# danielzgtg/TTS.cpp

Measured on AMD Instinct MI355X. Metric: audio-sec/wall-sec (RTF^-1), Parler-TTS-mini v1 Q4_K AR decode + DAC decode, higher is better.
Workload: dtype q4_K weights x q8_K activations (int dot, f32 combine); DAC f16 im2col x f32 weights, f64 accumulate

## Files before the change

### include/tts_hip.h

```cpp
#ifndef TTS_HIP_H
#define TTS_HIP_H

#include <stddef.h>
#include <stdint.h>

#ifdef __cplusplus
extern "C" {
#endif

#define TTS_MAX_DIMS 4
#define TTS_MAX_SRC 4
#define TTS_MAX_OP_PARAMS 16
#define TTS_MAX_NAME 64

enum tts_type {
    TTS_TYPE_F32 = 0,
    TTS_TYPE_F16 = 1,
    TTS_TYPE_Q4_0 = 2,
    TTS_TYPE_Q4_1 = 3,
    TTS_TYPE_Q5_0 = 6,
    TTS_TYPE_Q5_1 = 7,
    TTS_TYPE_Q8_0 = 8,
    TTS_TYPE_Q8_1 = 9,
    TTS_TYPE_Q4_K = 12,
// ... 50 lines not shown
};

enum tts_custom_op {
    TTS_CUSTOM_NONE = 0,
    TTS_CUSTOM_UV_NOISE = 1,
    TTS_CUSTOM_CFG_SCALE = 2
};

enum tts_unary_op {
    TTS_UNARY_ABS = 0,
    TTS_UNARY_NEG,
    TTS_UNARY_TANH,
    TTS_UNARY_RELU,
    TTS_UNARY_SIGMOID,
    TTS_UNARY_GELU,
    TTS_UNARY_SILU,
    TTS_UNARY_EXP,
    TTS_UNARY_COUNT
};

enum tts_status {
    TTS_STATUS_SUCCESS = 0,
    TTS_STATUS_FAILED = -1,
    TTS_STATUS_ALLOC_FAILED = -2,
    TTS_STATUS_UNSUPPORTED = -3,
    TTS_STATUS_BAD_ARG = -4,
    TTS_STATUS_NO_DEVICE = -5
};

#define TTS_PROF_ATTN 39

#define TTS_FLAG_INPUT 1
#define TTS_FLAG_HOSTDATA 2
#define TTS_FLAG_OUTPUT 4
#define TTS_FLAG_PERSIST 8
#define TTS_FLAG_REPACKED 16
#define TTS_FLAG_TILED_COPY 64
#define TTS_FLAG_TILED 32

typedef struct tts_tensor {
    int32_t type;
    int32_t op;
    int64_t ne[TTS_MAX_DIMS];
    size_t nb[TTS_MAX_DIMS];
    int32_t op_params[TTS_MAX_OP_PARAMS];
    struct tts_tensor * src[TTS_MAX_SRC];
    struct tts_tensor * view_src;
    size_t view_offs;
    void * data;
    int32_t flags;
    int32_t pad_;
    char name[TTS_MAX_NAME];
} tts_tensor;

size_t tts_type_size(int type);
int64_t tts_blck_size(int type);
size_t tts_row_size(int type, int64_t ne0);
const char * tts_type_name(int type);
const char * tts_op_name(int op);

typedef struct tts_hip_backend * tts_hip_backend_t;

int tts_hip_device_count(void);
int tts_hip_device_memory(int device, size_t * free_bytes, size_t * total_bytes);
void * tts_hip_event_new(int device);
void tts_hip_event_free(void * event);
int tts_hip_event_record(tts_hip_backend_t backend, void * event);
int tts_hip_event_wait(tts_hip_backend_t backend, void * event);
int tts_hip_event_synchronize(void * event);
int tts_hip_is_device_pointer(const void * p);
tts_hip_backend_t tts_hip_backend_init(int device);
void tts_hip_backend_free(tts_hip_backend_t backend);
const char * tts_hip_backend_name(tts_hip_backend_t backend);

void * tts_hip_buffer_alloc(tts_hip_backend_t backend, size_t size);
void tts_hip_buffer_free(tts_hip_backend_t backend, void * ptr);
size_t tts_hip_buffer_alignment(void);

int tts_hip_tensor_set(tts_hip_backend_t backend, void * dst_dev, const void * src_host, size_t size);
int tts_hip_tensor_get(tts_hip_backend_t backend, void * dst_host, const void * src_dev, size_t size);
int tts_hip_tensor_copy(tts_hip_backend_t backend, void * dst_dev, const void * src_dev, size_t size);
int tts_hip_copy_stream(tts_hip_backend_t backend, void * dst_dev, const void * src_dev, size_t size);
int tts_hip_plan_stats(tts_tensor * const * nodes, int n_nodes, int mask, int32_t * counts);
int tts_hip_tensor_set_async(tts_hip_backend_t backend, void * dst_dev, const void * src_host, size_t size);
int tts_hip_memset(tts_hip_backend_t backend, void * dst_dev, int value, size_t size);
int tts_hip_synchronize(tts_hip_backend_t backend);

int tts_hip_weight_set(tts_hip_backend_t backend, tts_tensor * t, const void * src_host);
int tts_hip_weight_get(tts_hip_backend_t backend, const tts_tensor * t, void * dst_host);
int tts_hip_quantize(tts_hip_backend_t backend, int type, const float * x_dev, void * dst_dev, int64_t rows, int64_t K);
void tts_repack_q4_K(const void * src, void * dst, int64_t nblocks, int inverse);
void tts_repack_q4_K_tiled(const void * src, void * dst, int64_t nrows, int64_t nb, int inverse);

int tts_hip_supports_op(const tts_tensor * node);
int tts_hip_graph_compute(tts_hip_backend_t backend, tts_tensor * const * nodes, int n_nodes);
int tts_hip_graph_prepare(tts_hip_backend_t backend, tts_tensor * const * nodes, int n_nodes, int slot);
int tts_hip_graph_launch(tts_hip_backend_t backend, int slot);

enum tts_hip_option {
    TTS_HIP_OPT_FUSION = 0,
    TTS_HIP_OPT_PROFILE_GEMV = 1,
    TTS_HIP_OPT_GRAPHS = 2,
    TTS_HIP_OPT_CONV_F32ACC = 3,
    TTS_HIP_OPT_CONVT_LDS = 4,
    TTS_HIP_OPT_ATTN_SPLIT = 5,
    TTS_HIP_OPT_KV_PREFETCH = 6,
    TTS_HIP_OPT_KV_PREFETCH_BLOCKS = 7,
    TTS_HIP_OPT_Q4K_TILE_BYTES = 8,
    TTS_HIP_OPT_GEMV_DEBUG = 10,
    TTS_HIP_OPT_CONV_SPLIT = 12,
    TTS_HIP_OPT_GEMV_UNIQUE = 11,
    TTS_HIP_OPT_GEMV_KS = 13,
    TTS_HIP_OPT_ATTN_FUSED = 14,
    TTS_HIP_OPT_GEMM_Q8 = 18,
    TTS_HIP_OPT_BGEMM_F32 = 19,
    TTS_HIP_OPT_CU_PARTITION = 20,
    TTS_HIP_OPT_Q4K_DUAL_BYTES = 16,
    TTS_HIP_OPT_GEMV_RSPLIT = 17,
    TTS_HIP_OPT_ATTN_PV16 = 15,
    TTS_HIP_OPT_GEMV_PREQUANT = 21,
    TTS_HIP_OPT_GEMV_KRELAY = 22,
    TTS_HIP_OPT_ATTN_KS = 23,
    TTS_HIP_OPT_ATTN_PV8 = 24,
    TTS_HIP_OPT_GEMV_KRELAY_LOOP = 26,
    TTS_HIP_OPT_GEMV_Q80_PRO = 27,
    TTS_HIP_OPT_GEMV_Q80_SLAB = 28,
    TTS_HIP_OPT_GEMV_Q80_RW = 29,
    TTS_HIP_OPT_GEMM_Q8_STAGED = 30,
    TTS_HIP_OPT_GEMV_KR_INKERNEL = 31,
    TTS_HIP_OPT_GEMV_F32_WIDE = 32,
    TTS_HIP_OPT_ATTN_PV_MP = 33,
    TTS_HIP_OPT_GEMM_KR_INKERNEL = 35,
    TTS_HIP_OPT_GEMM_KR_CT2 = 36,
    TTS_HIP_OPT_GEMM_KR_NW = 34,
    TTS_HIP_OPT_GEMV_NW_MIN = 25,
    TTS_HIP_OPT_GEMM_KR_XCD = 38,
    TTS_HIP_OPT_GEMM_KR_CP = 39,
    TTS_HIP_OPT_GEMM_KR_WALK = 40,
    TTS_HIP_OPT_GEMM_PF = 41,
    TTS_HIP_OPT_GEMM_PF_NW = 42,
    TTS_HIP_OPT_ATTN_ONE = 43,
    TTS_HIP_OPT_GEMV_KR_TAIL = 44,
    TTS_HIP_OPT_GEMV_Q50_SLAB = 45,
    TTS_HIP_OPT_GEMV_Q50_RW = 46,
    TTS_HIP_OPT_GEMM_Q5 = 47,
    TTS_HIP_OPT_GEMM_Q5_STAGED = 48,
    TTS_HIP_OPT_GEMV_Q40_SLAB = 49,
    TTS_HIP_OPT_GEMV_Q40_RW = 50,
    TTS_HIP_OPT_GEMM_Q4_0 = 51,
    TTS_HIP_OPT_GEMM_Q4_0_STAGED = 52,
    TTS_HIP_OPT_CONV_VFMA = 53,
    TTS_HIP_OPT_CONV_TILE96 = 54,
    TTS_HIP_OPT_CONV_PACK = 55,
    TTS_HIP_OPT_COALESCE = 37,
};
enum tts_fuse_bits {
    TTS_FUSE_LN = 1, TTS_FUSE_GROUP = 2, TTS_FUSE_KV = 4, TTS_FUSE_EPI = 8, TTS_FUSE_HEADS = 16, TTS_FUSE_ATTN = 32,
    TTS_FUSE_LSTM = 64,
    TTS_FUSE_SNAKE = 128,
    TTS_FUSE_EMBED = 256,
    TTS_FUSE_CONV = 512,
    TTS_FUSE_ADAIN = 1024,
    TTS_FUSE_XATTN = 2048,
    TTS_FUSE_MCPY = 4096,
    TTS_FUSE_CONTREAD = 8192
};
int tts_hip_set_option(tts_hip_backend_t backend, int option, int value);
int tts_hip_attn_decode(tts_hip_backend_t backend, const tts_tensor * q, const tts_tensor * k, const tts_tensor * v,
                        const float * mask, int64_t mbs, float scale, float * out, float * out2, const int64_t * koff,
                        const int64_t * voff, const int64_t * moff, const int32_t * pseq);
int tts_hip_coalesce_stats(int device, int64_t * out, int n);
void tts_hip_coalesce_set_wait(int us);
int tts_hip_coalesce_enable(int on);
#define TTS_HIP_HOOK_FAULT_WEIGHT_SET 1
int tts_hip_test_hook(int hook, int value);
int tts_hip_install_crash_handler(void);
int tts_hip_gemv_stats(tts_hip_backend_t backend, int type, double * ms, int64_t * launches, double * bytes, int reset);
int tts_hip_greedy_step(tts_hip_backend_t backend, const float * logits, int32_t B, int32_t NH, int32_t V, int32_t step,
                        int32_t bos, int32_t eos, int32_t * eos_seen, int32_t * hist, int32_t * next);
typedef struct tts_sampling {
    float temperature;
    float top_p;
    float repetition_penalty;
    int32_t top_k;
    int32_t do_sample;
    int32_t pad_;
    uint64_t seed;
} tts_sampling;
void tts_sampling_default(tts_sampling * cfg);
uint32_t tts_sampler_call_seed(uint64_t seed, int32_t stream, int64_t call);
int tts_sampler_sample(const tts_sampling * cfg, const float * logits, int32_t NH, int32_t V, uint32_t call_seed, int32_t * last,
                       int32_t * count, int32_t * out);
int tts_hip_sample_step(tts_hip_backend_t backend, const float * logits, int32_t B, int32_t NH, int32_t V, const tts_sampling * cfg,
                        int64_t call, int32_t * rep_state, int32_t step, int32_t bos, int32_t eos, int32_t * eos_seen, int32_t * hist,
                        int32_t * next);
int tts_sampling_device_ok(const tts_sampling * cfg, int32_t V);
int tts_hip_counters(tts_hip_backend_t backend, int64_t * out, int n);

int tts_hip_gemv(tts_hip_backend_t backend, int type, const void * w, const float * x, float * y,
                 int64_t K, int64_t N, int64_t M);
int tts_hip_gemv_ex(tts_hip_backend_t backend, int type, const void * w, const float * x, float * y,
                    int64_t K, int64_t N, int64_t M, int32_t wflags);
int tts_hip_gemv_res(tts_hip_backend_t backend, int type, const void * w, const float * x, float * y, const float * res,
                     int64_t K, int64_t N, int64_t M, int32_t wflags);

typedef struct tts_backend_iface {
    void * ctx;
    const char * name;
    void * (*alloc)(void * ctx, size_t size);
    void (*free)(void * ctx, void * ptr);
    int (*set)(void * ctx, void * dst, const void * src, size_t size);
    int (*set_tensor)(void * ctx, tts_tensor * t, const void * src);
    int (*get)(void * ctx, void * dst, const void * src, size_t size);
    int (*memset)(void * ctx, void * dst, int value, size_t size);
    int (*compute)(void * ctx, tts_tensor * const * nodes, int n_nodes);
    int (*synchronize)(void * ctx);
    int (*prepare)(void * ctx, tts_tensor * const * nodes, int n_nodes, int slot);
    int (*launch)(void * ctx, int slot);
    int (*set_async)(void * ctx, void * dst, const void * src, size_t size);
    int (*copy)(void * ctx, void * dst, const void * src, size_t size);
    int (*greedy_step)(void * ctx, const float * logits, int B, int NH, int V, int step, int bos, int eos, int32_t * eos_seen,
                       int32_t * hist, int32_t * next);
    int (*sample_step)(void * ctx, const float * logits, int B, int NH, int V, const tts_sampling * cfg, int64_t call, int32_t * rep_state,
                       int step, int bos, int eos, int32_t * eos_seen, int32_t * hist, int32_t * next);
} tts_backend_iface;

int tts_hip_backend_iface(tts_hip_backend_t backend, tts_backend_iface * out);

#ifdef __cplusplus
}
#endif

#endif
```

### tts.cpp_amd/csrc/backend.hip

```cpp
#include <cmath>
#include <atomic>
#include <cstring>
#include <map>
#include <mutex>
#include <thread>

#include "hip_internal.h"
#include <hip/hip_ext.h>

#include <dlfcn.h>
#include <execinfo.h>
#include <fcntl.h>
#include <signal.h>
#include <unistd.h>

using namespace tts;


static void build_gelu_table(uint16_t * t) {
    const float GELU_COEF_A = 0.044715f;
    const float SQRT_2_OVER_PI = 0.79788456080286535587989211986876f;
    for (int i = 0; i < 65536; ++i) {
        const float x = fp16_to_fp32_host((uint16_t)i);
        const float g = 0.5f * x * (1.0f + tanhf(SQRT_2_OVER_PI * x * (1.0f + GELU_COEF_A * x * x)));
// ... 5 lines not shown
static const size_t kShadowBytes = 4u << 20;
static const size_t kLstmFloats = 4u << 20;
static const size_t kAttnFloats = 4u << 20;
static const size_t kVecScratchFloats = 1u << 18;
static const size_t kPinBytes = 16u << 20;

namespace {
std::mutex g_reg_mu;
struct BufRec {
    size_t size = 0;
};
std::map<const char *, BufRec> g_buffers;
std::unordered_map<const void *, uint8_t *> g_tiled;
std::atomic<size_t> g_tiled_n{0};
struct PackRec {
    float * img = nullptr;
    size_t src_bytes = 0;
};
std::map<tts::ConvPackKey, PackRec> g_packs;
std::atomic<size_t> g_packs_n{0};
std::atomic<size_t> g_packs_bytes{0};
std::atomic<uintptr_t> g_packs_lo{UINTPTR_MAX}, g_packs_hi{0};
}

namespace tts {
const uint8_t * tiled_copy_find(const void * w) {
    std::lock_guard<std::mutex> lk(g_reg_mu);
    auto it = g_tiled.find(w);
    return it == g_tiled.end() ? nullptr : it->second;
}
static std::atomic<int> g_coalesce_on{[] {
    const char * e = getenv("TTS_HIP_COALESCE");
    return e && e[0] == '0' ? 0 : 1;
}()};
bool coalesce_enabled() { return g_coalesce_on.load(std::memory_order_relaxed) != 0; }
const float * conv_pack_get(tts_hip_backend * be, const ConvPackKey & k) {
    std::lock_guard<std::mutex> lk(g_reg_mu);
    auto it = g_packs.find(k);
    if (it != g_packs.end()) return it->second.img;
    if (be->capturing) return nullptr;
    PackRec r;
    const size_t es = k.w16 ? 2 : 4;
    r.src_bytes = (size_t)((k.K - 1) * k.wk + (k.IC - 1) * k.wic + (k.OC - 1) * k.woc + 1) * es;
    const size_t bytes = k.floats() * sizeof(float);
    if (hipMalloc((void **)&r.img, bytes) != hipSuccess) {
        (void)hipGetLastError();
        return nullptr;
    }
    launch_conv1d_pack(be->stream, k, r.img);
    g_packs[k] = r;
    g_packs_lo.store(std::min(g_packs_lo.load(), (uintptr_t)k.w));
    g_packs_hi.store(std::max(g_packs_hi.load(), (uintptr_t)k.w + r.src_bytes));
    g_packs_n.store(g_packs.size(), std::memory_order_release);
    g_packs_bytes.fetch_add(bytes, std::memory_order_relaxed);
    return r.img;
}
void conv_pack_written(tts_hip_backend * be, const void * p, size_t n) {
    if (g_packs_n.load(std::memory_order_acquire) == 0) return;
    const char * a = (const char *)p;
    if ((uintptr_t)a >= g_packs_hi.load() || (uintptr_t)a + n <= g_packs_lo.load()) return;
    std::lock_guard<std::mutex> lk(g_reg_mu);
    for (auto & e : g_packs) {
        const char * w = (const char *)e.first.w;
        if (!(w < a + n && a < w + e.second.src_bytes)) continue;
        const tts_hip_backend * ob = e.first.be;
        if (ob->device == be->device) {
            launch_conv1d_pack(be->stream, e.first, e.second.img);
        } else {
            hipStreamSynchronize(be->stream);
            hipSetDevice(ob->device);
            launch_conv1d_pack(ob->stream, e.first, e.second.img);
            hipSetDevice(be->device);
        }
    }
}
void conv_pack_freed(const tts_hip_backend * be, const void * p, size_t n) {
    if (g_packs_n.load(std::memory_order_acquire) == 0) return;
    const char * a = (const char *)p;
    std::vector<float *> dead;
    {
        std::lock_guard<std::mutex> lk(g_reg_mu);
        for (auto it = g_packs.begin(); it != g_packs.end();) {
            const char * w = (const char *)it->first.w;
            if (be ? it->first.be == be : (w >= a && w < a + n)) {
                dead.push_back(it->second.img);
                g_packs_bytes.fetch_sub(it->first.floats() * sizeof(float), std::memory_order_relaxed);
                it = g_packs.erase(it);
            } else {
                ++it;
            }
        }
        if (g_packs.empty()) g_packs_lo.store(UINTPTR_MAX), g_packs_hi.store(0);
        g_packs_n.store(g_packs.size(), std::memory_order_release);
    }
    if (dead.empty()) return;
    hipDeviceSynchronize();
    for (float * c : dead) hipFree(c);
}
bool buffer_lookup(const void * p, const char ** base, size_t * size) {
    std::lock_guard<std::mutex> lk(g_reg_mu);
    auto it = g_buffers.upper_bound((const char *)p);
    if (it == g_buffers.begin()) return false;
    --it;
    if ((const char *)p >= it->first + it->second.size) return false;
    if (base) *base = it->first;
    if (size) *size = it->second.size;
    return true;
}
}

extern "C" {

int tts_hip_coalesce_enable(int on) { return tts::g_coalesce_on.exchange(on ? 1 : 0); }

int tts_hip_device_count(void) {
    int n = 0;
    if (hipGetDeviceCount(&n) != hipSuccess) return 0;
    return n;
}

tts_hip_backend_t tts_hip_backend_init(int device) {
    int n = tts_hip_device_count();
    if (device < 0 || device >= n) return nullptr;
    if (hipSetDevice(device) != hipSuccess) return nullptr;
    auto * be = new tts_hip_backend();
    be->device = device;
    TTS_HIP_CHECK(hipStreamCreateWithFlags(&be->stream, hipStreamNonBlocking));
    TTS_HIP_CHECK(hipStreamCreateWithFlags(&be->cap_stream, hipStreamNonBlocking));
    TTS_HIP_CHECK(hipStreamCreateWithFlags(&be->pf_stream, hipStreamNonBlocking));
    TTS_HIP_CHECK(hipEventCreateWithFlags(&be->co_ev, hipEventDisableTiming));
    TTS_HIP_CHECK(hipEventCreateWithFlags(&be->pf_fork, hipEventDisableTiming));
    TTS_HIP_CHECK(hipEventCreateWithFlags(&be->pf_join, hipEventDisableTiming));
    hipDeviceProp_t prop;
    TTS_HIP_CHECK(hipGetDeviceProperties(&prop, device));
    snprintf(be->name, sizeof(be->name), "HIP%d(%s)", device, prop.gcnArchName);
    be->cu_total = prop.multiProcessorCount > 0 ? prop.multiProcessorCount : 256;
    be->cus = be->cu_total;
    TTS_HIP_CHECK(hipMalloc((void **)&be->scratch, kScratchBytes));
    be->scratch_size = kScratchBytes;
    TTS_HIP_CHECK(hipMalloc((void **)&be->shadow, kShadowBytes));
    be->shadow_size = kShadowBytes;
    be->hoist_size = (size_t)8 << 20;
    TTS_HIP_CHECK(hipMalloc(&be->hoist, be->hoist_size));
    TTS_HIP_CHECK(hipMalloc((void **)&be->lstm_buf, kLstmFloats * sizeof(float)));
    TTS_HIP_CHECK(hipMalloc((void **)&be->attn_buf, kAttnFloats * sizeof(float)));
    be->attn_floats = kAttnFloats;
    TTS_HIP_CHECK(hipMalloc((void **)&be->vec_scratch, kVecScratchFloats * sizeof(float)));
    be->conv_stage_floats = (size_t)8 << 20;
    TTS_HIP_CHECK(hipMalloc((void **)&be->conv_stage, be->conv_stage_floats * sizeof(float)));
    if (const char * e = getenv("TTS_HIP_OPT_CONV_VFMA"))
        if (e[0] >= '0' && e[0] <= '2' && !e[1]) be->conv_vfma = e[0] - '0';
    if (const char * e = getenv("TTS_HIP_OPT_CONV_PACK"))
        if (e[0] >= '0' && e[0] <= '1' && !e[1]) be->conv_pack = e[0] - '0';
    be->conv_part_doubles = (size_t)8 << 20;
    TTS_HIP_CHECK(hipMalloc((void **)&be->conv_part, be->conv_part_doubles * sizeof(double)));
    be->lstm_floats = kLstmFloats;
    TTS_HIP_CHECK(hipMalloc((void **)&be->argmax_keys, kArgmaxRows * sizeof(unsigned long long)));
    TTS_HIP_CHECK(hipMalloc((void **)&be->argmax_counts, kArgmaxRows * sizeof(unsigned)));
    TTS_HIP_CHECK(hipMemset(be->argmax_keys, 0, kArgmaxRows * sizeof(unsigned long long)));
    TTS_HIP_CHECK(hipMemset(be->argmax_counts, 0, kArgmaxRows * sizeof(unsigned)));
    TTS_HIP_CHECK(hipHostMalloc((void **)&be->pin, kPinBytes, hipHostMallocDefault));
    be->pin_size = kPinBytes;
    for (auto & e : be->plan_ev) TTS_HIP_CHECK(hipEventCreateWithFlags(&e, hipEventDisableTiming));
    std::vector<uint16_t> tab(65536);
    build_gelu_table(tab.data());
    TTS_HIP_CHECK(hipMalloc((void **)&be->gelu_table, 65536 * sizeof(uint16_t)));
    TTS_HIP_CHECK(hipMemcpy(be->gelu_table, tab.data(), 65536 * sizeof(uint16_t), hipMemcpyHostToDevice));
    return be;
}

void tts_hip_backend_free(tts_hip_backend_t be) {
    if (!be) return;
    tts::coalesce_backend_gone(be);
    hipSetDevice(be->device);
    hipStreamSynchronize(be->stream);
    tts::conv_pack_freed(be, nullptr, 0);
    for (auto & p : be->ev_pending) {
        hipEventDestroy(p.first);
        hipEventDestroy(p.second);
    }
    for (auto e : be->ev_free) hipEventDestroy(e);
    for (auto & r : be->pin_pending) hipEventDestroy(r.ev);
    for (auto e : be->pin_events) hipEventDestroy(e);
    for (auto e : be->plan_ev) hipEventDestroy(e);
    hipHostFree(be->pin);
    if (be->rb_host) hipHostFree(be->rb_host);
    hipFree(be->scratch);
    hipFree(be->shadow);
    hipFree(be->argmax_keys);
    hipFree(be->argmax_counts);
    hipFree(be->lstm_buf);
    hipFree(be->hoist);
    hipFree(be->attn_buf);
    hipFree(be->vec_scratch);
    hipFree(be->conv_stage);
    hipFree(be->conv_part);
    hipFree(be->gelu_table);
    if (be->sample_cand) hipFree(be->sample_cand);
    if (be->repack_tmp) hipFree(be->repack_tmp);
    for (char * r : be->repack_retired) hipFree(r);
    if (be->attn_stage) hipFree(be->attn_stage);
    for (auto & ex : be->gsig_exec)
        if (ex) hipGraphExecDestroy(ex);
    for (auto & ex : be->pexec)
        if (ex) hipGraphExecDestroy(ex);
    hipStreamDestroy(be->stream);
    hipStreamDestroy(be->cap_stream);
    hipStreamDestroy(be->pf_stream);
    hipEventDestroy(be->pf_fork);
    hipEventDestroy(be->pf_join);
    hipEventDestroy(be->co_ev);
    delete be;
}

const char * tts_hip_backend_name(tts_hip_backend_t be) { return be ? be->name : "HIP(null)"; }

int tts_hip_device_memory(int device, size_t * free_bytes, size_t * total_bytes) {
    if (device < 0 || device >= tts_hip_device_count()) return TTS_STATUS_NO_DEVICE;
    int prev = 0;
    hipGetDevice(&prev);
    hipSetDevice(device);
    size_t f = 0, t = 0;
    const hipError_t e = hipMemGetInfo(&f, &t);
    hipSetDevice(prev);
    if (e != hipSuccess) return TTS_STATUS_FAILED;
    if (free_bytes) *free_bytes = f;
    if (total_bytes) *total_bytes = t;
    return 0;
}

void * tts_hip_event_new(int device) {
    if (device < 0 || device >= tts_hip_device_count()) return nullptr;
    hipSetDevice(device);
    hipEvent_t ev = nullptr;
    if (hipEventCreateWithFlags(&ev, hipEventDisableTiming) != hipSuccess) return nullptr;
    return (void *)ev;
}
void tts_hip_event_free(void * event) {
    if (event) hipEventDestroy((hipEvent_t)event);
}
int tts_hip_event_record(tts_hip_backend_t be, void * event) {
    if (!be || !event) return TTS_STATUS_BAD_ARG;
    hipSetDevice(be->device);
    return hipEventRecord((hipEvent_t)event, be->stream) == hipSuccess ? 0 : TTS_STATUS_FAILED;
}
int tts_hip_event_wait(tts_hip_backend_t be, void * event) {
    if (!be || !event) return TTS_STATUS_BAD_ARG;
    hipSetDevice(be->device);
    return hipStreamWaitEvent(be->stream, (hipEvent_t)event, 0) == hipSuccess ? 0 : TTS_STATUS_FAILED;
}
int tts_hip_event_synchronize(void * event) {
    if (!event) return TTS_STATUS_BAD_ARG;
    return hipEventSynchronize((hipEvent_t)event) == hipSuccess ? 0 : TTS_STATUS_FAILED;
}
int tts_hip_is_device_pointer(const void * p) {
    if (!p) return 0;
    hipPointerAttribute_t a;
    if (hipPointerGetAttributes(&a, p) != hipSuccess) {
        (void)hipGetLastError();
        return 0;
    }
    return a.type == hipMemoryTypeDevice ? 1 : 0;
}

size_t tts_hip_buffer_alignment(void) { return 256; }

void * tts_hip_buffer_alloc(tts_hip_backend_t be, size_t size) {
    if (!be) return nullptr;
    hipSetDevice(be->device);
    void * p = nullptr;
    BufRec r;
    r.size = size ? size : 256;
    if (hipMalloc(&p, r.size) != hipSuccess) return nullptr;
    std::lock_guard<std::mutex> lk(g_reg_mu);
    g_buffers[(const char *)p] = r;
    return p;
}

static void drop_tiled_copies(const void * p, size_t n) {
    if (g_tiled_n.load(std::memory_order_acquire) == 0) return;
    const char * a = (const char *)p;
    std::vector<uint8_t *> dead;
    {
        std::lock_guard<std::mutex> lk(g_reg_mu);
        for (auto it = g_tiled.begin(); it != g_tiled.end();) {
            const char * k = (const char *)it->first;
            if (k >= a && k < a + n) {
                dead.push_back(it->second);
                it = g_tiled.erase(it);
            } else {
                ++it;
            }
        }
        g_tiled_n.store(g_tiled.size(), std::memory_order_release);
    }
    if (dead.empty()) return;
    hipDeviceSynchronize();
    for (uint8_t * c : dead) hipFree(c);
}

void tts_hip_buffer_free(tts_hip_backend_t be, void * ptr) {
    if (!be || !ptr) return;
    hipSetDevice(be->device);
    hipStreamSynchronize(be->stream);
    BufRec r;
    bool known = false;
// ... 324 lines not shown
        l0 = l1 + 1;
    }
    const struct sigaction & prev = sig == SIGBUS ? g_prev_bus : g_prev_segv;
    if (prev.sa_flags & SA_SIGINFO) {
        if (prev.sa_sigaction) prev.sa_sigaction(sig, si, uc);
    } else if (prev.sa_handler != SIG_DFL && prev.sa_handler != SIG_IGN && prev.sa_handler) {
        prev.sa_handler(sig);
    }
    signal(sig, SIG_DFL);
    raise(sig);
}

int tts_hip_install_crash_handler(void) {
    void * warm[2];
    (void)backtrace(warm, 2);
    struct sigaction sa;
    memset(&sa, 0, sizeof sa);
    sa.sa_sigaction = crash_handler;
    sa.sa_flags = SA_SIGINFO | SA_RESETHAND;
    sigemptyset(&sa.sa_mask);
    if (sigaction(SIGSEGV, &sa, &g_prev_segv) != 0 || sigaction(SIGBUS, &sa, &g_prev_bus) != 0) return TTS_STATUS_FAILED;
    return 0;
}

int tts_hip_test_hook(int hook, int value) {
    if (hook == TTS_HIP_HOOK_FAULT_WEIGHT_SET) {
        g_fault_weight_set.store(value != 0);
        return 0;
    }
    return TTS_STATUS_BAD_ARG;
}

int tts_hip_weight_set(tts_hip_backend_t be, tts_tensor * t, const void * src) {
    if (!be || !t) return TTS_STATUS_BAD_ARG;
    if (t->type == TTS_TYPE_Q4_K && g_fault_weight_set.load(std::memory_order_relaxed)) return TTS_STATUS_ALLOC_FAILED;
    return weight_set_impl(be, t, src);
}

static int weight_set_impl(tts_hip_backend_t be, tts_tensor * t, const void * src) {
    const size_t n = tensor_bytes(t);
    if (t->type == TTS_TYPE_Q4_K && t->ne[0] % 256 == 0 && t->ne[1] % 4 == 0 && t->ne[2] == 1 && t->ne[3] == 1 &&
        be->q4k_tile_bytes > 0 && (int64_t)n >= be->q4k_tile_bytes) {
        std::vector<uint8_t> tmp(n);
        tts_repack_q4_K_tiled(src, tmp.data(), t->ne[1], t->ne[0] / 256, 0);
        int st = tts_hip_tensor_set(be, t->data, tmp.data(), n);
        if (st == 0) t->flags |= TTS_FLAG_REPACKED | TTS_FLAG_TILED;
        return st;
    }
    if (t->type == TTS_TYPE_Q4_K && t->ne[0] % 256 == 0) {
        std::vector<uint8_t> tmp(n);
        tts_repack_q4_K(src, tmp.data(), (int64_t)(n / 144), 0);
        t->flags &= ~TTS_FLAG_TILED_COPY;
        int st = tts_hip_tensor_set(be, t->data, tmp.data(), n);
        if (st == 0) t->flags |= TTS_FLAG_REPACKED;
        if (st == 0 && be->q4k_dual_bytes > 0 && (int64_t)n >= be->q4k_dual_bytes && t->ne[0] >= 2048 && t->ne[1] % 16 == 0 &&
            t->ne[2] == 1 && t->ne[3] == 1) {
            tts_repack_q4_K_tiled(src, tmp.data(), t->ne[1], t->ne[0] / 256, 0);
            uint8_t * cp = nullptr;
            if (hipMalloc((void **)&cp, n) != hipSuccess) return TTS_STATUS_ALLOC_FAILED;
            if (hipMemcpy(cp, tmp.data(), n, hipMemcpyHostToDevice) != hipSuccess) {
                hipFree(cp);
                return TTS_STATUS_FAILED;
            }
            {
                std::lock_guard<std::mutex> lk(g_reg_mu);
                g_tiled[t->data] = cp;
                g_tiled_n.store(g_tiled.size(), std::memory_order_release);
            }
            t->flags |= TTS_FLAG_TILED_COPY;
        }
        return st;
    }
    return tts_hip_tensor_set(be, t->data, src, n);
}

int tts_hip_weight_get(tts_hip_backend_t be, const tts_tensor * t, void * dst) {
    if (!be || !t) return TTS_STATUS_BAD_ARG;
    const size_t n = tensor_bytes(t);
    if (t->type == TTS_TYPE_Q4_K && (t->flags & TTS_FLAG_TILED)) {
        std::vector<uint8_t> tmp(n);
        int st = tts_hip_tensor_get(be, tmp.data(), t->data, n);
        if (st == 0) tts_repack_q4_K_tiled(tmp.data(), dst, t->ne[1], t->ne[0] / 256, 1);
        return st;
    }
    if (t->type == TTS_TYPE_Q4_K && (t->flags & TTS_FLAG_REPACKED)) {
        std::vector<uint8_t> tmp(n);
        int st = tts_hip_tensor_get(be, tmp.data(), t->data, n);
        if (st == 0) tts_repack_q4_K(tmp.data(), dst, (int64_t)(n / 144), 1);
        return st;
    }
    return tts_hip_tensor_get(be, dst, t->data, n);
}

static bool is_f32(const tts_tensor * t) { return t && t->type == TTS_TYPE_F32; }

int tts_hip_supports_op(const tts_tensor * n) {
    if (!n) return 0;
    for (int i = 0; i < TTS_MAX_SRC; ++i)
        if (n->src[i] && (n->src[i]->flags & 2)) return 0;
    switch (n->op) {
        case TTS_OP_NONE: case TTS_OP_VIEW: case TTS_OP_RESHAPE: case TTS_OP_PERMUTE: case TTS_OP_TRANSPOSE:
            return 1;
        case TTS_OP_DUP: case TTS_OP_CONT: case TTS_OP_CPY:
            return (n->type == TTS_TYPE_F32 || n->type == TTS_TYPE_F16 || n->type == TTS_TYPE_I32) &&
                   (n->src[0]->type == TTS_TYPE_F32 || n->src[0]->type == TTS_TYPE_F16 || n->src[0]->type == TTS_TYPE_I32);
        case TTS_OP_ADD: case TTS_OP_SUB: case TTS_OP_MUL: case TTS_OP_DIV:
        case TTS_OP_SQR: case TTS_OP_SQRT: case TTS_OP_SIN: case TTS_OP_COS: case TTS_OP_SCALE: case TTS_OP_CLAMP:
        case TTS_OP_LEAKY_RELU: case TTS_OP_ROUND: case TTS_OP_MOD: case TTS_OP_UNARY: case TTS_OP_CONCAT:
        case TTS_OP_REPEAT: case TTS_OP_SUM_ROWS:
            return 1;
        case TTS_OP_NORM: case TTS_OP_RMS_NORM:
            return is_f32(n->src[0]) && n->src[0]->nb[0] == 4;
        case TTS_OP_SOFT_MAX:
            return is_f32(n->src[0]);
        case TTS_OP_ROPE:
            return is_f32(n->src[0]);
        case TTS_OP_IM2COL:
            return is_f32(n->src[1]) && n->op_params[6] == 0 && (n->type == TTS_TYPE_F16 || n->type == TTS_TYPE_F32);
        case TTS_OP_CONV_TRANSPOSE_1D:
            return is_f32(n->src[0]) && is_f32(n->src[1]) && n->op_params[4] >= 1;
        case TTS_OP_CUMSUM: case TTS_OP_UPSCALE: case TTS_OP_STFT: case TTS_OP_ISTFT: case TTS_OP_MAP_CUSTOM3: case TTS_OP_MAP_CUSTOM2:
            return tts::audio_op_supported(n);
        case TTS_OP_GET_ROWS:
            return n->src[1]->type == TTS_TYPE_I32 &&
                   (n->src[0]->type == TTS_TYPE_F32 || n->src[0]->type == TTS_TYPE_F16 || n->src[0]->type == TTS_TYPE_Q4_K ||
                    n->src[0]->type == TTS_TYPE_Q8_0 || n->src[0]->type == TTS_TYPE_Q5_0 || n->src[0]->type == TTS_TYPE_Q4_0 ||
                    (n->src[0]->type == TTS_TYPE_Q6_K && n->src[0]->ne[0] % 256 == 0));
        case TTS_OP_MUL_MAT: {
            const tts_tensor * a = n->src[0];
            const tts_tensor * b = n->src[1];
            if (!is_f32(b)) return 0;
            if (a->ne[0] != b->ne[0] || b->ne[2] % a->ne[2] || b->ne[3] % a->ne[3]) return 0;
            if (a->type == TTS_TYPE_F32 || a->type == TTS_TYPE_F16) return 1;
            if (a->type == TTS_TYPE_Q4_K || a->type == TTS_TYPE_Q6_K) return a->ne[0] % 256 == 0;
            if (a->type == TTS_TYPE_Q8_0 || a->type == TTS_TYPE_Q5_0 || a->type == TTS_TYPE_Q4_0) return a->ne[0] % 32 == 0;
            return 0;
        }
        default:
            return 0;
    }
}

}

extern "C" int tts_hip_set_option(tts_hip_backend_t be, int option, int value) {
    if (!be) return TTS_STATUS_BAD_ARG;
    switch (option) {
        case TTS_HIP_OPT_FUSION: be->fusion = value; return 0;
        case TTS_HIP_OPT_CONVT_LDS: be->convt_lds = value != 0; return 0;
        case TTS_HIP_OPT_CONV_SPLIT: be->conv_split = value < 0 ? 1 : value; return 0;
        case TTS_HIP_OPT_CONV_VFMA: be->conv_vfma = value < 0 || value > 2 ? 1 : value; return 0;
        case TTS_HIP_OPT_CONV_TILE96: be->conv_tile96 = value != 0; return 0;
        case TTS_HIP_OPT_CONV_PACK: be->conv_pack = value != 0; return 0;
        case TTS_HIP_OPT_PROFILE_GEMV: be->profile_gemv = value != 0; return 0;
        case TTS_HIP_OPT_GRAPHS: be->use_graphs = value != 0; return 0;
        case TTS_HIP_OPT_CONV_F32ACC:
            be->conv_f32acc = value == 1;
            be->conv_acc_mode = value == 2 ? 2 : 0;
            return 0;
        case TTS_HIP_OPT_ATTN_SPLIT: be->attn_split_minp = value; return 0;
        case TTS_HIP_OPT_ATTN_FUSED: be->attn_fused_minp = value; return 0;
        case TTS_HIP_OPT_ATTN_PV16: be->attn_pv_uv16 = value != 0; return 0;
        case TTS_HIP_OPT_KV_PREFETCH: be->kv_prefetch_minp = value; return 0;
        case TTS_HIP_OPT_Q4K_TILE_BYTES: be->q4k_tile_bytes = value; return 0;
        case TTS_HIP_OPT_Q4K_DUAL_BYTES: be->q4k_dual_bytes = value; return 0;
        case TTS_HIP_OPT_GEMV_RSPLIT: be->gemv_mf_rsplit = value != 0; return 0;
        case TTS_HIP_OPT_GEMV_PREQUANT: be->gemv_mf_prequant = value != 0; return 0;
        case TTS_HIP_OPT_GEMV_KRELAY: be->gemv_kr = value != 0; return 0;
        case TTS_HIP_OPT_GEMV_KRELAY_LOOP: be->gemv_kr_loop = value != 0; return 0;
        case TTS_HIP_OPT_GEMV_Q80_PRO: be->gemv_q80_pro = value != 0; return 0;
        case TTS_HIP_OPT_GEMV_Q80_SLAB: be->gemv_q80_slab = value != 0; return 0;
        case TTS_HIP_OPT_GEMV_KR_INKERNEL:
            if (value < 0) return TTS_STATUS_BAD_ARG;
            be->gemv_kr_ink = value;
            return 0;
        case TTS_HIP_OPT_GEMM_Q8_STAGED:
            if (value < 0 || value > 2) return TTS_STATUS_BAD_ARG;
            be->gemm_q8_staged = value;
            return 0;
        case TTS_HIP_OPT_GEMV_Q80_RW:
            if (value < 0 || value > 32 || (value & (value - 1))) return TTS_STATUS_BAD_ARG;
            be->gemv_q80_rw = value;
            return 0;
        case TTS_HIP_OPT_GEMV_Q50_SLAB: be->gemv_q50_slab = value != 0; return 0;
        case TTS_HIP_OPT_GEMV_Q50_RW:
            if (value < 0 || value > 32 || (value & (value - 1))) return TTS_STATUS_BAD_ARG;
            be->gemv_q50_rw = value;
            return 0;
        case TTS_HIP_OPT_GEMM_Q5: be->gemm_q5 = value != 0; return 0;
        case TTS_HIP_OPT_GEMM_Q5_STAGED:
            if (value < 0 || value > 2) return TTS_STATUS_BAD_ARG;
            be->gemm_q5_staged = value;
            return 0;
        case TTS_HIP_OPT_GEMV_Q40_SLAB: be->gemv_q40_slab = value != 0; return 0;
        case TTS_HIP_OPT_GEMV_Q40_RW:
            if (value < 0 || value > 32 || (value & (value - 1))) return TTS_STATUS_BAD_ARG;
            be->gemv_q40_rw = value;
            return 0;
        case TTS_HIP_OPT_GEMM_Q4_0: be->gemm_q4_0 = value != 0; return 0;
        case TTS_HIP_OPT_GEMM_Q4_0_STAGED:
            if (value < 0 || value > 2) return TTS_STATUS_BAD_ARG;
            be->gemm_q4_0_staged = value;
            return 0;
        case TTS_HIP_OPT_ATTN_KS: be->attn_ks = value; return 0;
        case TTS_HIP_OPT_GEMV_NW_MIN: be->gemv_nw_min = value; return 0;
        case TTS_HIP_OPT_ATTN_PV8: be->attn_pv8 = value != 0; return 0;
        case TTS_HIP_OPT_GEMM_KR_CT2: be->gemm_kr_ct2 = value != 0; return 0;
        case TTS_HIP_OPT_GEMM_KR_INKERNEL: be->gemm_kr_ink = value < 0 ? 0 : value; return 0;
        case TTS_HIP_OPT_ATTN_PV_MP: be->attn_pv_mp = value == 2 ? 2 : value != 0; return 0;
        case TTS_HIP_OPT_ATTN_ONE:
            if (value < 0 || value > 2) return TTS_STATUS_BAD_ARG;
            be->attn_one = value;
            return 0;
        case TTS_HIP_OPT_GEMV_KR_TAIL:
            if (value < 0 || value > 4) return TTS_STATUS_BAD_ARG;
            be->gemv_kr_tail = value;
            return 0;
        case TTS_HIP_OPT_GEMM_KR_NW: be->gemm_kr_nw = value == 8 ? 8 : 4; return 0;
        case TTS_HIP_OPT_GEMM_Q8: be->gemm_q8 = value != 0; return 0;
        case TTS_HIP_OPT_CU_PARTITION: {
            const int count = value & 0xFF, index = (value >> 8) & 0xFF;
            const bool inter = (value >> 16) & 1;
            hipSetDevice(be->device);
            TTS_HIP_CHECK(hipStreamSynchronize(be->stream));
            hipStream_t ns = nullptr;
            if (count <= 1) {
                TTS_HIP_CHECK(hipStreamCreateWithFlags(&ns, hipStreamNonBlocking));
                be->cus = be->cu_total;
            } else {
                if (index >= count) return TTS_STATUS_BAD_ARG;
                std::vector<uint32_t> mask((be->cu_total + 31) / 32, 0u);
                const int per = be->cu_total / count;
                int n = 0;
                for (int c = 0; c < be->cu_total; ++c) {
                    const bool on = inter ? (c % count == index) : (c / per == index && c < per * count);
                    if (on) mask[c / 32] |= 1u << (c % 32), ++n;
                }
                if (hipExtStreamCreateWithCUMask(&ns, (uint32_t)mask.size(), mask.data()) != hipSuccess) return TTS_STATUS_FAILED;
                be->cus = n;
            }
            TTS_HIP_CHECK(hipStreamDestroy(be->stream));
            be->stream = ns;
            for (auto & ex : be->gsig_exec)
                if (ex) hipGraphExecDestroy(ex), ex = nullptr;
            for (auto & g : be->gsig) g = 0;
            return 0;
        }
        case TTS_HIP_OPT_BGEMM_F32: be->bgemm_f32 = value != 0; return 0;
        case TTS_HIP_OPT_GEMV_F32_WIDE: be->gemv_f32_wide = value != 0; return 0;
        case TTS_HIP_OPT_GEMV_DEBUG: be->gemv_dbg = value; return 0;
        case TTS_HIP_OPT_GEMV_UNIQUE: be->gemv_unique = value != 0; return 0;
        case TTS_HIP_OPT_GEMV_KS: be->gemv_ks_tiles = value > 0 ? value : 0; return 0;
        case TTS_HIP_OPT_COALESCE: be->co_member = value != 0; return 0;
        case TTS_HIP_OPT_GEMM_KR_XCD: be->gemm_kr_xcd = value != 0; return 0;
        case TTS_HIP_OPT_GEMM_KR_CP: be->gemm_kr_cp = value != 0; return 0;
        case TTS_HIP_OPT_GEMM_KR_WALK: be->gemm_kr_walk = value < 0 ? 0 : value; return 0;
        case TTS_HIP_OPT_GEMM_PF: be->gemm_pf = value < 0 ? 0 : value; return 0;
        case TTS_HIP_OPT_GEMM_PF_NW: be->gemm_pf_nw = value == 8 ? 8 : 4; return 0;
        case TTS_HIP_OPT_KV_PREFETCH_BLOCKS: be->kv_prefetch_blocks = value > 0 ? value : 1; return 0;
        default: return TTS_STATUS_BAD_ARG;
    }
}

extern "C" int tts_hip_counters(tts_hip_backend_t be, int64_t * out, int n) {
    if (!be || !out) return TTS_STATUS_BAD_ARG;
    const int64_t v[10] = {be->graph_updates, be->graph_instantiations, be->lstm_chains, be->lstm_steps, be->plan_wait_ns,
                           be->cap_plan_ns, be->cap_launch_ns, be->cap_update_ns, (int64_t)g_packs_n.load(), (int64_t)g_packs_bytes.load()};
    int k = 0;
    for (; k < n && k < 10; ++k) out[k] = v[k];
    return k;
}

extern "C" int tts_hip_gemv_stats(tts_hip_backend_t be, int type, double * ms, int64_t * launches, double * bytes, int reset) {
    if (!be) return TTS_STATUS_BAD_ARG;
    hipSetDevice(be->device);
    TTS_HIP_CHECK(hipStreamSynchronize(be->stream));
    for (size_t i = 0; i < be->ev_pending.size(); ++i) {
        float t = 0;
        TTS_HIP_CHECK(hipEventElapsedTime(&t, be->ev_pending[i].first, be->ev_pending[i].second));
        const int ty = be->ev_type[i];
        be->gemv_ms[ty] += t;
        be->gemv_launches[ty] += 1;
        be->gemv_bytes[ty] += be->ev_bytes[i];
        be->ev_free.push_back(be->ev_pending[i].first);
        be->ev_free.push_back(be->ev_pending[i].second);
    }
    be->ev_pending.clear();
    be->ev_bytes.clear();
    be->ev_type.clear();
    double a = 0, c = 0;
    int64_t b = 0;
    for (int ty = 0; ty < TTS_TYPE_COUNT; ++ty) {
        if (type >= 0 && ty != type) continue;
        a += be->gemv_ms[ty];
        b += be->gemv_launches[ty];
        c += be->gemv_bytes[ty];
    }
    if (ms) *ms = a;
    if (launches) *launches = b;
    if (bytes) *bytes = c;
    if (reset) {
        for (int ty = 0; ty < TTS_TYPE_COUNT; ++ty) {
            be->gemv_ms[ty] = 0;
            be->gemv_launches[ty] = 0;
            be->gemv_bytes[ty] = 0;
        }
// ... 47 lines not shown
```

### tts.cpp_amd/csrc/graph_exec.hip

```cpp
#include <algorithm>
#include <cstring>
#include <deque>
#include <unordered_map>
#include <vector>

#include <array>

#include "hip_internal.h"
#include <chrono>

using namespace tts;

namespace tts {
void launch_kv_prefetch(tts_hip_backend * be, hipStream_t st, const TD & t, int pdim, int blocks);
void launch_gemv_q4K_xattn(tts_hip_backend * be, const GemvJob & j, const XAttnArgs & a);
void launch_attn_decode(tts_hip_backend * be, const TD & q, const TD & k, const TD & v, const float * mask, float scale,
                        float * out, int hd, int P, int H, int n, int B, float * out2, int64_t obs = -1, int64_t mbs = 0,
                        const int64_t * koff = nullptr, const int64_t * voff = nullptr, const int64_t * moff = nullptr,
                        const int * pseq = nullptr);
void launch_attn_bias(tts_hip_backend * be, const TD & q, const TD & k, const TD & v, const float * bias, const float * mask,
                      float scale, float * out, int P, int H, int n);
void launch_layernorm(tts_hip_backend * be, const tts_tensor * dst, const tts_tensor * x, const float * w, const float * b,
                      float eps, bool rms);
}
// ... 1160 lines not shown
                it.snake_mask = m;
                act[index[x]] = -1;
            }
        }
        act[index[M1]] = act[index[S]] = act[index[Q]] = act[index[M2]] = -1;
        if (rfuse) {
            it.b = nullptr;
            it.snake_one = O;
            act[index[R]] = -1;
        }
        act[i] = add_item(std::move(it));
    }

    static bool vec_c(const tts_tensor * t, int64_t C) {
        if (!t || t->type != TTS_TYPE_F32 || t->ne[2] * t->ne[3] != 1 || t->nb[0] != 4) return false;
        return (t->ne[0] == C && t->ne[1] == 1) || (t->ne[0] == 1 && t->ne[1] == C && t->nb[1] == 4);
    }
    static bool same_shape(const tts_tensor * a, int64_t n0, int64_t n1) {
        return a->type == TTS_TYPE_F32 && a->ne[0] == n0 && a->ne[1] == n1 && a->ne[2] * a->ne[3] == 1;
    }
    static bool plan_debug() {
        static const bool dbg = getenv("TTS_PLAN_DEBUG") != nullptr;
        return dbg;
    }
    static void plan_reject(const char * what, int code) {
        if (plan_debug()) fprintf(stderr, "plan: %s not fused (check %d)\n", what, code);
    }
    static bool adain_fail(int code) {
        plan_reject("adain", code);
        return false;
    }
    bool try_adain(int i) {
        const tts_tensor * N = nodes[i];
        const tts_tensor * X = N->src[0];
        if (!X || X->type != TTS_TYPE_F32 || N->type != TTS_TYPE_F32 || X->nb[0] != 4 || N->ne[2] * N->ne[3] != 1) return adain_fail(1);
        const int64_t T = N->ne[0], C = N->ne[1];
        if (!adain_supported(T)) return adain_fail(2);
        const tts_tensor * T1 = sole_consumer(N);
        if (!T1 || T1->op != TTS_OP_TRANSPOSE) return adain_fail(3);
        const tts_tensor * C1 = sole_consumer(T1);
        if (!C1 || C1->op != TTS_OP_CONT || !same_shape(C1, C, T) || uses[C1] != 2) return adain_fail(4);
        const auto & cc = consumers[C1];
        if (cc.size() != 2) return adain_fail(5);
        const tts_tensor *M = nodes[cc[0]], *A1 = nodes[cc[1]];
        if (M->op != TTS_OP_MUL || M->src[0] != C1 || !vec_c(M->src[1], C) || sole_consumer(M) != A1) return adain_fail(6);
        if (A1->op != TTS_OP_ADD || A1->src[0] != C1 || A1->src[1] != M || !same_shape(A1, C, T)) return adain_fail(7);
        const tts_tensor * A2 = sole_consumer(A1);
        if (!A2 || A2->op != TTS_OP_ADD || A2->src[0] != A1 || !vec_c(A2->src[1], C) || !same_shape(A2, C, T)) return adain_fail(8);
        const tts_tensor * T2 = sole_consumer(A2);
        if (!T2 || T2->op != TTS_OP_TRANSPOSE) return adain_fail(9);
        const tts_tensor * C2 = sole_consumer(T2);
        if (!C2 || C2->op != TTS_OP_CONT || !same_shape(C2, T, C) || !contiguous(C2)) return adain_fail(10);
        const tts_tensor *gamma = M->src[1], *beta = A2->src[1];
        std::vector<int> absorbed = {i, index[C1], index[M], index[A1], index[A2], index[C2]};
        auto affine_src = [&](const tts_tensor * v, const tts_tensor * user, const tts_tensor *& W, const tts_tensor *& B,
                              const tts_tensor *& st) {
            if (!v || v->op != TTS_OP_ADD || sole_consumer(v) != user) return false;
            const tts_tensor * mm = v->src[0];
            if (!mm || mm->op != TTS_OP_MUL_MAT || sole_consumer(mm) != v || !vec_c(v->src[1], C) || v->src[1]->ne[0] != C) return false;
            W = mm->src[0], st = mm->src[1], B = v->src[1];
            const int64_t S = W->ne[0];
            return W->type == TTS_TYPE_F32 && contiguous(W) && W->ne[1] == C && W->ne[2] * W->ne[3] == 1 && S % 4 == 0 &&
                   ((uintptr_t)W->data % 16) == 0 && st->type == TTS_TYPE_F32 && contiguous(st) && st->ne[0] == S &&
                   st->ne[1] * st->ne[2] * st->ne[3] == 1 && ((uintptr_t)st->data % 16) == 0;
        };
        const tts_tensor *gW = nullptr, *gB = nullptr, *gS = nullptr, *bW = nullptr, *bB = nullptr, *bS = nullptr;
        const bool inline_gb = affine_src(gamma, M, gW, gB, gS) && affine_src(beta, A2, bW, bB, bS) && gS == bS;
        if (inline_gb) {
            for (const tts_tensor * t : {gamma, (const tts_tensor *)gamma->src[0], beta, (const tts_tensor *)beta->src[0]}) absorbed.push_back(index[t]);
            gamma = beta = nullptr;
        }
        const tts_tensor * out = C2;
        const tts_tensor *alpha = nullptr, *recip = nullptr, *one = nullptr;
        if ((mask & TTS_FUSE_SNAKE) && uses[C2] == 2) {
            const auto & sc = consumers[C2];
            const tts_tensor *M1 = nodes[sc[0]], *SA = nodes[sc[1]];
            const tts_tensor *S = sole_consumer(M1), *Q = S ? sole_consumer(S) : nullptr, *M2 = Q ? sole_consumer(Q) : nullptr;
            const tts_tensor * R = M2 ? M2->src[1] : nullptr;
            const tts_tensor * O = R ? R->src[0] : nullptr;
            const bool r_inline = R && R->op == TTS_OP_DIV && O && R->src[1] == M1->src[1] && sole_consumer(R) == M2 &&
                                  O->type == TTS_TYPE_F32 && O->nb[1] == 0 && O->ne[0] == 1 && O->ne[2] * O->ne[3] == 1 &&
                                  same_shape(R, 1, C);
            if (M1->op == TTS_OP_MUL && M1->src[0] == C2 && S && S->op == TTS_OP_SIN && Q && Q->op == TTS_OP_SQR && M2 &&
                M2->op == TTS_OP_MUL && M2->src[0] == Q && sole_consumer(M2) == SA && SA->op == TTS_OP_ADD && SA->src[0] == C2 &&
                SA->src[1] == M2 && vec_c(M1->src[1], C) && vec_c(M2->src[1], C) && same_shape(SA, T, C) && contiguous(SA) &&
                same_shape(M1, T, C) && same_shape(S, T, C) && same_shape(Q, T, C) && same_shape(M2, T, C)) {
                alpha = M1->src[1];
                recip = M2->src[1];
                out = SA;
                for (const tts_tensor * t : {M1, S, Q, M2, SA}) absorbed.push_back(index[t]);
                if (r_inline) {
                    absorbed.push_back(index[R]);
                    recip = nullptr;
                    one = O;
                }
            }
        }
        const bool in_place = out->data == X->data && out->nb[1] == X->nb[1];
        if (overlap(out, X) && !in_place) return adain_fail(11);
        bool stage = false;
        for (const tts_tensor * t : {gamma, beta, alpha, recip, one})
            if (t && overlap(out, t)) stage = true;
        if (inline_gb)
            for (const tts_tensor * t : {gW, gB, bW, bB, gS})
                if (overlap(out, t)) return adain_fail(14);
        if (stage && 4 * C + 1 > (int64_t)vec_cap) return adain_fail(12);
        const int last = *std::max_element(absorbed.begin(), absorbed.end());
        std::vector<bool> is_abs(n, false);
        for (int k : absorbed) is_abs[k] = true;
        for (int k = i + 1; k < last; ++k) {
            if (is_abs[k] || is_view(nodes[k]->op)) continue;
            const tts_tensor * w = nodes[k];
            for (const tts_tensor * t : {X, gamma, beta, alpha, recip, one, gW, gB, bW, bB, gS})
                if (t && t != w && overlap(w, t)) {
                    if (plan_debug()) fprintf(stderr, "plan: adain node %d (%s) between %d..%d overlaps an input\n", k, tts_op_name(w->op), i, last);
                    return adain_fail(13);
                }
        }
        AdainArgs a;
        a.x = (const float *)X->data;
        a.xcs = (int64_t)(X->nb[1] / 4);
        a.y = (float *)out->data;
        a.ycs = (int64_t)(out->nb[1] / 4);
        auto vstride = [](const tts_tensor * t) { return t->ne[0] == 1 ? (int64_t)(t->nb[1] / 4) : (int64_t)1; };
        if (inline_gb) {
            a.gw = (const float *)gW->data, a.gb = (const float *)gB->data;
            a.bw = (const float *)bW->data, a.bb = (const float *)bB->data;
            a.style = (const float *)gS->data, a.S = gW->ne[0];
        } else {
            a.gamma = (const float *)gamma->data, a.gcs = vstride(gamma);
            a.beta = (const float *)beta->data, a.bcs = vstride(beta);
        }
        if (alpha) {
            a.alpha = (const float *)alpha->data, a.acs = vstride(alpha);
            if (recip) a.recip = (const float *)recip->data, a.rcs = vstride(recip);
            else a.one = (const float *)one->data;
        }
        a.T = T, a.C = C;
        a.stage = stage;
        memcpy(&a.eps, &N->op_params[0], 4);
        Item it;
        it.kind = Item::ADAIN;
        it.adain = a;
        it.dst = out;
        for (int k : absorbed)
            if (k != last) act[k] = -1;
        act[last] = add_item(std::move(it));
        return true;
    }

    static const tts_tensor * through_view(const tts_tensor * t) { return t && t->op == TTS_OP_RESHAPE ? t->src[0] : t; }
    bool wr_hull = false;
    const char *wr_lo = nullptr, *wr_hi = nullptr;
    void try_conv(int i) {
        const tts_tensor * col = nodes[i];
        const tts_tensor *kern = col->src[0], *x = col->src[1];
        if (col->type != TTS_TYPE_F16 || col->op_params[6] != 0 || col->ne[2] * col->ne[3] != 1) return plan_reject("conv", 1);
        if (!x || x->type != TTS_TYPE_F32 || x->ne[2] * x->ne[3] != 1) return plan_reject("conv", 2);
        if (!kern || (kern->type != TTS_TYPE_F32 && kern->type != TTS_TYPE_F16) || kern->ne[3] != 1) return plan_reject("conv", 3);
        const tts_tensor * cv = sole_consumer(col);
        if (!cv || cv->op != TTS_OP_RESHAPE || !contiguous(col)) return plan_reject("conv", 4);
        const tts_tensor * mm = sole_consumer(cv);
        if (!mm || mm->op != TTS_OP_MUL_MAT || mm->src[0] != cv || mm->type != TTS_TYPE_F32) return plan_reject("conv", 5);
        const tts_tensor * wv = mm->src[1];
        if (!wv || through_view(wv) != kern) return plan_reject("conv", 6);
        const int K = (int)kern->ne[0];
        const int64_t IC = kern->ne[1], OC = kern->ne[2], L = x->ne[0], OL = col->ne[1];
        if (x->ne[1] != IC || mm->ne[0] != OL || mm->ne[1] != OC || !contiguous(mm)) return plan_reject("conv", 7);
        const int s = col->op_params[0], p = col->op_params[2], d = col->op_params[4];
        if (!conv1d_fused_ok(IC, K, s, d, nullptr)) return plan_reject("conv", 8);
        if (kern->nb[0] != tts_type_size(kern->type)) return plan_reject("conv", 9);
        const tts_tensor * out = mm;
        std::vector<int> absorbed = {i, (int)index[mm]};
        const tts_tensor * r3 = sole_consumer(mm);
        const tts_tensor * cur = mm;
        if (r3 && r3->op == TTS_OP_RESHAPE && r3->ne[0] == OL && r3->ne[1] == OC) cur = r3;
        Conv1dArgs a;
        const tts_tensor * bias = nullptr;
        const tts_tensor * res = nullptr;
        const tts_tensor * nb = sole_consumer(cur);
        if (nb && nb->op == TTS_OP_ADD && nb->src[0] == cur && nb->type == TTS_TYPE_F32 && contiguous(nb) && nb->ne[0] == OL &&
            nb->ne[1] == OC && nb->ne[2] * nb->ne[3] == 1 && chan_vec(nb->src[1], OC) && nb->src[1]->ne[1] == OC) {
            bias = nb->src[1];
            out = nb;
            absorbed.push_back(index[nb]);
            const tts_tensor * nr = sole_consumer(nb);
            if (nr && nr->op == TTS_OP_ADD && nr->type == TTS_TYPE_F32 && contiguous(nr) && nr->ne[0] == OL && nr->ne[1] == OC &&
                nr->ne[2] * nr->ne[3] == 1) {
                const tts_tensor * other = nr->src[0] == nb ? nr->src[1] : nr->src[0];
                if (other && other != nb && other->type == TTS_TYPE_F32 && contiguous(other) && other->ne[0] == OL && other->ne[1] == OC &&
                    other->ne[2] * other->ne[3] == 1 && (!overlap(nr, other) || nr->data == other->data)) {
                    res = other;
                    out = nr;
                    absorbed.push_back(index[nr]);
                }
            }
        }
        float * stage = nullptr;
        for (;;) {
            if (overlap(out, kern) || (bias && overlap(out, bias))) return plan_reject("conv", 10);
            stage = nullptr;
            bool ok = true;
            bool in_col = false;
            if (overlap(out, x)) {
                const size_t need = (size_t)OL * (size_t)OC * 4;
                if (tbytes(col) >= need && !overlap(col, x) && !overlap(col, out) && !(res && overlap(col, res)) && !overlap(col, kern) &&
                    !(bias && overlap(col, bias))) {
                    stage = (float *)col->data;
                    in_col = true;
                } else if (conv_stage && need <= 4 * conv_stage_cap) {
                    stage = conv_stage;
                } else {
                    ok = false;
                }
            }
            for (int j = i + 1; ok && j < absorbed.back(); ++j) {
                if (std::find(absorbed.begin(), absorbed.end(), j) != absorbed.end() || is_view(nodes[j]->op)) continue;
                if (overlap(nodes[j], x) || (in_col && overlap(nodes[j], col))) ok = false;
            }
            if (ok) break;
            if (!res) return plan_reject("conv", 11);
            res = nullptr;
            absorbed.pop_back();
            out = bias ? nb : mm;
        }
        a.x = make_td(x);
        a.w = kern->data;
        a.w16 = kern->type == TTS_TYPE_F16;
        const size_t es = tts_type_size(kern->type);
        a.wk = (int64_t)(kern->nb[0] / es), a.wic = (int64_t)(kern->nb[1] / es), a.woc = (int64_t)(kern->nb[2] / es);
        a.y = (float *)out->data;
        a.ycs = (int64_t)(out->nb[1] / 4);
        if (stage) {
            a.copy_dst = a.y;
            a.y = stage;
            a.ycs = OL;
        }
        if (bias) a.bias = (const float *)bias->data, a.bcs = bias->ne[1] == 1 ? 0 : (int64_t)(bias->nb[1] / 4);
        if (res) a.res = (const float *)res->data, a.rcs = (int64_t)(res->nb[1] / 4);
        a.L = L, a.IC = IC, a.OL = OL, a.OC = OC;
        a.K = K, a.s = s, a.p = p, a.d = d;
        const size_t xb = (size_t)((x->ne[0] - 1) * x->nb[0] + (x->ne[1] - 1) * x->nb[1]) + 4;
        const size_t wb = tbytes(kern);
        if (xb >= 0x80000000u || wb >= 0x80000000u) return plan_reject("conv", 12);
        a.x_bytes = (uint32_t)xb, a.w_bytes = (uint32_t)wb;
        a.w_stable = kern->op == TTS_OP_NONE && !(kern->flags & (TTS_FLAG_HOSTDATA | TTS_FLAG_OUTPUT)) && buffer_lookup(kern->data, nullptr, nullptr);
        if (a.w_stable && !wr_hull) {
            wr_hull = true;
            for (int j = 0; j < n; ++j) {
                if (is_view(nodes[j]->op) || !nodes[j]->data) continue;
                const char * lo = (const char *)nodes[j]->data;
                wr_lo = wr_lo ? std::min(wr_lo, lo) : lo;
                wr_hi = std::max(wr_hi, lo + tbytes(nodes[j]));
            }
        }
        if (a.w_stable && wr_lo && (const char *)kern->data < wr_hi && (const char *)kern->data + wb > wr_lo)
            for (int j = 0; a.w_stable && j < n; ++j)
                if (!is_view(nodes[j]->op) && nodes[j]->data && overlap(nodes[j], kern)) a.w_stable = 0;
        Item it;
        it.kind = Item::CONV;
        it.conv = a;
        it.dst = out;
        for (size_t k = 0; k + 1 < absorbed.size(); ++k) act[absorbed[k]] = -1;
        act[absorbed.back()] = add_item(std::move(it));
    }

    bool embed_terms(const tts_tensor * a, const tts_tensor * root, std::vector<const tts_tensor *> & terms, std::vector<int> & members) {
        if (a->op != TTS_OP_ADD || a->type != TTS_TYPE_F32) return false;
        for (int d = 0; d < 4; ++d)
            if (a->ne[d] != root->ne[d]) return false;
        const tts_tensor *l = a->src[0], *r = a->src[1];
        if (!l || !r) return false;
        const bool la = l->op == TTS_OP_ADD, ra = r->op == TTS_OP_ADD;
        if (la && ra) return false;
        auto leaf_ok = [&](const tts_tensor * g) {
            if (g->op != TTS_OP_GET_ROWS || sole_consumer(g) != a || g->type != TTS_TYPE_F32) return false;
            const tts_tensor *tab = g->src[0], *idx = g->src[1];
            if (tab->type != TTS_TYPE_F32 && tab->type != TTS_TYPE_F16 && tab->type != TTS_TYPE_Q8_0 && tab->type != TTS_TYPE_Q5_0 && tab->type != TTS_TYPE_Q4_0 && tab->type != TTS_TYPE_Q4_K && tab->type != TTS_TYPE_Q6_K) return false;
            if (idx->type != TTS_TYPE_I32 || idx->ne[1] * idx->ne[2] * idx->ne[3] != 1 || (idx->nb[0] % 4)) return false;
            if (tab->ne[0] != root->ne[0] || g->ne[0] != root->ne[0] || tab->ne[2] * tab->ne[3] != 1) return false;
            const int64_t rows = g->ne[1] * g->ne[2] * g->ne[3], M = root->ne[1] * root->ne[2] * root->ne[3];
            return idx->ne[0] == rows && (rows == 1 || rows == M);
        };
        if (la || ra) {
            const tts_tensor * inner = la ? l : r;
            const tts_tensor * leaf = la ? r : l;
            if (sole_consumer(inner) != a || !leaf_ok(leaf)) return false;
            if (!embed_terms(inner, root, terms, members)) return false;
            terms.push_back(leaf);
            members.push_back(index[leaf]);
            members.push_back(index[inner]);
            return true;
        }
        if (!leaf_ok(l) || !leaf_ok(r)) return false;
        terms.push_back(l);
        terms.push_back(r);
        members.push_back(index[l]);
        members.push_back(index[r]);
        return true;
    }
    void try_rint(int i) {
        const tts_tensor * R = nodes[i];
        if (R->type != TTS_TYPE_F32 || R->op_params[0] != 1 || !contiguous(R)) return;
        std::vector<const tts_tensor *> leaves;
        std::vector<int> members{i};
        const tts_tensor * t = R;
        while (t->op == TTS_OP_CONCAT && t->op_params[0] == 1) {
            leaves.push_back(t->src[1]);
            t = t->src[0];
            if (t->op == TTS_OP_CONCAT) {
                if (uses[t] != 1 || !index.count(t)) return;
                members.push_back(index[t]);
            }
        }
        leaves.push_back(t);
        std::reverse(leaves.begin(), leaves.end());
        const tts_tensor * a = nullptr;
        int64_t r = 0;
        for (size_t k = 0; k < leaves.size(); ++k) {
            const tts_tensor * rp = leaves[k];
            if (rp->op != TTS_OP_REPEAT || uses[rp] != 1 || !index.count(rp)) return;
            const tts_tensor * c = rp->src[0];
            if (!c || c->op != TTS_OP_CONT || uses[c] != 1 || !index.count(c)) return;
            const tts_tensor * v = c->src[0];
            if (!v || v->op != TTS_OP_VIEW || !v->view_src || v->ne[1] != 1) return;
            const tts_tensor * base = v->view_src;
            if (k == 0) {
                a = base;
                r = rp->ne[1];
                if (a->type != TTS_TYPE_F32 || (int64_t)leaves.size() != a->ne[1]) return;
            }
            if (base != a || rp->ne[1] != r || (const char *)v->data != (const char *)a->data + k * a->nb[1]) return;
            for (int d = 0; d < 4; ++d)
                if (d != 1 && (v->ne[d] != a->ne[d] || v->nb[d] != a->nb[d] || rp->ne[d] != a->ne[d])) return;
            members.push_back(index[rp]);
            members.push_back(index[c]);
        }
        if (!a || R->ne[1] != a->ne[1] * r || overlap(R, a)) return;
        for (int m : members)
            if (act[m] != 0) return;
        const int first = *std::min_element(members.begin(), members.end());
        for (int j = first + 1; j < i; ++j) {
            if (is_view(nodes[j]->op) || std::find(members.begin(), members.end(), j) != members.end()) continue;
            if (overlap(nodes[j], a)) return;
        }
        Item it;
        it.kind = Item::RINT;
        it.x = a;
        it.dst = R;
        it.rint = (int)r;
        for (int m : members) act[m] = -1;
        if (a->op == TTS_OP_CONT && a->src[0] && index.count(a) && act[index[a]] == 0) {
            const tts_tensor * s0 = a->src[0];
            bool ok = s0->type == TTS_TYPE_F32 && !overlap(R, s0);
            for (int d = 0; d < 4; ++d) ok &= s0->ne[d] == a->ne[d];
            auto ca = consumers.find(a);
            ok &= ca != consumers.end();
            if (ok)
                for (int k : ca->second) {
                    const tts_tensor * v = nodes[k];
                    const tts_tensor * u = sole_consumer(v);
                    ok &= v->op == TTS_OP_VIEW && u && std::find(members.begin(), members.end(), index[u]) != members.end();
                }
            const int ia = ok ? index[a] : 0;
            for (int j = ia + 1; ok && j < i; ++j) {
                if (is_view(nodes[j]->op) || std::find(members.begin(), members.end(), j) != members.end()) continue;
                if (overlap(nodes[j], s0)) ok = false;
            }
            if (ok) {
                it.x = s0;
                act[ia] = -1;
            }
        }
        rint_to_cpy(i, R, it);
        act[i] = add_item(std::move(it));
    }

    void rint_to_cpy(int i, const tts_tensor * R, Item & it) {
        const tts_tensor * X = sole_consumer(R);
        std::vector<int> skip;
        while (X && X->op == TTS_OP_RESHAPE && X->src[0] && contiguous(X)) X = sole_consumer(X);
        if (X && X->op == TTS_OP_CONT && contiguous(X) && index.count(X) && act[index[X]] == 0) {
            skip.push_back(index[X]);
            X = sole_consumer(X);
        }
        if (!X || X->op != TTS_OP_CPY || !index.count(X) || act[index[X]] != 0) return;
        const int iP = index[X];
        skip.push_back(iP);
        const tts_tensor * D = X;
        if (D->type != TTS_TYPE_F32 || D->nb[0] != 4 || D->ne[0] != R->ne[0] * R->ne[1] * R->ne[2] || D->ne[1] != R->ne[3] ||
            D->ne[2] != 1 || D->ne[3] != 1 || overlap(D, it.x))
            return;
        for (int j = i + 1; j < iP; ++j)
            if (!is_view(nodes[j]->op) && std::find(skip.begin(), skip.end(), j) == skip.end()) return;
        tts_tensor t = *R;
        t.data = D->data;
        t.nb[0] = 4;
        t.nb[1] = 4 * R->ne[0];
        t.nb[2] = t.nb[1] * R->ne[1];
        t.nb[3] = D->nb[1];
        it.node = t;
        it.rint_cpy = true;
        for (int k : skip) act[k] = -1;
    }

    void try_gather_t(int i) {
        const tts_tensor * C2 = nodes[i];
        const tts_tensor * Tv = C2->src[0];
        if (!Tv || Tv->op != TTS_OP_TRANSPOSE || C2->type != TTS_TYPE_F32 || !contiguous(C2) || uses[Tv] != 1) return;
        const tts_tensor * G = Tv->view_src ? Tv->view_src : Tv->src[0];
        if (!G || G->op != TTS_OP_GET_ROWS || !index.count(G) || act[index[G]] != 0 || uses[G] != 1 || G->type != TTS_TYPE_F32 ||
// ... 930 lines not shown
                        CO_NO();
                    pseq = (int *)&tab[of[3]];
                    pseq[k] = (int)mk->ne[1];
                    pmax = std::max(pmax, (int)mk->ne[1]);
                    ragged |= mk->ne[1] != it.k->ne[1];
                    if (it.mask) {
                        const tts_tensor * mm = cm.member(bc, it.mask, k);
                        if (!mm || mm->ne[0] != mk->ne[1] || mm->ne[1] < it.q->ne[1]) CO_NO();
                    }
                }
                tb.pmax = pmax;
                bc.ragged |= ragged;
                for (int w = 0; w < 2; ++w) {
                    const tts_tensor * kv = w ? it.v : it.k;
                    if (inter(kv)) {
                        if (ragged) CO_NO();
                        continue;
                    }
                    if (bc.stride(kv->data)) CO_NO();
                    of[1 + w] = alloc(N);
                    if (!offsets(kv, of[1 + w], 16)) CO_NO();
                    for (int k = 0; k < N; ++k) tab[of[1 + w] + k] *= 16;
                }
                if (it.mask) {
                    if (inter(it.mask)) {
                        if (ragged) CO_NO();
                    } else {
                        of[4] = alloc(N);
                        if (!offsets(it.mask, of[4], 4)) CO_NO();
                    }
                }
                break;
            }
            case Item::LN:
                if (it.dst->ne[3] != 1 || it.x->ne[3] != 1 || !inter(it.dst) || !inter(it.x) || !equal_all(it.dst) || !equal_all(it.x)) CO_NO();
                if (!share(it.w) || !share(it.b)) CO_NO();
                break;
            case Item::EMBED:
                if (it.gather_t || it.dst->ne[1] * it.dst->ne[2] * it.dst->ne[3] != 1 || !inter(it.dst) || !equal_all(it.dst)) CO_NO();
                if (it.terms.size() > (size_t)EMBED_MAX_TERMS) CO_NO();
                for (size_t t = 0; t < it.terms.size(); ++t) {
                    const tts_tensor * g = it.terms[t];
                    if (g->ne[1] * g->ne[2] * g->ne[3] != 1 || !equal_all(g) || !share(g->src[0])) CO_NO();
                    const tts_tensor * idx = g->src[1];
                    if (inter(idx)) continue;
                    if (!input_mem(idx) || !equal_all(idx)) CO_NO();
                    ioffs[a - 1][t] = alloc(N);
                    if (!offsets(idx, ioffs[a - 1][t], 4)) CO_NO();
                }
                break;
            case Item::NODE: {
                auto * e = cm.pos.find(nd);
                if (!e) CO_NO();
                cm.pos[&it.node] = e->second;
                if (!equal_all(nd)) CO_NO();
                for (int s2 = 0; s2 < TTS_MAX_SRC; ++s2) {
                    const tts_tensor * x = it.node.src[s2];
                    if (!x) continue;
                    if (!cm.pos.find(x) && owned_mem(x)) CO_NO();
                    if (cm.pos.find(x) && !equal_all(x)) CO_NO();
                }
                if (co_per_slice(bc, &it.node))
                    for (int s2 = 0; s2 < TTS_MAX_SRC; ++s2)
                        if (it.node.src[s2] && owned_mem(it.node.src[s2]) && !share(it.node.src[s2])) CO_NO();
                break;
            }
            default: CO_NO();
        }
    }
    *n_scatter = 0;
    std::vector<const tts_tensor *> outs;
    for (int i = 0; i < n_nodes; ++i)
        if ((nodes[i]->flags & TTS_FLAG_OUTPUT) || i == n_nodes - 1) outs.push_back(nodes[i]);
    std::vector<std::array<int64_t, 3>> sc;
    for (const tts_tensor * o : outs) {
        if (owned_mem(o) || is_view(o->op)) continue;
        if (!inter(o) || !contiguous(o) || (tbytes(o) & 3) || !equal_all(o)) CO_NO();
        for (int k = 0; k < N; ++k) {
            const tts_tensor * m = cm.member(bc, o, k);
            if (!m || !m->data || !contiguous(m)) CO_NO();
            sc.push_back({(int64_t)(uintptr_t)bc.reloc(o->data, k), (int64_t)(uintptr_t)m->data, (int64_t)tbytes(o)});
        }
    }
    if (!sc.empty()) {
        *scatter = alloc(3 * sc.size());
        for (size_t e = 0; e < sc.size(); ++e)
            for (int c = 0; c < 3; ++c) tab[*scatter + 3 * (int64_t)e + c] = sc[e][c];
        *n_scatter = (int)sc.size();
    }
    for (size_t a = 0; a < pl.items.size(); ++a)
        for (int t = 0; t < EMBED_MAX_TERMS; ++t)
            if (ioffs[a][t] >= 0) bc.tabs[a].ioff[t] = (const int64_t *)(intptr_t)(ioffs[a][t] + 1);
    return true;
}

static void co_readback(tts_hip_backend * be, const std::vector<int64_t> & sc, int n_sc) {
    BatchCtx & bc = *be->bat;
    const int N = bc.N;
    if ((int)bc.mbe.size() != N) return;
    std::vector<size_t> need(N, 0), off(N, 0);
    for (int e = 0; e < n_sc; ++e) need[e % N] += ((size_t)sc[3 * e + 2] + 255) & ~(size_t)255;
    for (int k = 0; k < N; ++k) {
        tts_hip_backend * m = bc.mbe[k];
        m->rb_clear();
        if (need[k] <= m->rb_cap) continue;
        if (m->rb_host) {
            TTS_HIP_CHECK(hipStreamSynchronize(be->stream));
            TTS_HIP_CHECK(hipHostFree(m->rb_host));
            m->rb_host = nullptr;
            m->rb_cap = 0;
        }
        if (hipHostMalloc((void **)&m->rb_host, need[k], hipHostMallocDefault) != hipSuccess) {
            (void)hipGetLastError();
            m->rb_host = nullptr;
            continue;
        }
        m->rb_cap = need[k];
    }
    for (int e = 0; e < n_sc; ++e) {
        const int k = e % N;
        tts_hip_backend * m = bc.mbe[k];
        if (!m->rb_host) continue;
        const size_t bytes = (size_t)sc[3 * e + 2];
        TTS_HIP_CHECK(hipMemcpyAsync(m->rb_host + off[k], (const void *)(uintptr_t)sc[3 * e], bytes, hipMemcpyDeviceToHost, be->stream));
        std::lock_guard<std::mutex> l(m->rb_mu);
        m->rb.push_back({(const char *)(uintptr_t)sc[3 * e + 1], bytes, off[k]});
        m->rb_any.store(true, std::memory_order_release);
        off[k] += (bytes + 255) & ~(size_t)255;
    }
}

__global__ void k_co_scatter(const int64_t * __restrict__ tab, int n) {
    const int e = blockIdx.y;
    if (e >= n) return;
    const uint32_t * src = (const uint32_t *)(uintptr_t)tab[3 * e];
    uint32_t * dst = (uint32_t *)(uintptr_t)tab[3 * e + 1];
    const int64_t w = tab[3 * e + 2] / 4;
    for (int64_t i = (int64_t)blockIdx.x * blockDim.x + threadIdx.x; i < w; i += (int64_t)gridDim.x * blockDim.x) dst[i] = src[i];
}

static bool capture_worthy(tts_hip_backend * be, tts_tensor * const * nodes, int n_nodes) {
    if (!be->use_graphs || be->profile_gemv) return false;
    for (int i = 0; i < n_nodes; ++i) {
        const tts_tensor * t = nodes[i];
        if (t->op == TTS_OP_MUL_MAT && t->src[1] && t->src[1]->ne[1] > 64) return false;
    }
    return true;
}

namespace tts {
static void plan_setup(Planner & pl, const tts_hip_backend * be);
}
static void conv_pack_prepare(tts_hip_backend * be, tts_tensor * const * nodes, int n_nodes) {
    if (!be->conv_pack || !(be->fusion & TTS_FUSE_CONV)) return;
    bool any = false;
    for (int i = 0; i < n_nodes && !any; ++i) any = nodes[i]->op == TTS_OP_IM2COL;
    if (!any) return;
    Planner pl;
    plan_setup(pl, be);
    pl.build(nodes, n_nodes);
    for (const Item & it : pl.items) {
        ConvPackKey k;
        if (it.kind == Item::CONV && conv1d_pack_key(be, it.conv, &k)) (void)conv_pack_get(be, k);
    }
}

static int capture_into(tts_hip_backend * be, tts_tensor * const * nodes, int n_nodes, hipGraphExec_t & ex) {
    conv_pack_prepare(be, nodes, n_nodes);
    hipStream_t run = be->stream;
    be->stream = be->cap_stream;
    be->capturing = true;
    const auto t0 = std::chrono::steady_clock::now();
    TTS_HIP_CHECK(hipStreamBeginCapture(be->stream, hipStreamCaptureModeThreadLocal));
    const int st = graph_compute_launches(be, nodes, n_nodes);
    hipGraph_t graph = nullptr;
    TTS_HIP_CHECK(hipStreamEndCapture(be->stream, &graph));
    be->stream = run;
    be->capturing = false;
    const auto t1 = std::chrono::steady_clock::now();
    be->cap_launch_ns += std::chrono::duration_cast<std::chrono::nanoseconds>(t1 - t0).count();
    if (st != 0) {
        if (graph) hipGraphDestroy(graph);
        return st;
    }
    bool ok = false;
    if (ex) {
        hipGraphNode_t err_node = nullptr;
        hipGraphExecUpdateResult res;
        ok = hipGraphExecUpdate(ex, graph, &err_node, &res) == hipSuccess && res == hipGraphExecUpdateSuccess;
        if (ok) be->graph_updates++;
        else {
            (void)hipGetLastError();
            TTS_HIP_CHECK(hipGraphExecDestroy(ex));
            ex = nullptr;
        }
    }
    if (!ok) {
        TTS_HIP_CHECK(hipGraphInstantiate(&ex, graph, nullptr, nullptr, 0));
        be->graph_instantiations++;
    }
    TTS_HIP_CHECK(hipGraphDestroy(graph));
    be->cap_update_ns += std::chrono::duration_cast<std::chrono::nanoseconds>(std::chrono::steady_clock::now() - t1).count();
    return 0;
}

extern "C" int tts_hip_graph_compute(tts_hip_backend_t be, tts_tensor * const * nodes, int n_nodes) {
    if (!be) return TTS_STATUS_BAD_ARG;
    hipSetDevice(be->device);
    be->rb_clear();
    const int cs = coalesce_submit(be, nodes, n_nodes);
    if (cs != kCoalesceNotTaken) return cs;
    uint64_t sig = 0x9E3779B97F4A7C15ull ^ (uint64_t)n_nodes;
    for (int i = 0; i < n_nodes; ++i) sig = (sig ^ (uint64_t)nodes[i]->op) * 0x100000001B3ull;
    if (n_nodes > 0)
        for (int d = 0; d < 4; ++d)
            sig = (sig ^ (uint64_t)nodes[0]->ne[d] ^ ((uint64_t)nodes[n_nodes - 1]->ne[d] << 32)) * 0x100000001B3ull;
    sig |= 1;
    int slot = -1;
    for (int k = 0; k < tts_hip_backend::N_GSIG; ++k)
        if (be->gsig[k] == sig) slot = k;
    if (slot < 0) {
        slot = be->gsig_next;
        be->gsig_next = (be->gsig_next + 1) % tts_hip_backend::N_GSIG;
        be->gsig[slot] = sig;
        if (be->gsig_exec[slot]) {
            TTS_HIP_CHECK(hipGraphExecDestroy(be->gsig_exec[slot]));
            be->gsig_exec[slot] = nullptr;
        }
        return graph_compute_launches(be, nodes, n_nodes);
    }
    if (!capture_worthy(be, nodes, n_nodes)) return graph_compute_launches(be, nodes, n_nodes);
    const int st = capture_into(be, nodes, n_nodes, be->gsig_exec[slot]);
    if (st != 0) return st;
    TTS_HIP_CHECK(hipGraphLaunch(be->gsig_exec[slot], be->stream));
    return 0;
}

extern "C" int tts_hip_graph_prepare(tts_hip_backend_t be, tts_tensor * const * nodes, int n_nodes, int slot) {
    if (!be || slot < 0 || slot > 1) return TTS_STATUS_BAD_ARG;
    hipSetDevice(be->device);
    be->rb_clear();
    if (be->plan_ev_pending[slot]) {
        const auto t0 = std::chrono::steady_clock::now();
        TTS_HIP_CHECK(hipEventSynchronize(be->plan_ev[slot]));
        be->plan_wait_ns += std::chrono::duration_cast<std::chrono::nanoseconds>(std::chrono::steady_clock::now() - t0).count();
        be->plan_ev_pending[slot] = false;
    }
    be->plan_nodes[slot] = nodes;
    be->plan_n[slot] = n_nodes;
    be->plan_eager[slot] = !capture_worthy(be, nodes, n_nodes);
    if (be->plan_eager[slot]) return 0;
    const int st = capture_into(be, nodes, n_nodes, be->pexec[slot]);
    be->plan_prepared[slot] = st == 0;
    return st;
}

extern "C" int tts_hip_graph_launch(tts_hip_backend_t be, int slot) {
    if (!be || slot < 0 || slot > 1) return TTS_STATUS_BAD_ARG;
    hipSetDevice(be->device);
    be->rb_clear();
    if (be->plan_eager[slot]) {
        const int st = graph_compute_launches(be, be->plan_nodes[slot], be->plan_n[slot]);
        if (st != 0) return st;
    } else {
        if (!be->pexec[slot]) return TTS_STATUS_BAD_ARG;
        TTS_HIP_CHECK(hipGraphLaunch(be->pexec[slot], be->stream));
        be->plan_prepared[slot] = false;
    }
    TTS_HIP_CHECK(hipEventRecord(be->plan_ev[slot], be->stream));
    be->plan_ev_pending[slot] = true;
    return 0;
}

extern "C" int tts_hip_plan_stats(tts_tensor * const * nodes, int n_nodes, int mask, int32_t * counts) {
    Planner pl;
    pl.mask = mask;
    pl.vec_cap = 1u << 18;
    static float lstm_stand_in alignas(256);
    pl.lstm_buf = &lstm_stand_in;
    pl.lstm_cap = (size_t)4 << 20;
    static float conv_stand_in alignas(256);
    pl.conv_stage = &conv_stand_in;
    pl.conv_stage_cap = (size_t)8 << 20;
    static char hoist_stand_in alignas(256);
    pl.hoist_buf = &hoist_stand_in;
    pl.hoist_cap = (size_t)8 << 20;
    if (mask) pl.build(nodes, n_nodes);
    else pl.act.assign(n_nodes, 0);
    for (int k = 0; k < 16; ++k) counts[k] = 0;
    for (const Item & it : pl.items) {
        counts[(int)it.kind]++;
        if (it.xattn >= 0) counts[14]++;
        if (it.kind == Item::GEMV) {
            counts[12] += (int32_t)it.mms.size();
            if ((int32_t)it.mms.size() > counts[13]) counts[13] = (int32_t)it.mms.size();
        }
    }
    static const bool dump = getenv("TTS_PLAN_DUMP") != nullptr;
    if (dump)
        for (int i = 0; i < n_nodes; ++i)
            if (pl.act[i] > 0) {
                const Item & it = pl.items[pl.act[i] - 1];
                fprintf(stderr, "item %d kind %d", i, (int)it.kind);
                if (it.kind == Item::GEMV)
                    fprintf(stderr, " mms %d K %lld N %lld M %lld epi %d ln %d", (int)it.mms.size(), (long long)it.mms[0]->src[0]->ne[0],
                            (long long)it.mms[0]->src[0]->ne[1], (long long)(nel(it.mms[0]->src[1]) / it.mms[0]->src[1]->ne[0]), it.epi, (int)it.ln);
                if (it.kind == Item::COPY) fprintf(stderr, " bytes %zu", it.cp_bytes);
                fprintf(stderr, "\n");
            }
    for (int i = 0; i < n_nodes; ++i)
        if (pl.act[i] == 0 && !is_view(nodes[i]->op)) {
            counts[15]++;
            if (dump)
                fprintf(stderr, "unfused %d op %d [%lld %lld %lld %lld] %s <- %s\n", i, (int)nodes[i]->op, (long long)nodes[i]->ne[0],
                        (long long)nodes[i]->ne[1], (long long)nodes[i]->ne[2], (long long)nodes[i]->ne[3], nodes[i]->name,
                        nodes[i]->src[0] ? nodes[i]->src[0]->name : "");
        }
    return (int)pl.items.size();
}

namespace tts {
static void plan_setup(Planner & pl, const tts_hip_backend * be) {
    pl.mask = be->fusion;
    pl.q80pro = be->gemv_q80_pro != 0;
    pl.lstm_buf = be->lstm_buf;
    pl.lstm_cap = be->lstm_floats;
    pl.vec_cap = be->vec_scratch ? (1u << 18) : 0;
    pl.conv_stage = be->conv_stage;
    pl.conv_stage_cap = be->conv_stage_floats;
    pl.hoist_buf = (char *)be->hoist;
    pl.hoist_cap = be->hoist_size;
}

int graph_compute_launches(tts_hip_backend_t be, tts_tensor * const * nodes, int n_nodes) {
    be->graph_epoch++;
    be->aq.src = nullptr;
    if (be->profile_gemv) launch_profile_spin(be, 4000.0);
    const auto tp0 = std::chrono::steady_clock::now();
    Planner pl;
    plan_setup(pl, be);
    if (be->fusion) pl.build(nodes, n_nodes);
    else pl.act.assign(n_nodes, 0);
    be->cap_plan_ns += std::chrono::duration_cast<std::chrono::nanoseconds>(std::chrono::steady_clock::now() - tp0).count();
    CoMap cm;
    int64_t sc_off = -1;
    int n_sc = 0;
    std::vector<int64_t> sc_host;
    if (be->bat) {
        const auto tq0 = std::chrono::steady_clock::now();
        struct Acc {
            tts_hip_backend * be;
            std::chrono::steady_clock::time_point t0;
            ~Acc() { be->co_prep_ns += std::chrono::duration_cast<std::chrono::nanoseconds>(std::chrono::steady_clock::now() - t0).count(); }
        } acc{be, tq0};
        BatchCtx & bc = *be->bat;
        cm.build(nodes, n_nodes);
        bc.comap = &cm;
        std::vector<std::tuple<const void *, const void *, size_t>> shared;
        std::vector<int64_t> tab;
        std::vector<std::array<int64_t, 5>> offs;
        if (!co_prepare(be, pl, nodes, n_nodes, shared, tab, offs, &sc_off, &n_sc)) {
            bc.comap = nullptr;
            return TTS_STATUS_UNSUPPORTED;
        }
        if (!coalesce_check_shared(be, shared)) {
            bc.differs = true;
            bc.comap = nullptr;
            return TTS_STATUS_UNSUPPORTED;
        }
        if (n_sc > 0) sc_host.assign(tab.begin() + sc_off, tab.begin() + sc_off + 3 * (int64_t)n_sc);
        if (!tab.empty()) {
            const size_t bytes = tab.size() * sizeof(int64_t);
            if (bytes > be->co_tab_bytes) {
                TTS_HIP_CHECK(hipStreamSynchronize(be->stream));
                if (be->co_tab) TTS_HIP_CHECK(hipFree(be->co_tab));
                be->co_tab_bytes = std::max(bytes * 2, (size_t)64 << 10);
                TTS_HIP_CHECK(hipMalloc((void **)&be->co_tab, be->co_tab_bytes));
            }
            if (tts_hip_tensor_set_async(be, be->co_tab, tab.data(), bytes) != 0) {
                bc.comap = nullptr;
                return TTS_STATUS_UNSUPPORTED;
            }
        }
        for (size_t a = 0; a < pl.items.size(); ++a) {
            ItemTab & tb = bc.tabs[a];
            const auto & of = offs[a];
            tb.yoff = of[0] >= 0 ? be->co_tab + of[0] : nullptr;
            tb.koff = of[1] >= 0 ? be->co_tab + of[1] : nullptr;
            tb.voff = of[2] >= 0 ? be->co_tab + of[2] : nullptr;
            tb.pseq = of[3] >= 0 ? (const int *)(be->co_tab + of[3]) : nullptr;
            tb.moff = of[4] >= 0 ? be->co_tab + of[4] : nullptr;
            for (auto & io : tb.ioff)
                if (io) io = be->co_tab + ((intptr_t)io - 1);
        }
    }
    std::vector<int> pf_items;
    if (be->fusion && be->kv_prefetch_minp > 0) {
        for (int i = 0; i < n_nodes; ++i) {
            const int a = pl.act[i];
            if (a > 0 && pl.items[a - 1].kind == Item::ATTN && pl.items[a - 1].k->ne[1] >= be->kv_prefetch_minp) pf_items.push_back(a - 1);
        }
    }
    size_t pf_next = 0;
    int pf_pending = -1;
    auto pf_fork = [&]() {
        if (pf_next >= pf_items.size()) return;
        const Item & t = pl.items[pf_items[pf_next]];
        TTS_HIP_CHECK(hipEventRecord(be->pf_fork, be->stream));
        TTS_HIP_CHECK(hipStreamWaitEvent(be->pf_stream, be->pf_fork, 0));
        launch_kv_prefetch(be, be->pf_stream, make_td(t.k), 1, be->kv_prefetch_blocks);
        launch_kv_prefetch(be, be->pf_stream, make_td(t.v), 0, be->kv_prefetch_blocks);
        TTS_HIP_CHECK(hipEventRecord(be->pf_join, be->pf_stream));
        pf_pending = pf_items[pf_next];
    };
    pf_fork();
    for (int i = 0; i < n_nodes; ++i) {
        tts_tensor * n = nodes[i];
        const int a = be->fusion ? pl.act[i] : 0;
        if (a < 0) continue;
        if (a == 0 && is_view(n->op)) continue;
        const bool is_pf = a > 0 && pf_pending == a - 1;
        if (is_pf) {
            TTS_HIP_CHECK(hipStreamWaitEvent(be->stream, be->pf_join, 0));
            pf_pending = -1;
        }
        const int st = a > 0 ? run_item(be, pl.items[a - 1], pl.items) : run_node(be, n);
        if (is_pf) {
            ++pf_next;
            pf_fork();
        }
        if (st != 0) {
            fprintf(stderr, "tts_hip_graph_compute: node %d (%s, %s) failed: %d\n", i, n->name, tts_op_name(n->op), st);
            if (pf_pending >= 0) (void)hipStreamWaitEvent(be->stream, be->pf_join, 0);
            return st;
        }
        if (be->bat) be->aq.src = nullptr;
        if (be->aq.src) {
            const char * s0 = (const char *)be->aq.src;
            const char * s1 = s0 + (size_t)be->aq.K * (size_t)be->aq.M * 4;
            bool keep = false;
            if (a > 0) {
                const Item & it = pl.items[a - 1];
                if (it.kind == Item::GEMV) {
                    keep = true;
                    for (size_t k = 0; k < it.tgt.size(); ++k) {
                        const char * y0 = (const char *)it.tgt[k].y;
                        const tts_tensor * mm = it.mms[k];
                        const int64_t Mm = mm->ne[1] * mm->ne[2] * mm->ne[3];
                        const char * y1 = y0 + 4 * (size_t)((Mm - 1) * it.tgt[k].ycs + (mm->ne[0] - 1) * it.tgt[k].yrs + 1);
                        if (y0 < s1 && s0 < y1) keep = false;
                    }
                }
            } else if (n->op == TTS_OP_MUL_MAT) {
                const char * y0 = (const char *)n->data;
                keep = !(y0 < s1 && s0 < y0 + tbytes(n));
            }
            if (!keep) be->aq.src = nullptr;
        }
    }
    if (pf_pending >= 0) TTS_HIP_CHECK(hipStreamWaitEvent(be->stream, be->pf_join, 0));
    if (be->bat) {
        if (n_sc > 0) {
            hipLaunchKernelGGL(k_co_scatter, dim3(4, (unsigned)n_sc), dim3(256), 0, be->stream, (const int64_t *)be->co_tab + sc_off, n_sc);
            TTS_HIP_CHECK(hipGetLastError());
            co_readback(be, sc_host, n_sc);
        }
        be->bat->comap = nullptr;
    }
    return 0;
}
}

extern "C" int tts_hip_gemv(tts_hip_backend_t be, int type, const void * w, const float * x, float * y, int64_t K, int64_t N,
                            int64_t M) {
    return tts_hip_gemv_ex(be, type, w, x, y, K, N, M, 0);
}

extern "C" int tts_hip_gemv_ex(tts_hip_backend_t be, int type, const void * w, const float * x, float * y, int64_t K, int64_t N,
                               int64_t M, int32_t wflags) {
    return tts_hip_gemv_res(be, type, w, x, y, nullptr, K, N, M, wflags);
}

extern "C" int tts_hip_gemv_res(tts_hip_backend_t be, int type, const void * w, const float * x, float * y, const float * res,
                                int64_t K, int64_t N, int64_t M, int32_t wflags) {
    if (!be) return TTS_STATUS_BAD_ARG;
    if ((wflags & TTS_FLAG_TILED) && (type != TTS_TYPE_Q4_K || N % 4)) return TTS_STATUS_BAD_ARG;
    if (tts::wtype_q8k_act(type) && K % 256) return TTS_STATUS_BAD_ARG;
    if (type == TTS_TYPE_Q6_K && ((uintptr_t)w & 1)) return TTS_STATUS_BAD_ARG;
    if (tts::wtype_q80_act(type) && K % 32) return TTS_STATUS_BAD_ARG;
    if (type != TTS_TYPE_Q4_K && type != TTS_TYPE_Q6_K && type != TTS_TYPE_Q8_0 && type != TTS_TYPE_Q5_0 && type != TTS_TYPE_Q4_0 && type != TTS_TYPE_F16 && type != TTS_TYPE_F32) return TTS_STATUS_UNSUPPORTED;
    if ((type == TTS_TYPE_F32 || type == TTS_TYPE_F16) && K % 4) return TTS_STATUS_BAD_ARG;
    hipSetDevice(be->device);
    GemvJob j;
    j.wtype = type;
    j.K = K;
    j.N = N;
    j.M = M;
    j.w_row_bytes = (int64_t)tts_row_size(type, K);
    j.W[0] = (const uint8_t *)w;
    j.Y[0] = y;
    j.ycs[0] = N;
    j.yrs[0] = 1;
    j.x = x;
    j.xcs = K;
    if (res) {
        j.epi = EPI_ADD;
        j.res = res;
        j.rcs = N;
    }
    const bool q80pro = tts::wtype_q80_act(type) && K % QK_K == 0 && M <= 8 && be->gemv_q80_pro;
    if (tts::wtype_q8k_act(type) || q80pro) {
        j.pro = PRO_QUANT;
        j.tiled = (wflags & TTS_FLAG_TILED) ? 1 : 0;
        if ((uintptr_t)x & 15) {
            if ((size_t)(4 * K * M) > be->scratch_size) return TTS_STATUS_ALLOC_FAILED;
            launch_copy_cols(be, (float *)be->scratch, x, K, K, M);
            be->aq.src = nullptr;
            j.x = (const float *)be->scratch;
        }
    } else if (type != TTS_TYPE_F32) {
        if (act_quant_bytes(type, K, M) > be->scratch_size) return TTS_STATUS_ALLOC_FAILED;
        launch_quantize_act(be, type, x, K, K, M, j.aq);
    } else {
        j.aq.vtype = TTS_TYPE_F32;
    }
    be->aq.src = nullptr;
    if (type == TTS_TYPE_Q6_K && !tts::gemv_q6k_ok(j)) return TTS_STATUS_UNSUPPORTED;
    launch_gemv_job(be, j);
    return 0;
}
```

### tts.cpp_amd/csrc/hip_internal.h

```cpp
#pragma once

#include <hip/hip_fp16.h>
#include <hip/hip_runtime.h>

#include <cstdio>
#include <cstdlib>
#include <atomic>
#include <deque>
#include <mutex>
#include <unordered_map>
#include <tuple>
#include <vector>

#include "common.h"

#define TTS_HIP_CHECK(expr)                                                                          \
    do {                                                                                             \
        hipError_t err_ = (expr);                                                                    \
        if (err_ != hipSuccess) {                                                                    \
            fprintf(stderr, "%s:%d: HIP error %s: %s\n", __FILE__, __LINE__, #expr, hipGetErrorString(err_)); \
            abort();                                                                                 \
        }                                                                                            \
    } while (0)

// ... 253 lines not shown
    const int64_t * voff = nullptr;
    const int64_t * moff = nullptr;
    const int * pseq = nullptr;
};

constexpr int EMBED_MAX_TERMS = 16;
struct BatchCls {
    const char * b0 = nullptr;
    size_t size = 0;
    char * win = nullptr;
    int64_t stride = 0;
};
struct ItemTab {
    const int64_t * yoff = nullptr;
    int32_t yoff_mats = 0;
    const int64_t *koff = nullptr, *voff = nullptr;
    const int64_t * moff = nullptr;
    const int * pseq = nullptr;
    int pmax = 0;
    const int64_t * ioff[EMBED_MAX_TERMS] = {};
};
struct BatchCtx {
    int N = 0;
    uint64_t key = 0;
    std::vector<BatchCls> cls;
    std::vector<tts_tensor * const *> mnodes;
    std::vector<tts_hip_backend *> mbe;
    int n_nodes = 0;
    bool checked = false;
    int canon = 0;
    bool ragged = false;
    bool differs = false;
    std::vector<ItemTab> tabs;
    void * comap = nullptr;
    const BatchCls * find(const void * p) const {
        const char * c = (const char *)p;
        size_t lo = 0, hi = cls.size();
        while (lo < hi) {
            const size_t m = (lo + hi) / 2;
            if (cls[m].b0 <= c) lo = m + 1;
            else hi = m;
        }
        if (lo == 0) return nullptr;
        const BatchCls & b = cls[lo - 1];
        return c < b.b0 + b.size ? &b : nullptr;
    }
    template <typename T>
    T * win(T * p) const {
        const BatchCls * b = p ? find(p) : nullptr;
        return b ? (T *)(b->win + ((const char *)p - b->b0)) : p;
    }
    int64_t stride(const void * p) const {
        const BatchCls * b = p ? find(p) : nullptr;
        return b ? b->stride : 0;
    }
    template <typename T>
    T * reloc(T * p, int k) const {
        const BatchCls * b = p ? find(p) : nullptr;
        return b ? (T *)(b->win + k * b->stride + ((const char *)p - b->b0)) : p;
    }
};

}

struct tts_hip_backend {
    int device = 0;
    hipStream_t stream = nullptr;
    char name[64] = {0};
    char * scratch = nullptr;
    size_t scratch_size = 0;
    float * shadow = nullptr;
    size_t shadow_size = 0;
    void * hoist = nullptr;
    size_t hoist_size = 0;
    float * attn_buf = nullptr;
    size_t attn_floats = 0;
    int attn_split_minp = 128;
    int attn_ks = 2;
    int attn_pv_mp = 1;
    int attn_one = 1;
    int attn_pv8 = 0;
    int attn_pv_uv16 = 0;
    int attn_fused_minp = 0;
    unsigned long long * argmax_keys = nullptr;
    unsigned * argmax_counts = nullptr;
    int64_t q4k_tile_bytes = 4 << 20;
    int gemv_dbg = 0;
    int gemv_unique = 1;
    int gemm_q8 = 1;
    int64_t cus = 256;
    int cu_total = 256;
    int bgemm_f32 = 1;
    int gemv_f32_wide = 1;
    int gemm_kr_nw = 4;
    int64_t gemv_ks_tiles = 256;
    int gemv_mf_prequant = 1;
    int gemv_kr = 1;
    int gemv_kr_loop = 1;
    int gemv_kr_tail = 1;
    int gemv_q80_pro = 1;
    int gemv_q80_slab = 1;
    int gemv_q80_rw = 0;
    int gemm_q8_staged = 2;
    int gemv_q50_slab = 1;
    int gemv_q50_rw = 0;
    int gemm_q5 = 1;
    int gemm_q5_staged = 2;
    int gemv_q40_slab = 1;
    int gemv_q40_rw = 0;
    int gemm_q4_0 = 1;
    int gemm_q4_0_staged = 2;
    int64_t gemv_kr_ink = 0;
    int gemm_kr_walk = 0;
    int gemm_pf = 64;
    int gemm_pf_nw = 4;
    int gemm_kr_cp = 0;
    int gemm_kr_xcd = 0;
    int gemm_kr_ct2 = 0;
    int64_t gemm_kr_ink = 0;
    int gemv_nw_min = 0;
    int gemv_mf_rsplit = 1;
    int64_t q4k_dual_bytes = 1 << 20;
    void * sample_cand = nullptr;
    size_t sample_cand_size = 0;
    int kv_prefetch_minp = 0;
    int kv_prefetch_blocks = 128;
    hipStream_t pf_stream = nullptr;
    hipEvent_t pf_fork = nullptr, pf_join = nullptr;
    uint8_t * pin = nullptr;
    size_t pin_size = 0, pin_head = 0;
    struct PinRec {
        size_t off, size;
        hipEvent_t ev;
    };
    std::deque<PinRec> pin_pending;
    std::vector<hipEvent_t> pin_events;
    std::mutex pin_mu;
    hipEvent_t plan_ev[2] = {nullptr, nullptr};
    bool plan_ev_pending[2] = {false, false};
    float * lstm_buf = nullptr;
    float * conv_stage = nullptr;
    size_t conv_stage_floats = 0;
    float * vec_scratch = nullptr;
    size_t lstm_floats = 0;
    tts::ActQuant aq;
    int64_t graph_epoch = 0;
    uint16_t * gelu_table = nullptr;
    bool convt_lds = true;
    double * conv_part = nullptr;
    size_t conv_part_doubles = 0;
    int conv_vfma = 1;
    int conv_tile96 = 1;
    int conv_pack = 1;
    bool capturing = false;
    int conv_split = 1;
    int fusion = 0x3FFF;
    bool profile_gemv = false;
    double gemv_ms[TTS_TYPE_COUNT] = {0};
    int64_t gemv_launches[TTS_TYPE_COUNT] = {0};
    double gemv_bytes[TTS_TYPE_COUNT] = {0};
    std::vector<std::pair<hipEvent_t, hipEvent_t>> ev_pending;
    std::vector<double> ev_bytes;
    std::vector<int> ev_type;
    std::vector<hipEvent_t> ev_free;
    char * repack_tmp = nullptr;
    size_t repack_tmp_size = 0;
    std::vector<char *> repack_retired;
    float * attn_stage = nullptr;
    size_t attn_stage_size = 0;
    bool use_graphs = false;
    static constexpr int N_GSIG = 4;
    uint64_t gsig[N_GSIG] = {};
    hipGraphExec_t gsig_exec[N_GSIG] = {};
    int gsig_next = 0;
    bool conv_f32acc = false;
    int conv_acc_mode = 0;
    hipStream_t cap_stream = nullptr;
    int64_t graph_updates = 0, graph_instantiations = 0;
    int64_t lstm_chains = 0, lstm_steps = 0;
    int64_t plan_wait_ns = 0;
    int64_t cap_plan_ns = 0, cap_launch_ns = 0, cap_update_ns = 0;
    hipGraphExec_t pexec[2] = {nullptr, nullptr};
    tts_tensor * const * plan_nodes[2] = {nullptr, nullptr};
    int plan_n[2] = {0, 0};
    bool plan_eager[2] = {true, true};
    bool plan_prepared[2] = {false, false};
    tts::BatchCtx * bat = nullptr;
    hipEvent_t co_ev = nullptr;
    int64_t * co_tab = nullptr;
    size_t co_tab_bytes = 0;
    int64_t co_prep_ns = 0;
    bool co_member = true;
    struct RbEnt {
        const char * dev;
        size_t bytes, off;
    };
    char * rb_host = nullptr;
    size_t rb_cap = 0;
    std::vector<RbEnt> rb;
    std::mutex rb_mu;
    std::atomic<bool> rb_any{false};
    void rb_clear() {
        if (!rb_any.load(std::memory_order_acquire)) return;
        std::lock_guard<std::mutex> l(rb_mu);
        rb.clear();
        rb_any.store(false, std::memory_order_release);
    }
};

namespace tts {

const uint8_t * tiled_copy_find(const void * weight);

void profile_pair(tts_hip_backend * be, hipEvent_t & e0, hipEvent_t & e1);
void profile_push(tts_hip_backend * be, hipEvent_t e0, hipEvent_t e1, double bytes, int type);

void launch_quantize_act(tts_hip_backend * be, int wtype, const float * x, int64_t xcs, int64_t K, int64_t M, ActQuant & aq);
void launch_gemv_job(tts_hip_backend * be, const GemvJob & job);
bool gemv_q6k_ok(const GemvJob & j);
bool launch_bgemm_f32(tts_hip_backend * be, const tts_tensor * node);
bool gemm_f32_ok(const GemvJob & j);
void launch_gemm_f32(tts_hip_backend * be, const GemvJob & j);
void launch_copy_cols(tts_hip_backend * be, float * dst, const float * src, int64_t K, int64_t scs, int64_t M);
void launch_profile_spin(tts_hip_backend * be, double us);
void launch_im2col(tts_hip_backend * be, const tts_tensor * node);
constexpr int kLstmQMaxK = 512;
struct LstmStepArgs {
    const float * pre[4];
    const void * w[4];
    int64_t w_rs[4];
    const float * bias[4];
    const float * hprev;
    const float * cprev;
    float * h;
    float * c;
    int Hd, K, wtype;
};
void launch_lstm_step(tts_hip_backend * be, const LstmStepArgs & a, const LstmStepArgs * b = nullptr);
void launch_repeat_interleave1(tts_hip_backend * be, const tts_tensor * dst, const tts_tensor * a, int r);
void launch_copy_bytes(tts_hip_backend * be, void * dst, const void * src, size_t bytes);
void launch_cpy_multi(tts_hip_backend * be, const tts_tensor * src, const tts_tensor * const * dsts, int nd);
void launch_rope_multi(tts_hip_backend * be, const tts_tensor * rope, const tts_tensor * src, const tts_tensor * const * dsts, int nd);
void launch_greedy_step(tts_hip_backend * be, const float * logits, int B, int NH, int V, int step, int bos, int eos, int32_t * eos_seen,
                        int32_t * hist, int32_t * next);
int launch_sample_step(tts_hip_backend * be, const float * logits, int B, int NH, int V, const tts_sampling * c, int64_t call,
                       int32_t * rep_state, int step, int bos, int eos, int32_t * eos_seen, int32_t * hist, int32_t * next);
struct BatchCtx;
void launch_embed_sum(tts_hip_backend * be, const tts_tensor * out, const tts_tensor * const * gr, int n, const BatchCtx * bat = nullptr,
                      const ItemTab * tab = nullptr);
void launch_snake(tts_hip_backend * be, const tts_tensor * dst, const tts_tensor * x, const tts_tensor * alpha, const tts_tensor * recip,
                  const tts_tensor * one = nullptr, const tts_tensor * mask = nullptr);
void launch_lstm_finish(tts_hip_backend * be, const tts_tensor * final_out, const float * hist, int64_t Hd, int64_t T);
bool audio_op_supported(const tts_tensor * n);
int launch_audio_op(tts_hip_backend * be, const tts_tensor * n);
void launch_conv_transpose_1d(tts_hip_backend * be, const tts_tensor * node);
constexpr int CONV1D_MAX_R = 128;
struct Conv1dArgs {
    TD x;
    const void * w = nullptr;
    int w16 = 0;
    int64_t wk = 0, wic = 0, woc = 0;
    float * y = nullptr;
    int64_t ycs = 0;
    const float * bias = nullptr;
    int64_t bcs = 0;
    const float * res = nullptr;
    int64_t rcs = 0;
    int64_t L = 0, IC = 0, OL = 0, OC = 0;
    int K = 1, s = 1, p = 0, d = 1;
    int icc = 0, xw = 0, rs = 0;
    float * copy_dst = nullptr;
    uint32_t x_bytes = 0, w_bytes = 0;
    double * part = nullptr;
    int ic_per_split = 0;
    int w_stable = 0;
    const float * wimg = nullptr;
};
constexpr int CONV1D_XN = 16, CONV1D_WN = 16;
inline int conv1d_icc(int64_t IC, int K, int xw) {
    int best = 0;
    double best_eff = -1.0;
    const int top = (int)(IC < 64 ? IC : 64);
    for (int c = 1; c <= top; ++c) {
        const int r = c * K, rp = (r + 31) & ~31;
        if (rp > 64 || c * xw > 256 * CONV1D_XN) break;
        const double eff = (double)r / rp + 1e-4 * c;
        if (eff > best_eff) best_eff = eff, best = c;
    }
    return best;
}
bool conv1d_fused_ok(int64_t IC, int K, int s, int d, size_t * lds);
__host__ __device__ inline int64_t conv1d_pack_index(int nchunk, int oct, int rp, int ct, int chunk, int row, int r) {
    const int lane = (r & 3) * 16 + (row & 15);
    return (int64_t)(ct * nchunk + chunk) * oct * rp + ((((row >> 4) * (rp >> 4) + (r >> 4)) * 64 + lane) * 4 + ((r >> 2) & 3));
}
struct ConvPackKey {
    const tts_hip_backend * be;
    const void * w;
    int w16, K, oct, icc, rp;
    int64_t IC, OC, wk, wic, woc;
    bool operator<(const ConvPackKey & o) const {
        return std::tie(be, w, w16, K, oct, icc, rp, IC, OC, wk, wic, woc) <
               std::tie(o.be, o.w, o.w16, o.K, o.oct, o.icc, o.rp, o.IC, o.OC, o.wk, o.wic, o.woc);
    }
    int nchunk() const { return (int)((IC + icc - 1) / icc); }
    int ntile() const { return (int)((OC + oct - 1) / oct); }
    size_t floats() const { return (size_t)ntile() * nchunk() * oct * rp; }
};
void launch_conv1d_pack(hipStream_t stream, const ConvPackKey & k, float * img);
const float * conv_pack_get(tts_hip_backend * be, const ConvPackKey & k);
void conv_pack_written(tts_hip_backend * be, const void * p, size_t n);
void conv_pack_freed(const tts_hip_backend * be, const void * p, size_t n);
bool conv1d_pack_key(const tts_hip_backend * be, const Conv1dArgs & a, ConvPackKey * k);
struct AdainArgs {
    const float * x = nullptr;
    int64_t xcs = 0;
    float * y = nullptr;
    int64_t ycs = 0;
    const float *gamma = nullptr, *beta = nullptr, *alpha = nullptr, *recip = nullptr;
    const float * one = nullptr;
    int stage = 0;
    const float *gw = nullptr, *gb = nullptr, *bw = nullptr, *bb = nullptr, *style = nullptr;
    int64_t S = 0;
    int64_t gcs = 1, bcs = 1, acs = 1, rcs = 1;
    int64_t T = 0, C = 0;
    float eps = 0.f;
};
bool adain_supported(int64_t T);
void launch_adain_snake(tts_hip_backend * be, const AdainArgs & a);
void launch_conv1d_fused(tts_hip_backend * be, Conv1dArgs a);
bool launch_gemm_f16(tts_hip_backend * be, const tts_tensor * node);
size_t act_quant_bytes(int wtype, int64_t K, int64_t M);
void act_quant_layout(int wtype, char * base, int64_t K, int64_t M, ActQuant & aq);

void launch_repack_q4_K(tts_hip_backend * be, const void * src, void * dst, int64_t nblocks, int inverse);

int launch_op(tts_hip_backend * be, const tts_tensor * node);
void launch_copy_stream(tts_hip_backend * be, void * dst, const void * src, int64_t n16);

int graph_compute_launches(tts_hip_backend * be, tts_tensor * const * nodes, int n_nodes);
constexpr int kCoalesceNotTaken = 1 << 20;
int coalesce_submit(tts_hip_backend * be, tts_tensor * const * nodes, int n_nodes);
bool buffer_lookup(const void * p, const char ** base, size_t * size);
bool coalesce_check_shared(tts_hip_backend * ex, const std::vector<std::tuple<const void *, const void *, size_t>> & pairs);
void coalesce_backend_gone(const tts_hip_backend * be);
void coalesce_written(const void * p, size_t size);
bool coalesce_enabled();
bool co_debug();

}
```

### tts.cpp_amd/csrc/k_conv.hip

```cpp
#include "hip_internal.h"

namespace tts {

template <bool F16OUT>
__global__ void k_im2col(TD dst, TD x, int K, int s0, int p0, int d0, int64_t n) {
    const int64_t KW = dst.ne[0];
    const int64_t OL = dst.ne[1];
    const int64_t L = x.ne[0];
    for (int64_t e = (int64_t)blockIdx.x * blockDim.x + threadIdx.x; e < n; e += (int64_t)gridDim.x * blockDim.x) {
        const int64_t kk = e % KW;
        const int64_t ol = (e / KW) % OL;
        const int64_t nn = e / (KW * OL);
        const int64_t ic = kk / K, k = kk % K;
        const int64_t il = ol * s0 + k * d0 - p0;
        float v = 0.f;
        if (il >= 0 && il < L) v = *(const float *)(x.data + il * x.nb[0] + ic * x.nb[1] + nn * x.nb[2]);
        char * o = dst.data + kk * dst.nb[0] + ol * dst.nb[1] + nn * dst.nb[2];
        if (F16OUT) *(__half *)o = __float2half_rn(v);
        else *(float *)o = v;
    }
}

void launch_im2col(tts_hip_backend * be, const tts_tensor * node) {
    const tts_tensor * a = node->src[0];
// ... 273 lines not shown

template <bool W16, bool BIAS, bool RES, bool H32 = false, int MT = 2>
__global__ __launch_bounds__(256) __attribute__((amdgpu_waves_per_eu(MT == 2 ? 1 : 2))) void k_conv1d_f64(Conv1dArgs a) {
    constexpr int OCT = 32 * MT, WN = CONV1D_WN * MT / 2;
    extern __shared__ float sm[];
    __shared__ int xoff[CONV1D_MAX_R];
    __shared__ int wofs[CONV1D_MAX_R];
    const int lane = threadIdx.x & 63, wave = threadIdx.x >> 6;
    const int c16 = lane & 15, kq = lane >> 4;
    const int64_t ol0 = (int64_t)blockIdx.x * 64;
    const int oc0 = blockIdx.y * OCT;
    const int K = a.K, s = a.s, icc = a.icc, xw = a.xw, rs = a.rs;
    const int R = icc * K, Rp = (R + 31) & ~31;
    float * xs = sm;
    float * ws = sm + icc * xw + 1;
    const int zslot = icc * xw;
    for (int r = threadIdx.x; r < Rp; r += 256) {
        const int ic = r / K, k = r - ic * K;
        xoff[r] = r < R ? ic * xw + k * a.d : zslot;
        wofs[r] = r < R ? (int)(k * a.wk + ic * a.wic) : -1;
    }
    if (threadIdx.x == 0) xs[zslot] = 0.f;
    __syncthreads();
    const int wr0 = (wave >> 1) * 16 * MT, wc0 = (wave & 1) * 32;
    const bool wave_live = oc0 + wr0 < a.OC && ol0 + wc0 < a.OL;
    f64x4_t acc[MT][2] = {};
    const int64_t base = ol0 * s - a.p;
    const int EX = icc * xw, EW = OCT * Rp;
    constexpr int esz = W16 ? 2 : 4;
    const uint32_t OOB = 0x80000000u;
    const auto xr = __builtin_amdgcn_make_buffer_rsrc(a.x.data, 0, a.x_bytes, 0x00020000);
    const auto wr = __builtin_amdgcn_make_buffer_rsrc(const_cast<void *>(a.w), 0, a.w_bytes, 0x00020000);
    const int rsh = Rp == 64 ? 6 : 5;
    uint32_t xrel[CONV1D_XN], wrel[WN];
#pragma unroll
    for (int u = 0; u < CONV1D_XN; ++u) {
        const int e = (int)threadIdx.x + 256 * u;
        const int ic = e / xw, q = e - ic * xw;
        const int64_t pos = base + q;
        const bool ok = e < EX && pos >= 0 && pos < a.L;
        xrel[u] = ok ? (uint32_t)(pos * a.x.nb[0] + (int64_t)ic * a.x.nb[1]) : OOB;
    }
#pragma unroll
    for (int u = 0; u < WN; ++u) {
        const int e = (int)threadIdx.x + 256 * u;
        const int oc = e >> rsh, r = e & (Rp - 1);
        const int wo = e < EW ? wofs[r] : -1;
        const bool ok = wo >= 0 && oc0 + oc < a.OC;
        wrel[u] = ok ? (uint32_t)(((int64_t)(oc0 + oc) * a.woc + wo) * esz) : OOB;
    }
    float xv[CONV1D_XN], wv[WN];
    auto fetch = [&](int ic0) {
        const int nic = min(icc, (int)(a.IC - ic0));
        const uint32_t xc = (uint32_t)((int64_t)ic0 * a.x.nb[1]);
        const uint32_t wc = (uint32_t)((int64_t)ic0 * a.wic * esz);
#pragma unroll
        for (int u = 0; u < CONV1D_XN; ++u) {
            const uint32_t off = (xrel[u] == OOB || (int)threadIdx.x + 256 * u >= nic * xw) ? OOB : xrel[u] + xc;
            xv[u] = __builtin_bit_cast(float, __builtin_amdgcn_raw_buffer_load_b32(xr, off, 0, 0));
        }
#pragma unroll
        for (int u = 0; u < WN; ++u) {
            const uint32_t off = (wrel[u] == OOB || (((int)threadIdx.x + 256 * u) & (Rp - 1)) >= nic * K) ? OOB : wrel[u] + wc;
            if (W16) wv[u] = __half2float(__builtin_bit_cast(__half, __builtin_amdgcn_raw_buffer_load_b16(wr, off, 0, 0)));
            else wv[u] = __builtin_bit_cast(float, __builtin_amdgcn_raw_buffer_load_b32(wr, off, 0, 0));
        }
    };
    const int ic_lo = a.part ? (int)blockIdx.z * a.ic_per_split : 0;
    const int ic_hi = a.part ? (int)min((int64_t)(ic_lo + a.ic_per_split), a.IC) : (int)a.IC;
    fetch(ic_lo);
    for (int ic0 = ic_lo; ic0 < ic_hi; ic0 += icc) {
#pragma unroll
        for (int u = 0; u < CONV1D_XN; ++u)
            if ((int)threadIdx.x + 256 * u < EX) xs[(int)threadIdx.x + 256 * u] = __half2float(__float2half_rn(xv[u]));
#pragma unroll
        for (int u = 0; u < WN; ++u) {
            const int e = (int)threadIdx.x + 256 * u;
            if (e < EW) ws[e + (e >> rsh)] = W16 ? wv[u] : __half2float(__float2half_rn(wv[u]));
        }
        __syncthreads();
        if (ic0 + icc < ic_hi) fetch(ic0 + icc);
        if (!wave_live) {
            __syncthreads();
            continue;
        }
        if (H32) {
            for (int r0 = 0; r0 < Rp; r0 += 32) {
                int xo[8];
#pragma unroll
                for (int u = 0; u < 8; ++u) xo[u] = xoff[r0 + 8 * kq + u];
                h16x8_t A[MT], B[2];
#pragma unroll
                for (int u = 0; u < 8; ++u) {
                    const bool z = xo[u] == zslot;
#pragma unroll
                    for (int t = 0; t < MT; ++t) A[t][u] = (_Float16)ws[(wr0 + 16 * t + c16) * rs + r0 + 8 * kq + u];
#pragma unroll
                    for (int t = 0; t < 2; ++t) B[t][u] = (_Float16)xs[z ? zslot : xo[u] + (wc0 + 16 * t + c16) * s];
                }
#pragma unroll
                for (int ti = 0; ti < MT; ++ti)
#pragma unroll
                    for (int tj = 0; tj < 2; ++tj) {
                        const f32x4 pr = __builtin_amdgcn_mfma_f32_16x16x32_f16(A[ti], B[tj], f32x4{0.f, 0.f, 0.f, 0.f}, 0, 0, 0);
#pragma unroll
                        for (int e = 0; e < 4; ++e) acc[ti][tj][e] += (double)pr[e];
                    }
            }
        } else
        for (int r0 = 0; r0 < Rp; r0 += 32) {
            int xo[8];
#pragma unroll
            for (int u = 0; u < 8; ++u) xo[u] = xoff[r0 + 4 * u + kq];
            float af[8][MT], bf[8][2];
#pragma unroll
            for (int u = 0; u < 8; ++u) {
                const int r = r0 + 4 * u + kq;
                const bool z = xo[u] == zslot;
#pragma unroll
                for (int t = 0; t < MT; ++t) af[u][t] = ws[(wr0 + 16 * t + c16) * rs + r];
#pragma unroll
                for (int t = 0; t < 2; ++t) bf[u][t] = xs[z ? zslot : xo[u] + (wc0 + 16 * t + c16) * s];
            }
#pragma unroll
            for (int u = 0; u < 8; ++u)
#pragma unroll
                for (int ti = 0; ti < MT; ++ti)
#pragma unroll
                    for (int tj = 0; tj < 2; ++tj)
                        acc[ti][tj] = __builtin_amdgcn_mfma_f64_16x16x4f64((double)af[u][ti], (double)bf[u][tj], acc[ti][tj], 0, 0, 0);
        }
        __syncthreads();
    }
    conv1d_store<BIAS, RES, H32, MT>(a, acc, ol0, oc0, wr0, wc0, c16, kq);
}

__global__ __launch_bounds__(256) void k_conv1d_pack(ConvPackKey k, float * __restrict__ img, int nchunk, int64_t n) {
    const int64_t e = (int64_t)blockIdx.x * 256 + threadIdx.x;
    if (e >= n) return;
    const int per = k.oct * k.rp;
    const int slice = (int)(e / per), w = (int)(e - (int64_t)slice * per);
    const int ct = slice / nchunk, chunk = slice - ct * nchunk;
    const int row = w / k.rp, r = w - row * k.rp;
    const int icl = r / k.K, tap = r - icl * k.K;
    const int64_t oc = (int64_t)ct * k.oct + row, ic = (int64_t)chunk * k.icc + icl;
    float v = 0.f;
    if (icl < k.icc && ic < k.IC && oc < k.OC) {
        const int64_t o = oc * k.woc + (int64_t)tap * k.wk + ic * k.wic;
        v = k.w16 ? __half2float(((const __half *)k.w)[o]) : __half2float(__float2half_rn(((const float *)k.w)[o]));
    }
    img[conv1d_pack_index(nchunk, k.oct, k.rp, ct, chunk, row, r)] = v;
}

void launch_conv1d_pack(hipStream_t stream, const ConvPackKey & k, float * img) {
    const int64_t n = (int64_t)k.floats();
    hipLaunchKernelGGL(k_conv1d_pack, dim3((unsigned)((n + 255) / 256)), dim3(256), 0, stream, k, img, k.nchunk(), n);
    TTS_HIP_CHECK(hipGetLastError());
}

template <bool BIAS, bool RES, int MT>
__global__ __launch_bounds__(256) __attribute__((amdgpu_waves_per_eu(MT == 2 ? 1 : 2))) void k_conv1d_f64p(Conv1dArgs a) {
    constexpr int OCT = 32 * MT, WQ = 2 * MT;
    extern __shared__ float sm[];
    __shared__ int xoff[CONV1D_MAX_R];
    const int tid = threadIdx.x, lane = tid & 63, wave = tid >> 6;
    const int c16 = lane & 15, kq = lane >> 4;
    const int64_t ol0 = (int64_t)blockIdx.x * 64;
    const int oc0 = blockIdx.y * OCT;
    const int K = a.K, s = a.s, icc = a.icc, xw = a.xw;
    const int R = icc * K, Rp = (R + 31) & ~31;
    f32x4_t * ws4 = (f32x4_t *)sm;
    float * xs = sm + OCT * Rp;
    const int zslot = icc * xw;
    for (int r = tid; r < Rp; r += 256) {
        const int ic = r / K, k = r - ic * K;
        xoff[r] = r < R ? ic * xw + k * a.d : zslot;
    }
    if (tid == 0) xs[zslot] = 0.f;
    __syncthreads();
    const int wr0 = (wave >> 1) * 16 * MT, wc0 = (wave & 1) * 32;
    const bool wave_live = oc0 + wr0 < a.OC && ol0 + wc0 < a.OL;
    f64x4_t acc[MT][2] = {};
    const int64_t base = ol0 * s - a.p;
    const int EX = icc * xw;
    const int nx = (EX + 255) >> 8;
    const int nw = Rp == 64 ? WQ : WQ / 2;
    const int G = Rp >> 4;
    const uint32_t OOB = 0x80000000u;
    const auto xr = __builtin_amdgcn_make_buffer_rsrc(a.x.data, 0, a.x_bytes, 0x00020000);
    uint32_t xrel[CONV1D_XN];
#pragma unroll
    for (int u = 0; u < CONV1D_XN; ++u) {
        const int e = tid + 256 * u;
        const int ic = e / xw, q = e - ic * xw;
        const int64_t pos = base + q;
        const bool ok = e < EX && pos >= 0 && pos < a.L;
        xrel[u] = ok ? (uint32_t)(pos * a.x.nb[0] + (int64_t)ic * a.x.nb[1]) : OOB;
    }
    const int nchunk = (int)((a.IC + icc - 1) / icc);
    const int slice4 = OCT * Rp / 4;
    const f32x4_t * wp = (const f32x4_t *)a.wimg + (int64_t)blockIdx.y * nchunk * slice4 + tid;
    float xv[CONV1D_XN];
    f32x4_t wv[WQ];
    auto fetch = [&](int ic0) {
        const int nic = min(icc, (int)(a.IC - ic0));
        const uint32_t xc = (uint32_t)((int64_t)ic0 * a.x.nb[1]);
#pragma unroll
        for (int u = 0; u < CONV1D_XN; ++u)
            if (u < nx) {
                const uint32_t off = (xrel[u] == OOB || tid + 256 * u >= nic * xw) ? OOB : xrel[u] + xc;
                xv[u] = __builtin_bit_cast(float, __builtin_amdgcn_raw_buffer_load_b32(xr, off, 0, 0));
            }
#pragma unroll
        for (int u = 0; u < WQ; ++u)
            if (u < nw) wv[u] = wp[256 * u];
        wp += slice4;
    };
    fetch(0);
    for (int ic0 = 0; ic0 < a.IC; ic0 += icc) {
#pragma unroll
        for (int u = 0; u < CONV1D_XN; ++u)
            if (u < nx && tid + 256 * u < EX) xs[tid + 256 * u] = __half2float(__float2half_rn(xv[u]));
#pragma unroll
        for (int u = 0; u < WQ; ++u)
            if (u < nw) ws4[tid + 256 * u] = wv[u];
        __syncthreads();
        if (ic0 + icc < a.IC) fetch(ic0 + icc);
        if (!wave_live) {
            __syncthreads();
            continue;
        }
        for (int r0 = 0; r0 < Rp; r0 += 32) {
            int xo[8];
#pragma unroll
            for (int u = 0; u < 8; ++u) xo[u] = xoff[r0 + 4 * u + kq];
            float af[8][MT], bf[8][2];
#pragma unroll
            for (int h = 0; h < 2; ++h)
#pragma unroll
                for (int t = 0; t < MT; ++t) {
                    const f32x4_t v = ws4[(((wr0 >> 4) + t) * G + (r0 >> 4) + h) * 64 + lane];
#pragma unroll
                    for (int j = 0; j < 4; ++j) af[4 * h + j][t] = v[j];
                }
#pragma unroll
            for (int u = 0; u < 8; ++u) {
                const bool z = xo[u] == zslot;
#pragma unroll
                for (int t = 0; t < 2; ++t) bf[u][t] = xs[z ? zslot : xo[u] + (wc0 + 16 * t + c16) * s];
            }
#pragma unroll
            for (int u = 0; u < 8; ++u)
#pragma unroll
                for (int ti = 0; ti < MT; ++ti)
#pragma unroll
                    for (int tj = 0; tj < 2; ++tj)
                        acc[ti][tj] = __builtin_amdgcn_mfma_f64_16x16x4f64((double)af[u][ti], (double)bf[u][tj], acc[ti][tj], 0, 0, 0);
        }
        __syncthreads();
    }
    conv1d_store<BIAS, RES, false, MT>(a, acc, ol0, oc0, wr0, wc0, c16, kq);
}

constexpr int CONV1DV_NP = 4;
template <bool W16, bool BIAS, bool RES>
__global__ __launch_bounds__(256) void k_conv1d_f64v(Conv1dArgs a) {
    constexpr int NP = CONV1DV_NP;
    extern __shared__ double smd[];
    const int K = a.K, d = a.d, icc = a.icc, xw = a.xw, R = icc * K;
    double * xs = smd;
    double * ws = smd + icc * xw;
    const int tid = threadIdx.x;
    const int64_t ol0 = (int64_t)blockIdx.x * (256 * NP);
    const int oc = blockIdx.y;
    const int64_t base = ol0 - a.p;
    const int EX = icc * xw;
    constexpr int esz = W16 ? 2 : 4;
    const uint32_t OOB = 0x80000000u;
    const auto xr = __builtin_amdgcn_make_buffer_rsrc(a.x.data, 0, a.x_bytes, 0x00020000);
    const auto wr = __builtin_amdgcn_make_buffer_rsrc(const_cast<void *>(a.w), 0, a.w_bytes, 0x00020000);
    uint32_t xrel[CONV1D_XN];
#pragma unroll
    for (int u = 0; u < CONV1D_XN; ++u) {
        const int e = tid + 256 * u;
        const int ic = e / xw, q = e - ic * xw;
        const int64_t pos = base + q;
        const bool ok = e < EX && pos >= 0 && pos < a.L;
        xrel[u] = ok ? (uint32_t)(pos * a.x.nb[0] + (int64_t)ic * a.x.nb[1]) : OOB;
    }
    const int wicl = tid < R ? tid / K : -1;
    const uint32_t wrel = tid < R ? (uint32_t)(((int64_t)oc * a.woc + (int64_t)(tid - wicl * K) * a.wk + (int64_t)wicl * a.wic) * esz) : OOB;
    float xv[CONV1D_XN], wv;
    auto fetch = [&](int ic0) {
        const int nic = min(icc, (int)(a.IC - ic0));
        const uint32_t xc = (uint32_t)((int64_t)ic0 * a.x.nb[1]);
        const uint32_t wc = (uint32_t)((int64_t)ic0 * a.wic * esz);
#pragma unroll
        for (int u = 0; u < CONV1D_XN; ++u) {
            const uint32_t off = (xrel[u] == OOB || tid + 256 * u >= nic * xw) ? OOB : xrel[u] + xc;
            xv[u] = __builtin_bit_cast(float, __builtin_amdgcn_raw_buffer_load_b32(xr, off, 0, 0));
        }
        const uint32_t off = (wrel == OOB || wicl >= nic) ? OOB : wrel + wc;
        if (W16) wv = __half2float(__builtin_bit_cast(__half, __builtin_amdgcn_raw_buffer_load_b16(wr, off, 0, 0)));
        else wv = __builtin_bit_cast(float, __builtin_amdgcn_raw_buffer_load_b32(wr, off, 0, 0));
    };
    double acc[NP];
#pragma unroll
    for (int j = 0; j < NP; ++j) acc[j] = 0.0;
    fetch(0);
    for (int ic0 = 0; ic0 < a.IC; ic0 += icc) {
        const int nic = min(icc, (int)(a.IC - ic0));
#pragma unroll
        for (int u = 0; u < CONV1D_XN; ++u)
            if (tid + 256 * u < EX) xs[tid + 256 * u] = (double)__half2float(__float2half_rn(xv[u]));
        if (wicl >= 0) ws[tid] = (double)(W16 ? wv : __half2float(__float2half_rn(wv)));
        __syncthreads();
        if (ic0 + icc < a.IC) fetch(ic0 + icc);
        const double * xp = xs + tid;
        for (int icl = 0; icl < nic; ++icl, xp += xw)
            for (int k = 0; k < K; ++k) {
                const double w = ws[icl * K + k];
#pragma unroll
                for (int j = 0; j < NP; ++j) acc[j] = __builtin_fma(xp[k * d + 256 * j], w, acc[j]);
            }
        __syncthreads();
    }
    const float bias = BIAS ? a.bias[(int64_t)oc * a.bcs] : 0.f;
#pragma unroll
    for (int j = 0; j < NP; ++j) {
        const int64_t ol = ol0 + tid + 256 * j;
        if (ol >= a.OL) continue;
        const float res = RES ? a.res[ol + (int64_t)oc * a.rcs] : 0.f;
        a.y[ol + (int64_t)oc * a.ycs] = conv1d_epilogue<BIAS, RES>(acc[j], bias, res);
    }
}

static bool conv1d_vfma_geometry(const Conv1dArgs & a, int * xw, int * icc, size_t * lds) {
    if (a.s != 1 || a.K < 1 || a.K > 64 || a.OC > 65535) return false;
    const int64_t w = 256 * CONV1DV_NP + (int64_t)(a.K - 1) * a.d;
    if (w > 256 * CONV1D_XN) return false;
    int c = (int)std::min<int64_t>(std::min<int64_t>(a.IC, 256 * CONV1D_XN / w), 256 / a.K);
    if (c < 1) return false;
    *xw = (int)w, *icc = c, *lds = ((size_t)c * (size_t)w + (size_t)c * a.K) * sizeof(double);
    return true;
}

bool conv1d_fused_ok(int64_t IC, int K, int s, int d, size_t * lds) {
    if (K < 1 || K > 64 || s < 1 || d < 1 || IC < 1) return false;
    const int xw = 63 * s + (K - 1) * d + 1;
    const int icc = conv1d_icc(IC, K, xw);
    if (icc < 1) return false;
    const int rs = ((icc * K + 31) & ~31) + 1;
    const size_t bytes = ((size_t)icc * xw + 1 + 64 * (size_t)rs) * 4;
    if (lds) *lds = bytes;
    return bytes <= 64 * 1024;
}

bool conv1d_pack_key(const tts_hip_backend * be, const Conv1dArgs & a0, ConvPackKey * k) {
    if (!be->conv_pack || !a0.w_stable || be->conv_acc_mode == 2) return false;
    Conv1dArgs a = a0;
    a.xw = 63 * a.s + (a.K - 1) * a.d + 1;
    a.icc = conv1d_icc(a.IC, a.K, a.xw);
    if (a.icc < 1) return false;
    const int64_t tiles = ((a.OL + 63) / 64) * ((a.OC + 63) / 64), nchunk = (a.IC + a.icc - 1) / a.icc;
    if (split_count(be, tiles, nchunk, 2, a.OL * a.OC) > 1) return false;
    int vxw = 0, vicc = 0;
    size_t vlds = 0;
    if (be->conv_vfma && (be->conv_vfma == 2 || a.OC < 8) && conv1d_vfma_geometry(a, &vxw, &vicc, &vlds)) return false;
    k->be = be, k->w = a.w, k->w16 = a.w16, k->K = a.K;
    k->oct = be->conv_tile96 && a.OC % 96 == 0 ? 96 : 64;
    k->icc = a.icc, k->rp = (a.icc * a.K + 31) & ~31;
    k->IC = a.IC, k->OC = a.OC, k->wk = a.wk, k->wic = a.wic, k->woc = a.woc;
    return true;
}

void launch_conv1d_fused(tts_hip_backend * be, Conv1dArgs a) {
    ConvPackKey pk;
    a.wimg = conv1d_pack_key(be, a, &pk) ? conv_pack_get(be, pk) : nullptr;
    a.xw = 63 * a.s + (a.K - 1) * a.d + 1;
    a.icc = conv1d_icc(a.IC, a.K, a.xw);
    a.rs = ((a.icc * a.K + 31) & ~31) + 1;
    size_t lds = 0;
    if (!conv1d_fused_ok(a.IC, a.K, a.s, a.d, &lds)) {
        fprintf(stderr, "tts_hip: conv1d_fused shape unsupported\n");
        abort();
    }
    dim3 grid((unsigned)((a.OL + 63) / 64), (unsigned)((a.OC + 63) / 64));
    Conv1dArgs e = a;
    const int64_t nchunk = (a.IC + a.icc - 1) / a.icc;
    const int nz = be->conv_acc_mode == 2 ? 1 : split_count(be, (int64_t)grid.x * grid.y, nchunk, 2, a.OL * a.OC);
    if (nz > 1) {
        a.ic_per_split = (int)(((nchunk + nz - 1) / nz) * a.icc);
        grid.z = (unsigned)((a.IC + a.ic_per_split - 1) / a.ic_per_split);
        a.part = be->conv_part;
        a.bias = nullptr;
        a.res = nullptr;
    }
    const int sel = (a.w16 ? 4 : 0) | (a.bias ? 2 : 0) | (a.res ? 1 : 0);
#define TTS_CONV1D_SEL(KERNEL, GRID, LDS, ...)                                                                           \
    switch (sel) {                                                                                                        \
        case 0: hipLaunchKernelGGL((KERNEL<false, false, false __VA_ARGS__>), GRID, dim3(256), LDS, be->stream, a); break; \
        case 1: hipLaunchKernelGGL((KERNEL<false, false, true __VA_ARGS__>), GRID, dim3(256), LDS, be->stream, a); break;  \
        case 2: hipLaunchKernelGGL((KERNEL<false, true, false __VA_ARGS__>), GRID, dim3(256), LDS, be->stream, a); break;  \
        case 3: hipLaunchKernelGGL((KERNEL<false, true, true __VA_ARGS__>), GRID, dim3(256), LDS, be->stream, a); break;   \
        case 4: hipLaunchKernelGGL((KERNEL<true, false, false __VA_ARGS__>), GRID, dim3(256), LDS, be->stream, a); break;  \
        case 5: hipLaunchKernelGGL((KERNEL<true, false, true __VA_ARGS__>), GRID, dim3(256), LDS, be->stream, a); break;   \
        case 6: hipLaunchKernelGGL((KERNEL<true, true, false __VA_ARGS__>), GRID, dim3(256), LDS, be->stream, a); break;   \
        default: hipLaunchKernelGGL((KERNEL<true, true, true __VA_ARGS__>), GRID, dim3(256), LDS, be->stream, a); break;   \
    }
#define TTS_COMMA ,
    int vxw = 0, vicc = 0;
    size_t vlds = 0;
    if (nz == 1 && be->conv_acc_mode != 2 && be->conv_vfma && (be->conv_vfma == 2 || a.OC < 8) && conv1d_vfma_geometry(a, &vxw, &vicc, &vlds)) {
        a.xw = vxw, a.icc = vicc;
        const dim3 vgrid((unsigned)((a.OL + 256 * CONV1DV_NP - 1) / (256 * CONV1DV_NP)), (unsigned)a.OC);
        TTS_CONV1D_SEL(k_conv1d_f64v, vgrid, vlds)
    } else if (a.wimg) {
        const size_t plds = ((size_t)pk.oct * pk.rp + (size_t)a.icc * a.xw + 1) * 4;
        grid.y = (unsigned)pk.ntile();
        const int psel = (pk.oct == 96 ? 4 : 0) | (a.bias ? 2 : 0) | (a.res ? 1 : 0);
        switch (psel) {
            case 0: hipLaunchKernelGGL((k_conv1d_f64p<false, false, 2>), grid, dim3(256), plds, be->stream, a); break;
            case 1: hipLaunchKernelGGL((k_conv1d_f64p<false, true, 2>), grid, dim3(256), plds, be->stream, a); break;
            case 2: hipLaunchKernelGGL((k_conv1d_f64p<true, false, 2>), grid, dim3(256), plds, be->stream, a); break;
            case 3: hipLaunchKernelGGL((k_conv1d_f64p<true, true, 2>), grid, dim3(256), plds, be->stream, a); break;
            case 4: hipLaunchKernelGGL((k_conv1d_f64p<false, false, 3>), grid, dim3(256), plds, be->stream, a); break;
            case 5: hipLaunchKernelGGL((k_conv1d_f64p<false, true, 3>), grid, dim3(256), plds, be->stream, a); break;
            case 6: hipLaunchKernelGGL((k_conv1d_f64p<true, false, 3>), grid, dim3(256), plds, be->stream, a); break;
            default: hipLaunchKernelGGL((k_conv1d_f64p<true, true, 3>), grid, dim3(256), plds, be->stream, a); break;
        }
    } else if (nz == 1 && be->conv_acc_mode != 2 && be->conv_tile96 && a.OC % 96 == 0) {
        grid.y = (unsigned)(a.OC / 96);
        lds += 32 * (size_t)a.rs * 4;
        TTS_CONV1D_SEL(k_conv1d_f64, grid, lds, TTS_COMMA false TTS_COMMA 3)
    } else if (be->conv_acc_mode == 2) {
        TTS_CONV1D_SEL(k_conv1d_f64, grid, lds, TTS_COMMA true)
    } else {
        TTS_CONV1D_SEL(k_conv1d_f64, grid, lds)
    }
#undef TTS_COMMA
#undef TTS_CONV1D_SEL
    TTS_HIP_CHECK(hipGetLastError());
    if (a.part) launch_split_reduce(be, (int)grid.z, a.OL, a.OC, e.y, e.ycs, e.bias, e.bcs, e.res, e.rcs);
    if (a.copy_dst)
        launch_copy_bytes(be, a.copy_dst, a.y, (size_t)a.OL * (size_t)a.OC * 4);
}

__global__ __launch_bounds__(256) void k_conv_transpose_1d(TD y, TD x, TD w, int s, int p, int d, int g) {
    const int64_t OL = y.ne[0];
    const int64_t o = (int64_t)blockIdx.x * blockDim.x + threadIdx.x;
    const int oc = blockIdx.y;
    if (o >= OL) return;
    const int K = (int)w.ne[0], OCg = (int)w.ne[1];
    const int64_t L = x.ne[0];
    const int IC = (int)x.ne[1], ICg = IC / g;
    const int grp = oc / OCg, ocl = oc % OCg;
    double acc = 0.0;
    const int64_t num0 = o + p;
    for (int k = (d == 1 ? (int)(num0 % s) : 0); k < K; k += (d == 1 ? s : 1)) {
        const int64_t num = num0 - (int64_t)k * d;
        if (num < 0) break;
        if (num % s) continue;
        const int64_t i = num / s;
        if (i >= L) continue;
        const char * xp = x.data + i * x.nb[0] + (int64_t)grp * ICg * x.nb[1];
        const char * wp = w.data + (int64_t)k * w.nb[0] + (int64_t)ocl * w.nb[1] + (int64_t)grp * ICg * w.nb[2];
        if (w.type == TTS_TYPE_F16) {
            for (int icl = 0; icl < ICg; ++icl)
                acc = __fma_rn((double)__half2float(__float2half_rn(*(const float *)(xp + icl * x.nb[1]))),
                               (double)__half2float(*(const __half *)(wp + icl * w.nb[2])), acc);
        } else {
            for (int icl = 0; icl < ICg; ++icl)
                acc = __fma_rn((double)*(const float *)(xp + icl * x.nb[1]), (double)*(const float *)(wp + icl * w.nb[2]), acc);
        }
    }
    *(float *)(y.data + o * y.nb[0] + (int64_t)oc * y.nb[1]) = (float)acc;
}

__global__ __launch_bounds__(64) void k_conv_transpose_1d_mfma(TD y, TD x, TD w, int s, int p) {
    const int lane = threadIdx.x, r16 = lane & 15, kq = lane >> 4;
    const int rr = blockIdx.z;
    const int64_t q0 = (int64_t)blockIdx.x * 16;
    const int oc0 = blockIdx.y * 16;
    const int K = (int)w.ne[0], OC = (int)w.ne[1], IC = (int)w.ne[2];
    const int64_t L = x.ne[0], OL = y.ne[0];
    const int J = (K - rr + s - 1) / s;
    const int oca = min(oc0 + r16, OC - 1);
    const int64_t qb = q0 + r16;
    f64x4_t acc = {};
    for (int j = 0; j < J; ++j) {
        const int k = rr + s * j;
        const int64_t i = qb - j;
        const bool iin = i >= 0 && i < L;
        const char * wp = w.data + (int64_t)k * w.nb[0] + (int64_t)oca * w.nb[1];
        const char * xp = x.data + (iin ? i : 0) * x.nb[0];
        for (int ic0 = 0; ic0 < IC; ic0 += 16) {
            double av[4], bv[4];
#pragma unroll
            for (int u = 0; u < 4; ++u) {
                const int ic = ic0 + 4 * u + kq;
                const int icc = min(ic, IC - 1);
                const bool w16 = w.type == TTS_TYPE_F16;
                const float wa = w16 ? __half2float(*(const __half *)(wp + (int64_t)icc * w.nb[2])) : *(const float *)(wp + (int64_t)icc * w.nb[2]);
                float xb = *(const float *)(xp + (int64_t)icc * x.nb[1]);
                if (w16) xb = __half2float(__float2half_rn(xb));
                av[u] = ic < IC ? (double)wa : 0.0;
                bv[u] = (ic < IC && iin) ? (double)xb : 0.0;
            }
#pragma unroll
            for (int u = 0; u < 4; ++u) acc = __builtin_amdgcn_mfma_f64_16x16x4f64(av[u], bv[u], acc, 0, 0, 0);
        }
    }
    const int64_t o = qb * s + rr - p;
    if (o < 0 || o >= OL) return;
#pragma unroll
    for (int e = 0; e < 4; ++e) {
        const int oc = oc0 + kq + 4 * e;
        if (oc < OC) *(float *)(y.data + o * y.nb[0] + (int64_t)oc * y.nb[1]) = (float)acc[e];
    }
}

template <int S, bool W16>
__global__ __launch_bounds__(256) void k_convt_f64_lds(TD y, TD x, TD w, int p, double * __restrict__ part = nullptr, int icps = 0) {
    constexpr int JM = 2, K = 2 * S;
    constexpr int QT = 64, OCT = 32, ICC = 16, XW = QT + JM - 1;
    constexpr int NX = ICC * XW, NW4 = ICC * K * OCT / 4;
    constexpr int XR = (NX + 255) / 256, WR = (NW4 + 255) / 256;
    constexpr int XWP = 80;
    constexpr int WK = S == 8 ? 34 : S == 4 ? 36 : OCT + 1;
    constexpr int WIC0 = K * WK, WIC = WIC0 + ((16 - WIC0 % 32) + 32) % 32;
    __shared__ float xs[ICC][XWP];
    __shared__ float ws[ICC * WIC];
    const int lane = threadIdx.x & 63, qw = threadIdx.x >> 6;
    const int c16 = lane & 15, kq = lane >> 4;
    const int OC = (int)w.ne[1], IC = (int)w.ne[2];
    const int64_t L = x.ne[0], OL = y.ne[0];
    const int64_t q0 = (int64_t)blockIdx.x * QT;
    const int oc0 = blockIdx.y * OCT;
    f64x4_t acc[S][2];
#pragma unroll
    for (int r = 0; r < S; ++r) acc[r][0] = acc[r][1] = (f64x4_t){0.0, 0.0, 0.0, 0.0};
    float xr[XR];
    float4 wr[WR];
    auto fetch = [&](int ic0) {
#pragma unroll
        for (int u = 0; u < XR; ++u) {
            const int t = threadIdx.x + 256 * u;
            const int ic = t / XW, qq = t - ic * XW;
            const int64_t pos = q0 - (JM - 1) + qq;
            const bool ok = t < NX && pos >= 0 && pos < L && ic0 + ic < IC;
            xr[u] = ok ? *(const float *)(x.data + pos * x.nb[0] + (int64_t)(ic0 + ic) * x.nb[1]) : 0.f;
            if (W16) xr[u] = __half2float(__float2half_rn(xr[u]));
        }
#pragma unroll
        for (int u = 0; u < WR; ++u) {
            const int t = threadIdx.x + 256 * u;
            const int ic = t / (K * OCT / 4), rem = (t - ic * (K * OCT / 4)) * 4;
            const int oc = rem / K;
            const bool ok = t < NW4 && oc0 + oc < OC && ic0 + ic < IC;
            const char * src = w.data + (int64_t)(oc0 + oc) * w.nb[1] + (int64_t)(ic0 + ic) * w.nb[2] + (rem - oc * K) * (W16 ? 2 : 4);
            if (W16) {
                const uint2 h = ok ? *(const uint2 *)src : make_uint2(0u, 0u);
                wr[u] = make_float4(__half2float(__ushort_as_half((unsigned short)(h.x & 0xFFFF))), __half2float(__ushort_as_half((unsigned short)(h.x >> 16))),
                                    __half2float(__ushort_as_half((unsigned short)(h.y & 0xFFFF))), __half2float(__ushort_as_half((unsigned short)(h.y >> 16))));
            } else {
                wr[u] = ok ? *(const float4 *)src : make_float4(0.f, 0.f, 0.f, 0.f);
            }
        }
    };
    auto stage = [&]() {
#pragma unroll
        for (int u = 0; u < XR; ++u) {
            const int t = threadIdx.x + 256 * u;
            if (t < NX) xs[t / XW][t % XW] = xr[u];
        }
#pragma unroll
        for (int u = 0; u < WR; ++u) {
            const int t = threadIdx.x + 256 * u;
            if (t >= NW4) continue;
            const int ic = t / (K * OCT / 4), rem = (t - ic * (K * OCT / 4)) * 4;
            const int oc = rem / K, k = rem - oc * K;
            float * o = ws + ic * WIC + k * WK + oc;
            o[0] = wr[u].x, o[WK] = wr[u].y, o[2 * WK] = wr[u].z, o[3 * WK] = wr[u].w;
        }
    };
    const int ic_lo = part ? (int)blockIdx.z * icps : 0;
    const int ic_hi = part ? min(IC, ic_lo + icps) : IC;
    fetch(ic_lo);
    for (int ic0 = ic_lo; ic0 < ic_hi; ic0 += ICC) {
        stage();
        __syncthreads();
        if (ic0 + ICC < ic_hi) fetch(ic0 + ICC);
#pragma unroll
        for (int kk = 0; kk < 4; ++kk) {
            const int icl = 4 * kk + kq;
            float bx[JM], aw[JM][S][2];
#pragma unroll
            for (int j = 0; j < JM; ++j) {
                bx[j] = xs[icl][qw * 16 + c16 + (JM - 1) - j];
#pragma unroll
                for (int r = 0; r < S; ++r)
#pragma unroll
                    for (int h = 0; h < 2; ++h) aw[j][r][h] = ws[icl * WIC + (r + S * j) * WK + h * 16 + c16];
            }
#pragma unroll
            for (int j = 0; j < JM; ++j) {
                const double bv = (double)bx[j];
#pragma unroll
                for (int r = 0; r < S; ++r)
#pragma unroll
                    for (int h = 0; h < 2; ++h) acc[r][h] = __builtin_amdgcn_mfma_f64_16x16x4f64((double)aw[j][r][h], bv, acc[r][h], 0, 0, 0);
            }
        }
        __syncthreads();
    }
    const int64_t q = q0 + qw * 16 + c16;
#pragma unroll
    for (int r = 0; r < S; ++r) {
        const int64_t o = q * S + r - p;
        if (o < 0 || o >= OL) continue;
#pragma unroll
        for (int h = 0; h < 2; ++h)
#pragma unroll
            for (int e = 0; e < 4; ++e) {
                const int oc = oc0 + h * 16 + kq + 4 * e;
                if (oc >= OC) continue;
                if (part) part[((int64_t)blockIdx.z * OC + oc) * OL + o] = acc[r][h][e];
                else *(float *)(y.data + o * y.nb[0] + (int64_t)oc * y.nb[1]) = (float)acc[r][h][e];
            }
    }
}

void launch_conv_transpose_1d(tts_hip_backend * be, const tts_tensor * node) {
    const tts_tensor * w = node->src[0];
    const tts_tensor * x = node->src[1];
    const int s = node->op_params[0], p = node->op_params[1], d = node->op_params[2], g = node->op_params[4];
    const bool w16 = w->type == TTS_TYPE_F16;
    const size_t wal = w16 ? 8 : 16;
    const bool wvec = w->nb[0] == (w16 ? 2u : 4u) && w->nb[1] % wal == 0 && w->nb[2] % wal == 0 && ((uintptr_t)w->data % 16) == 0;
    if (d == 1 && g == 1 && w->ne[1] >= 16 && x->ne[1] >= 16 && (s == 2 || s == 4 || s == 6 || s == 8 || s == 10) && w->ne[0] == 2 * s && wvec &&
        be->convt_lds && node->nb[0] == 4) {
        const int64_t nq = (node->ne[0] + p) / s + 1;
        dim3 grid((unsigned)((nq + 63) / 64), (unsigned)((w->ne[1] + 31) / 32));
        const TD Y = make_td(node), X = make_td(x), W = make_td(w);
        const int64_t IC = x->ne[1], OL = node->ne[0], OC = node->ne[1];
        const int64_t nchunk = (IC + 15) / 16;
        const int nz = split_count(be, (int64_t)grid.x * grid.y, nchunk, 2, OL * OC);
        const int icps = nz > 1 ? (int)(((nchunk + nz - 1) / nz) * 16) : 0;
        double * part = nz > 1 ? be->conv_part : nullptr;
        grid.z = nz > 1 ? (unsigned)((IC + icps - 1) / icps) : 1u;
#define TTS_CONVT_LDS(SS)                                                                                       \
    do {                                                                                                        \
        if (w16) hipLaunchKernelGGL((k_convt_f64_lds<SS, true>), grid, dim3(256), 0, be->stream, Y, X, W, p, part, icps);  \
        else hipLaunchKernelGGL((k_convt_f64_lds<SS, false>), grid, dim3(256), 0, be->stream, Y, X, W, p, part, icps);     \
    } while (0)
        if (s == 2) TTS_CONVT_LDS(2);
        else if (s == 4) TTS_CONVT_LDS(4);
        else if (s == 6) TTS_CONVT_LDS(6);
        else if (s == 8) TTS_CONVT_LDS(8);
        else TTS_CONVT_LDS(10);
#undef TTS_CONVT_LDS
        TTS_HIP_CHECK(hipGetLastError());
        if (part) launch_split_reduce(be, (int)grid.z, OL, OC, (float *)node->data, (int64_t)(node->nb[1] / 4), nullptr, 0, nullptr, 0);
        return;
    }
    if (d == 1 && g == 1 && w->ne[1] >= 16 && x->ne[1] >= 16) {
        const int64_t nq = (node->ne[0] + p) / s + 1;
        const dim3 grid((unsigned)((nq + 15) / 16), (unsigned)((w->ne[1] + 15) / 16), (unsigned)s);
        hipLaunchKernelGGL(k_conv_transpose_1d_mfma, grid, dim3(64), 0, be->stream, make_td(node), make_td(x), make_td(w), s, p);
        TTS_HIP_CHECK(hipGetLastError());
        return;
    }
    const dim3 grid((unsigned)((node->ne[0] + 255) / 256), (unsigned)node->ne[1]);
    hipLaunchKernelGGL(k_conv_transpose_1d, grid, dim3(256), 0, be->stream, make_td(node), make_td(x), make_td(w), node->op_params[0],
                       node->op_params[1], node->op_params[2], node->op_params[4]);
    TTS_HIP_CHECK(hipGetLastError());
}

}
```

### tts.cpp_amd/ttship/__init__.py

```python
import ctypes
import os
import pathlib

_HERE = pathlib.Path(__file__).resolve().parent
PKG_ROOT = _HERE.parent
REPO_ROOT = PKG_ROOT.parent
LIB_PATH = PKG_ROOT / "lib" / "libtts_hip.so"

F32, F16, Q4_0, Q5_0, Q8_0, Q4_K, Q6_K, Q8_K, I32 = 0, 1, 2, 6, 8, 12, 14, 15, 26
QUANT_MIX_Q4_K_M = 1
PROF_ATTN = 39

OPS = ["NONE", "DUP", "ADD", "SUB", "MUL", "DIV", "SQR", "SQRT", "SIN", "COS", "SUM_ROWS", "REPEAT",
       "CONCAT", "NORM", "RMS_NORM", "MUL_MAT", "SCALE", "CPY", "CONT", "RESHAPE", "VIEW", "PERMUTE",
       "TRANSPOSE", "GET_ROWS", "SOFT_MAX", "ROPE", "CLAMP", "CONV_TRANSPOSE_1D", "IM2COL", "UPSCALE",
       "PAD", "LEAKY_RELU", "UNARY", "CUMSUM", "MOD", "ROUND", "STFT", "ISTFT", "MAP_CUSTOM3", "MAP_CUSTOM2"]
OP = {n: i for i, n in enumerate(OPS)}
FUSE = {"LN": 1, "GROUP": 2, "KV": 4, "EPI": 8, "HEADS": 16, "ATTN": 32, "LSTM": 64, "SNAKE": 128, "EMBED": 256, "CONV": 512, "ADAIN": 1024, "XATTN": 2048, "MCPY": 4096, "CONTREAD": 8192}
FUSE_ALL = sum(FUSE.values())
UNARY = {"ABS": 0, "NEG": 1, "TANH": 2, "RELU": 3, "SIGMOID": 4, "GELU": 5, "SILU": 6, "EXP": 7}

OPT = {"FUSION": 0, "PROFILE_GEMV": 1, "GRAPHS": 2, "CONV_F32ACC": 3, "CONVT_LDS": 4, "ATTN_SPLIT": 5, "KV_PREFETCH": 6, "KV_PREFETCH_BLOCKS": 7, "Q4K_TILE_BYTES": 8, "GEMV_DEBUG": 10, "GEMV_UNIQUE": 11, "CONV_SPLIT": 12, "GEMV_KS": 13, "ATTN_FUSED": 14, "ATTN_PV16": 15, "Q4K_DUAL_BYTES": 16, "GEMV_RSPLIT": 17, "GEMM_Q8": 18, "BGEMM_F32": 19, "CU_PARTITION": 20, "GEMV_PREQUANT": 21, "GEMV_KRELAY": 22, "ATTN_KS": 23, "ATTN_PV8": 24, "GEMV_NW_MIN": 25, "GEMV_KRELAY_LOOP": 26, "GEMV_Q80_PRO": 27, "GEMV_Q80_SLAB": 28, "GEMV_Q80_RW": 29, "GEMM_Q8_STAGED": 30, "GEMV_KR_INKERNEL": 31, "GEMV_F32_WIDE": 32, "ATTN_PV_MP": 33, "GEMM_KR_NW": 34, "GEMM_KR_INKERNEL": 35, "GEMM_KR_CT2": 36, "COALESCE": 37, "GEMM_KR_XCD": 38, "GEMM_KR_CP": 39, "GEMM_KR_WALK": 40, "GEMM_PF": 41, "GEMM_PF_NW": 42, "ATTN_ONE": 43, "GEMV_KR_TAIL": 44, "GEMV_Q50_SLAB": 45, "GEMV_Q50_RW": 46, "GEMM_Q5": 47, "GEMM_Q5_STAGED": 48, "GEMV_Q40_SLAB": 49, "GEMV_Q40_RW": 50, "GEMM_Q4_0": 51, "GEMM_Q4_0_STAGED": 52, "CONV_VFMA": 53, "CONV_TILE96": 54, "CONV_PACK": 55}
ATTN_SPLIT_DEFAULT = 128
ATTN_ONE_DEFAULT = 1
GEMV_KR_TAIL_DEFAULT = 1
ATTN_FUSED_ON = 128

TYPE_SIZE = {F32: 4, F16: 2, Q4_K: 144, Q6_K: 210, Q8_0: 34, Q5_0: 22, Q4_0: 18, I32: 4}
BLCK_SIZE = {F32: 1, F16: 1, Q4_K: 256, Q6_K: 256, Q8_0: 32, Q5_0: 32, Q4_0: 32, I32: 1}


class TtsTensor(ctypes.Structure):
    pass


TtsTensor._fields_ = [
    ("type", ctypes.c_int32),
    ("op", ctypes.c_int32),
    ("ne", ctypes.c_int64 * 4),
    ("nb", ctypes.c_uint64 * 4),
    ("op_params", ctypes.c_int32 * 16),
    ("src", ctypes.POINTER(TtsTensor) * 4),
    ("view_src", ctypes.POINTER(TtsTensor)),
    ("view_offs", ctypes.c_uint64),
    ("data", ctypes.c_void_p),
    ("flags", ctypes.c_int32),
    ("pad_", ctypes.c_int32),
    ("name", ctypes.c_char * 64),
]


class BackendIface(ctypes.Structure):
    _fields_ = [
        ("ctx", ctypes.c_void_p),
        ("name", ctypes.c_char_p),
        ("alloc", ctypes.c_void_p),
        ("free", ctypes.c_void_p),
        ("set", ctypes.c_void_p),
        ("set_tensor", ctypes.c_void_p),
        ("get", ctypes.c_void_p),
        ("memset", ctypes.c_void_p),
        ("compute", ctypes.c_void_p),
        ("synchronize", ctypes.c_void_p),
        ("prepare", ctypes.c_void_p),
        ("launch", ctypes.c_void_p),
        ("set_async", ctypes.c_void_p),
        ("copy", ctypes.c_void_p),
        ("greedy_step", ctypes.c_void_p),
        ("sample_step", ctypes.c_void_p),
    ]


class Sampling(ctypes.Structure):
    _fields_ = [
        ("temperature", ctypes.c_float),
        ("top_p", ctypes.c_float),
        ("repetition_penalty", ctypes.c_float),
        ("top_k", ctypes.c_int32),
        ("do_sample", ctypes.c_int32),
        ("pad_", ctypes.c_int32),
        ("seed", ctypes.c_uint64),
    ]


def sampling(**kw):
    c = Sampling()
    lib().tts_sampling_default(ctypes.byref(c))
    for k, v in kw.items():
        setattr(c, k, v)
    return c


def call_seed(seed, stream, call):
    return int(lib().tts_sampler_call_seed(seed, stream, call))


def host_sample(cfg, logits, call_seed_, last=None, count=None):
    import numpy as np
    lg = np.ascontiguousarray(logits, dtype=np.float32)
    NH, V = lg.shape
    out = np.zeros(NH, dtype=np.int32)
    if last is None:
        last = np.full(NH, -1, dtype=np.int32)
    if count is None:
        count = np.zeros(NH, dtype=np.int32)
    st = lib().tts_sampler_sample(ctypes.byref(cfg), lg.ctypes.data, NH, V, call_seed_, last.ctypes.data, count.ctypes.data, out.ctypes.data)
    if st != 0:
        raise RuntimeError(f"tts_sampler_sample failed {st}")
    return out


class ParlerConfig(ctypes.Structure):
    _fields_ = [
        ("n_layers", ctypes.c_int32),
        ("hidden_size", ctypes.c_int32),
        ("n_attn_heads", ctypes.c_int32),
        ("ffn_size", ctypes.c_int32),
        ("n_output_heads", ctypes.c_int32),
        ("output_vocab", ctypes.c_int32),
        ("audio_vocab", ctypes.c_int32),
        ("max_ctx", ctypes.c_int32),
        ("n_encode", ctypes.c_int32),
        ("prompt_vocab", ctypes.c_int32),
        ("max_positions", ctypes.c_int32),
        ("weight_type", ctypes.c_int32),
        ("head_type", ctypes.c_int32),
        ("use_cross_attn", ctypes.c_int32),
        ("batch", ctypes.c_int32),
        ("eos_token", ctypes.c_int32),
        ("bos_token", ctypes.c_int32),
        ("seed", ctypes.c_uint64),
        ("arena_bytes", ctypes.c_uint64),
        ("debug_no_reuse", ctypes.c_int32),
        ("pad_", ctypes.c_int32),
    ]


class T5Config(ctypes.Structure):
    _fields_ = [
        ("n_layers", ctypes.c_int32),
        ("hidden_size", ctypes.c_int32),
        ("n_attn_heads", ctypes.c_int32),
        ("head_size", ctypes.c_int32),
        ("ffn_size", ctypes.c_int32),
        ("relative_attn_buckets", ctypes.c_int32),
        ("vocab_size", ctypes.c_int32),
        ("max_context_length", ctypes.c_int32),
        ("output_size", ctypes.c_int32),
        ("has_down_proj", ctypes.c_int32),
        ("weight_type", ctypes.c_int32),
        ("eos_token_id", ctypes.c_int32),
        ("seed", ctypes.c_uint64),
        ("arena_bytes", ctypes.c_uint64),
        ("debug_no_reuse", ctypes.c_int32),
        ("pad_", ctypes.c_int32),
    ]


class OrpheusConfig(ctypes.Structure):
    _fields_ = [
        ("n_layers", ctypes.c_int32),
        ("hidden_size", ctypes.c_int32),
        ("n_attn_heads", ctypes.c_int32),
        ("n_kv_attn_heads", ctypes.c_int32),
        ("head_size", ctypes.c_int32),
        ("ffn_size", ctypes.c_int32),
        ("vocab_size", ctypes.c_int32),
        ("max_ctx", ctypes.c_int32),
        ("weight_type", ctypes.c_int32),
        ("batch", ctypes.c_int32),
        ("seed", ctypes.c_uint64),
        ("arena_bytes", ctypes.c_uint64),
        ("rope_theta", ctypes.c_float),
        ("rope_factor", ctypes.c_float),
        ("rope_low_freq_factor", ctypes.c_float),
# ... 1395 lines not shown
```

Baseline: 122.4.

## Pre-pack transposed-conv weights into MFMA tile layout and cache x offsets in registers

Adds a cached, pre-packed weight image for the DAC transposed convolutions, produced by a new pack kernel and keyed by a new kind field. A new kernel, k_convt_f64_img, streams weights from that image as contiguous 16-byte pieces instead of gathering strided weights. The packed conv1d kernel gains an XREG variant that loads the input-offset table into registers once, rather than re-reading it from LDS on every chunk. Both are on by default and only apply when the weights are a stable constant leaf; the cost is the extra memory for the packed image and a one-time packing step.

Measured after the change: 125.1, median of 6. 2.2% higher.

```diff
diff --git a/include/tts_hip.h b/include/tts_hip.h
--- a/include/tts_hip.h
+++ b/include/tts_hip.h
@@ -226,6 +226,8 @@
     TTS_HIP_OPT_CONV_VFMA = 53,
     TTS_HIP_OPT_CONV_TILE96 = 54,
     TTS_HIP_OPT_CONV_PACK = 55,
+    TTS_HIP_OPT_CONVT_PACK = 56,
+    TTS_HIP_OPT_CONV_XREG = 57,
     TTS_HIP_OPT_COALESCE = 37,
 };
 enum tts_fuse_bits {
diff --git a/tts.cpp_amd/csrc/backend.hip b/tts.cpp_amd/csrc/backend.hip
--- a/tts.cpp_amd/csrc/backend.hip
+++ b/tts.cpp_amd/csrc/backend.hip
@@ -181,6 +181,10 @@
         if (e[0] >= '0' && e[0] <= '2' && !e[1]) be->conv_vfma = e[0] - '0';
     if (const char * e = getenv("TTS_HIP_OPT_CONV_PACK"))
         if (e[0] >= '0' && e[0] <= '1' && !e[1]) be->conv_pack = e[0] - '0';
+    if (const char * e = getenv("TTS_HIP_OPT_CONVT_PACK"))
+        if (e[0] >= '0' && e[0] <= '1' && !e[1]) be->convt_pack = e[0] - '0';
+    if (const char * e = getenv("TTS_HIP_OPT_CONV_XREG"))
+        if (e[0] >= '0' && e[0] <= '1' && !e[1]) be->conv_xreg = e[0] - '0';
     be->conv_part_doubles = (size_t)8 << 20;
     TTS_HIP_CHECK(hipMalloc((void **)&be->conv_part, be->conv_part_doubles * sizeof(double)));
     be->lstm_floats = kLstmFloats;
@@ -811,6 +815,8 @@
         case TTS_HIP_OPT_CONV_VFMA: be->conv_vfma = value < 0 || value > 2 ? 1 : value; return 0;
         case TTS_HIP_OPT_CONV_TILE96: be->conv_tile96 = value != 0; return 0;
         case TTS_HIP_OPT_CONV_PACK: be->conv_pack = value != 0; return 0;
+        case TTS_HIP_OPT_CONVT_PACK: be->convt_pack = value != 0; return 0;
+        case TTS_HIP_OPT_CONV_XREG: be->conv_xreg = value != 0; return 0;
         case TTS_HIP_OPT_PROFILE_GEMV: be->profile_gemv = value != 0; return 0;
         case TTS_HIP_OPT_GRAPHS: be->use_graphs = value != 0; return 0;
         case TTS_HIP_OPT_CONV_F32ACC:
diff --git a/tts.cpp_amd/csrc/graph_exec.hip b/tts.cpp_amd/csrc/graph_exec.hip
--- a/tts.cpp_amd/csrc/graph_exec.hip
+++ b/tts.cpp_amd/csrc/graph_exec.hip
@@ -1336,6 +1336,22 @@
     static const tts_tensor * through_view(const tts_tensor * t) { return t && t->op == TTS_OP_RESHAPE ? t->src[0] : t; }
     bool wr_hull = false;
     const char *wr_lo = nullptr, *wr_hi = nullptr;
+    bool const_leaf(const tts_tensor * kern) {
+        if (kern->op != TTS_OP_NONE || (kern->flags & (TTS_FLAG_HOSTDATA | TTS_FLAG_OUTPUT)) || !buffer_lookup(kern->data, nullptr, nullptr)) return false;
+        if (!wr_hull) {
+            wr_hull = true;
+            for (int j = 0; j < n; ++j) {
+                if (is_view(nodes[j]->op) || !nodes[j]->data) continue;
+                const char * lo = (const char *)nodes[j]->data;
+                wr_lo = wr_lo ? std::min(wr_lo, lo) : lo;
+                wr_hi = std::max(wr_hi, lo + tbytes(nodes[j]));
+            }
+        }
+        if (wr_lo && (const char *)kern->data < wr_hi && (const char *)kern->data + tbytes(kern) > wr_lo)
+            for (int j = 0; j < n; ++j)
+                if (!is_view(nodes[j]->op) && nodes[j]->data && overlap(nodes[j], kern)) return false;
+        return true;
+    }
     void try_conv(int i) {
         const tts_tensor * col = nodes[i];
         const tts_tensor *kern = col->src[0], *x = col->src[1];
@@ -1428,19 +1444,7 @@
         const size_t wb = tbytes(kern);
         if (xb >= 0x80000000u || wb >= 0x80000000u) return plan_reject("conv", 12);
         a.x_bytes = (uint32_t)xb, a.w_bytes = (uint32_t)wb;
-        a.w_stable = kern->op == TTS_OP_NONE && !(kern->flags & (TTS_FLAG_HOSTDATA | TTS_FLAG_OUTPUT)) && buffer_lookup(kern->data, nullptr, nullptr);
-        if (a.w_stable && !wr_hull) {
-            wr_hull = true;
-            for (int j = 0; j < n; ++j) {
-                if (is_view(nodes[j]->op) || !nodes[j]->data) continue;
-                const char * lo = (const char *)nodes[j]->data;
-                wr_lo = wr_lo ? std::min(wr_lo, lo) : lo;
-                wr_hi = std::max(wr_hi, lo + tbytes(nodes[j]));
-            }
-        }
-        if (a.w_stable && wr_lo && (const char *)kern->data < wr_hi && (const char *)kern->data + wb > wr_lo)
-            for (int j = 0; a.w_stable && j < n; ++j)
-                if (!is_view(nodes[j]->op) && nodes[j]->data && overlap(nodes[j], kern)) a.w_stable = 0;
+        a.w_stable = const_leaf(kern);
         Item it;
         it.kind = Item::CONV;
         it.conv = a;
@@ -2677,16 +2681,21 @@
 static void plan_setup(Planner & pl, const tts_hip_backend * be);
 }
 static void conv_pack_prepare(tts_hip_backend * be, tts_tensor * const * nodes, int n_nodes) {
-    if (!be->conv_pack || !(be->fusion & TTS_FUSE_CONV)) return;
+    const bool conv = be->conv_pack && (be->fusion & TTS_FUSE_CONV), convt = be->convt_pack && be->fusion;
     bool any = false;
-    for (int i = 0; i < n_nodes && !any; ++i) any = nodes[i]->op == TTS_OP_IM2COL;
+    for (int i = 0; i < n_nodes && !any; ++i) any = (conv && nodes[i]->op == TTS_OP_IM2COL) || (convt && nodes[i]->op == TTS_OP_CONV_TRANSPOSE_1D);
     if (!any) return;
     Planner pl;
     plan_setup(pl, be);
     pl.build(nodes, n_nodes);
     for (const Item & it : pl.items) {
         ConvPackKey k;
-        if (it.kind == Item::CONV && conv1d_pack_key(be, it.conv, &k)) (void)conv_pack_get(be, k);
+        if (conv && it.kind == Item::CONV && conv1d_pack_key(be, it.conv, &k)) (void)conv_pack_get(be, k);
+    }
+    for (int i = 0; convt && i < n_nodes; ++i) {
+        ConvPackKey k;
+        if (pl.act[i] == 0 && nodes[i]->op == TTS_OP_CONV_TRANSPOSE_1D && !be->bat && convt_pack_key(be, nodes[i], pl.const_leaf(nodes[i]->src[0]), &k))
+            (void)conv_pack_get(be, k);
     }
 }
 
@@ -2949,7 +2958,11 @@
             TTS_HIP_CHECK(hipStreamWaitEvent(be->stream, be->pf_join, 0));
             pf_pending = -1;
         }
-        const int st = a > 0 ? run_item(be, pl.items[a - 1], pl.items) : run_node(be, n);
+        int st = 0;
+        if (a > 0) st = run_item(be, pl.items[a - 1], pl.items);
+        else if (n->op == TTS_OP_CONV_TRANSPOSE_1D && be->fusion && be->convt_pack && !be->bat)
+            launch_conv_transpose_1d(be, n, pl.const_leaf(n->src[0]));
+        else st = run_node(be, n);
         if (is_pf) {
             ++pf_next;
             pf_fork();
diff --git a/tts.cpp_amd/csrc/hip_internal.h b/tts.cpp_amd/csrc/hip_internal.h
--- a/tts.cpp_amd/csrc/hip_internal.h
+++ b/tts.cpp_amd/csrc/hip_internal.h
@@ -429,6 +429,8 @@
     int conv_vfma = 1;
     int conv_tile96 = 1;
     int conv_pack = 1;
+    int convt_pack = 1;
+    int conv_xreg = 1;
     bool capturing = false;
     int conv_split = 1;
     int fusion = 0x3FFF;
@@ -530,7 +532,7 @@
 void launch_lstm_finish(tts_hip_backend * be, const tts_tensor * final_out, const float * hist, int64_t Hd, int64_t T);
 bool audio_op_supported(const tts_tensor * n);
 int launch_audio_op(tts_hip_backend * be, const tts_tensor * n);
-void launch_conv_transpose_1d(tts_hip_backend * be, const tts_tensor * node);
+void launch_conv_transpose_1d(tts_hip_backend * be, const tts_tensor * node, int w_stable = 0);
 constexpr int CONV1D_MAX_R = 128;
 struct Conv1dArgs {
     TD x;
@@ -571,14 +573,16 @@
     const int lane = (r & 3) * 16 + (row & 15);
     return (int64_t)(ct * nchunk + chunk) * oct * rp + ((((row >> 4) * (rp >> 4) + (r >> 4)) * 64 + lane) * 4 + ((r >> 2) & 3));
 }
+__host__ __device__ inline int convt_pack_index(int tap, int half, int icl, int c16) { return (((tap * 2 + half) * 16 + icl) * 16) + c16; }
 struct ConvPackKey {
     const tts_hip_backend * be;
     const void * w;
+    int kind = 0;
     int w16, K, oct, icc, rp;
     int64_t IC, OC, wk, wic, woc;
     bool operator<(const ConvPackKey & o) const {
-        return std::tie(be, w, w16, K, oct, icc, rp, IC, OC, wk, wic, woc) <
-               std::tie(o.be, o.w, o.w16, o.K, o.oct, o.icc, o.rp, o.IC, o.OC, o.wk, o.wic, o.woc);
+        return std::tie(be, w, kind, w16, K, oct, icc, rp, IC, OC, wk, wic, woc) <
+               std::tie(o.be, o.w, o.kind, o.w16, o.K, o.oct, o.icc, o.rp, o.IC, o.OC, o.wk, o.wic, o.woc);
     }
     int nchunk() const { return (int)((IC + icc - 1) / icc); }
     int ntile() const { return (int)((OC + oct - 1) / oct); }
@@ -589,6 +593,7 @@
 void conv_pack_written(tts_hip_backend * be, const void * p, size_t n);
 void conv_pack_freed(const tts_hip_backend * be, const void * p, size_t n);
 bool conv1d_pack_key(const tts_hip_backend * be, const Conv1dArgs & a, ConvPackKey * k);
+bool convt_pack_key(const tts_hip_backend * be, const tts_tensor * node, int w_stable, ConvPackKey * k);
 struct AdainArgs {
     const float * x = nullptr;
     int64_t xcs = 0;
diff --git a/tts.cpp_amd/csrc/k_conv.hip b/tts.cpp_amd/csrc/k_conv.hip
--- a/tts.cpp_amd/csrc/k_conv.hip
+++ b/tts.cpp_amd/csrc/k_conv.hip
@@ -449,13 +449,30 @@
     img[conv1d_pack_index(nchunk, k.oct, k.rp, ct, chunk, row, r)] = v;
 }
 
+__global__ __launch_bounds__(256) void k_convt_pack(ConvPackKey k, float * __restrict__ img, int nchunk, int64_t n) {
+    const int64_t e = (int64_t)blockIdx.x * 256 + threadIdx.x;
+    if (e >= n) return;
+    const int per = 512 * k.K;
+    const int slice = (int)(e / per), w = (int)(e - (int64_t)slice * per);
+    const int ct = slice / nchunk, chunk = slice - ct * nchunk;
+    const int c16 = w & 15, icl = (w >> 4) & 15, half = (w >> 8) & 1, tap = w >> 9;
+    const int64_t oc = (int64_t)ct * 32 + half * 16 + c16, ic = (int64_t)chunk * 16 + icl;
+    float v = 0.f;
+    if (ic < k.IC && oc < k.OC) {
+        const int64_t o = oc * k.woc + (int64_t)tap * k.wk + ic * k.wic;
+        v = k.w16 ? __half2float(((const __half *)k.w)[o]) : ((const float *)k.w)[o];
+    }
+    img[(int64_t)slice * per + convt_pack_index(tap, half, icl, c16)] = v;
+}
+
 void launch_conv1d_pack(hipStream_t stream, const ConvPackKey & k, float * img) {
     const int64_t n = (int64_t)k.floats();
-    hipLaunchKernelGGL(k_conv1d_pack, dim3((unsigned)((n + 255) / 256)), dim3(256), 0, stream, k, img, k.nchunk(), n);
+    if (k.kind == 1) hipLaunchKernelGGL(k_convt_pack, dim3((unsigned)((n + 255) / 256)), dim3(256), 0, stream, k, img, k.nchunk(), n);
+    else hipLaunchKernelGGL(k_conv1d_pack,dim3((unsigned)((n + 255) / 256)), dim3(256), 0, stream, k, img, k.nchunk(), n);
     TTS_HIP_CHECK(hipGetLastError());
 }
 
-template <bool BIAS, bool RES, int MT>
+template <bool BIAS, bool RES, int MT, bool XREG>
 __global__ __launch_bounds__(256) __attribute__((amdgpu_waves_per_eu(MT == 2 ? 1 : 2))) void k_conv1d_f64p(Conv1dArgs a) {
     constexpr int OCT = 32 * MT, WQ = 2 * MT;
     extern __shared__ float sm[];
@@ -477,6 +494,13 @@
     __syncthreads();
     const int wr0 = (wave >> 1) * 16 * MT, wc0 = (wave & 1) * 32;
     const bool wave_live = oc0 + wr0 < a.OC && ol0 + wc0 < a.OL;
+    int xoa[2][8];
+    if (XREG) {
+#pragma unroll
+        for (int b = 0; b < 2; ++b)
+#pragma unroll
+            for (int u = 0; u < 8; ++u) xoa[b][u] = 32 * b < Rp ? xoff[32 * b + 4 * u + kq] : zslot;
+    }
     f64x4_t acc[MT][2] = {};
     const int64_t base = ol0 * s - a.p;
     const int EX = icc * xw;
@@ -527,10 +551,7 @@
             __syncthreads();
             continue;
         }
-        for (int r0 = 0; r0 < Rp; r0 += 32) {
-            int xo[8];
-#pragma unroll
-            for (int u = 0; u < 8; ++u) xo[u] = xoff[r0 + 4 * u + kq];
+        auto batch = [&](int r0, const int (&xo)[8]) {
             float af[8][MT], bf[8][2];
 #pragma unroll
             for (int h = 0; h < 2; ++h)
@@ -553,6 +574,17 @@
 #pragma unroll
                     for (int tj = 0; tj < 2; ++tj)
                         acc[ti][tj] = __builtin_amdgcn_mfma_f64_16x16x4f64((double)af[u][ti], (double)bf[u][tj], acc[ti][tj], 0, 0, 0);
+        };
+        if (XREG) {
+            batch(0, xoa[0]);
+            if (Rp == 64) batch(32, xoa[1]);
+        } else {
+            for (int r0 = 0; r0 < Rp; r0 += 32) {
+                int xo[8];
+#pragma unroll
+                for (int u = 0; u < 8; ++u) xo[u] = xoff[r0 + 4 * u + kq];
+                batch(r0, xo);
+            }
         }
         __syncthreads();
     }
@@ -664,8 +696,8 @@
     int vxw = 0, vicc = 0;
     size_t vlds = 0;
     if (be->conv_vfma && (be->conv_vfma == 2 || a.OC < 8) && conv1d_vfma_geometry(a, &vxw, &vicc, &vlds)) return false;
-    k->be = be, k->w = a.w, k->w16 = a.w16, k->K = a.K;
-    k->oct = be->conv_tile96 && a.OC % 96 == 0 ? 96 : 64;
+    k->be = be, k->w = a.w, k->kind = 0, k->w16 = a.w16, k->K = a.K;
+    k->oct =be->conv_tile96 && a.OC % 96 == 0 ? 96 : 64;
     k->icc = a.icc, k->rp = (a.icc * a.K + 31) & ~31;
     k->IC = a.IC, k->OC = a.OC, k->wk = a.wk, k->wic = a.wic, k->woc = a.woc;
     return true;
@@ -716,16 +748,19 @@
         const size_t plds = ((size_t)pk.oct * pk.rp + (size_t)a.icc * a.xw + 1) * 4;
         grid.y = (unsigned)pk.ntile();
         const int psel = (pk.oct == 96 ? 4 : 0) | (a.bias ? 2 : 0) | (a.res ? 1 : 0);
-        switch (psel) {
-            case 0: hipLaunchKernelGGL((k_conv1d_f64p<false, false, 2>), grid, dim3(256), plds, be->stream, a); break;
-            case 1: hipLaunchKernelGGL((k_conv1d_f64p<false, true, 2>), grid, dim3(256), plds, be->stream, a); break;
-            case 2: hipLaunchKernelGGL((k_conv1d_f64p<true, false, 2>), grid, dim3(256), plds, be->stream, a); break;
-            case 3: hipLaunchKernelGGL((k_conv1d_f64p<true, true, 2>), grid, dim3(256), plds, be->stream, a); break;
-            case 4: hipLaunchKernelGGL((k_conv1d_f64p<false, false, 3>), grid, dim3(256), plds, be->stream, a); break;
-            case 5: hipLaunchKernelGGL((k_conv1d_f64p<false, true, 3>), grid, dim3(256), plds, be->stream, a); break;
-            case 6: hipLaunchKernelGGL((k_conv1d_f64p<true, false, 3>), grid, dim3(256), plds, be->stream, a); break;
-            default: hipLaunchKernelGGL((k_conv1d_f64p<true, true, 3>), grid, dim3(256), plds, be->stream, a); break;
-        }
+#define TTS_CONV1D_PACKED(XREG)                                                                                                     \
+    switch (psel) {                                                                                                                  \
+        case 0: hipLaunchKernelGGL((k_conv1d_f64p<false, false, 2, XREG>), grid, dim3(256), plds, be->stream, a); break;             \
+        case 1: hipLaunchKernelGGL((k_conv1d_f64p<false, true, 2, XREG>), grid, dim3(256), plds, be->stream, a); break;              \
+        case 2: hipLaunchKernelGGL((k_conv1d_f64p<true, false, 2, XREG>), grid, dim3(256), plds, be->stream, a); break;              \
+        case 3: hipLaunchKernelGGL((k_conv1d_f64p<true, true, 2, XREG>), grid, dim3(256), plds, be->stream, a); break;               \
+        case 4: hipLaunchKernelGGL((k_conv1d_f64p<false, false, 3, XREG>), grid, dim3(256), plds, be->stream, a); break;             \
+        case 5: hipLaunchKernelGGL((k_conv1d_f64p<false, true, 3, XREG>), grid, dim3(256), plds, be->stream, a); break;              \
+        case 6: hipLaunchKernelGGL((k_conv1d_f64p<true, false, 3, XREG>), grid, dim3(256), plds, be->stream, a); break;              \
+        default: hipLaunchKernelGGL((k_conv1d_f64p<true, true, 3, XREG>), grid, dim3(256), plds, be->stream, a); break;              \
+    }
+        if (be->conv_xreg) { TTS_CONV1D_PACKED(true) } else { TTS_CONV1D_PACKED(false) }
+#undef TTS_CONV1D_PACKED
     } else if (nz == 1 && be->conv_acc_mode != 2 && be->conv_tile96 && a.OC % 96 == 0) {
         grid.y = (unsigned)(a.OC / 96);
         lds += 32 * (size_t)a.rs * 4;
@@ -928,25 +963,168 @@
     }
 }
 
-void launch_conv_transpose_1d(tts_hip_backend * be, const tts_tensor * node) {
+template <int S, bool W16, int NWV>
+__global__ __launch_bounds__(64 * NWV) __attribute__((amdgpu_waves_per_eu(NWV == 8 ? (S <= 8 ? 4 : 2) : 1))) void k_convt_f64_img(TD y, TD x, uint32_t x_bytes, const float * __restrict__ wimg, int OC, int IC, int p) {
+    constexpr int JM = 2, K = 2 * S, NT = 64 * NWV, HN = NWV == 8 ? 1 : 2;
+    constexpr int QT = 64, OCT = 32, ICC = 16, XW = QT + JM - 1, XWP = 80;
+    constexpr int NX = ICC * XW, NW4 = ICC * K * OCT / 4;
+    constexpr int XR = (NX + NT - 1) / NT, WR = NW4 / NT;
+    static_assert(NW4 % NT == 0, "whole 16-byte pieces per thread");
+    __shared__ float xs[ICC][XWP];
+    __shared__ f32x4_t ws4[NW4];
+    const float * ws = (const float *)ws4;
+    const int tid = threadIdx.x, lane = tid & 63, qw = (tid >> 6) & 3, h0 = NWV == 8 ? tid >> 8 : 0;
+    const int c16 = lane & 15, kq = lane >> 4;
+    const int64_t L = x.ne[0], OL = y.ne[0];
+    const int64_t q0 = (int64_t)blockIdx.x * QT;
+    const int oc0 = blockIdx.y * OCT;
+    f64x4_t acc[S][HN];
+#pragma unroll
+    for (int r = 0; r < S; ++r)
+#pragma unroll
+        for (int h = 0; h < HN; ++h) acc[r][h] = (f64x4_t){0.0, 0.0, 0.0, 0.0};
+    const int nchunk = (IC + ICC - 1) / ICC;
+    const f32x4_t * wp = (const f32x4_t *)wimg + (int64_t)blockIdx.y * nchunk * NW4 + tid;
+    const uint32_t OOB = 0x80000000u;
+    const auto xd = __builtin_amdgcn_make_buffer_rsrc(x.data, 0, x_bytes, 0x00020000);
+    uint32_t xrel[XR];
+#pragma unroll
+    for (int u = 0; u < XR; ++u) {
+        const int t = tid + NT * u;
+        const int ic = t / XW, qq = t - ic * XW;
+        const int64_t pos = q0 - (JM - 1) + qq;
+        xrel[u] = t < NX && pos >= 0 && pos < L ? (uint32_t)(pos * x.nb[0] + (int64_t)ic * x.nb[1]) : OOB;
+    }
+    float xr[XR];
+    f32x4_t wr[WR];
+    auto fetch = [&](int ic0) {
+        const int nic = min(ICC, IC - ic0);
+        const uint32_t xc = (uint32_t)((int64_t)ic0 * x.nb[1]);
+#pragma unroll
+        for (int u = 0; u < XR; ++u) {
+            const uint32_t off = (xrel[u] == OOB || tid + NT * u >= nic * XW) ? OOB : xrel[u] + xc;
+            xr[u] = __builtin_bit_cast(float, __builtin_amdgcn_raw_buffer_load_b32(xd, off, 0, 0));
+            if (W16) xr[u] = __half2float(__float2half_rn(xr[u]));
+        }
+#pragma unroll
+        for (int u = 0; u < WR; ++u) wr[u] = wp[NT * u];
+        wp += NW4;
+    };
+    fetch(0);
+    for (int ic0 = 0; ic0 < IC; ic0 += ICC) {
+#pragma unroll
+        for (int u = 0; u < XR; ++u) {
+            const int t = tid + NT * u;
+            if (t < NX) xs[t / XW][t % XW] = xr[u];
+        }
+#pragma unroll
+        for (int u = 0; u < WR; ++u) ws4[tid + NT * u] = wr[u];
+        __syncthreads();
+        if (ic0 + ICC < IC) fetch(ic0 + ICC);
+#pragma unroll
+        for (int kk = 0; kk < 4; ++kk) {
+            const int icl = 4 * kk + kq;
+            float bx[JM], aw[JM][S][HN];
+#pragma unroll
+            for (int j = 0; j < JM; ++j) {
+                bx[j] = xs[icl][qw * 16 + c16 + (JM - 1) - j];
+#pragma unroll
+                for (int r = 0; r < S; ++r)
+#pragma unroll
+                    for (int h = 0; h < HN; ++h) aw[j][r][h] = ws[convt_pack_index(r + S * j, h0 + h, icl, c16)];
+            }
+#pragma unroll
+            for (int j = 0; j < JM; ++j) {
+                const double bv = (double)bx[j];
+#pragma unroll
+                for (int r = 0; r < S; ++r)
+#pragma unroll
+                    for (int h = 0; h < HN; ++h) acc[r][h] = __builtin_amdgcn_mfma_f64_16x16x4f64((double)aw[j][r][h], bv, acc[r][h], 0, 0, 0);
+            }
+        }
+        __syncthreads();
+    }
+    const int64_t q = q0 + qw * 16 + c16;
+#pragma unroll
+    for (int r = 0; r < S; ++r) {
+        const int64_t o = q * S + r - p;
+        if (o < 0 || o >= OL) continue;
+#pragma unroll
+        for (int h = 0; h < HN; ++h)
+#pragma unroll
+            for (int e = 0; e < 4; ++e) {
+                const int oc = oc0 + (h0 + h) * 16 + kq + 4 * e;
+                if (oc < OC) *(float *)(y.data + o * y.nb[0] + (int64_t)oc * y.nb[1]) = (float)acc[r][h][e];
+            }
+    }
+}
+
+static bool convt_lds_geometry(const tts_hip_backend * be, const tts_tensor * node, dim3 * grid, int * nz, int * icps) {
     const tts_tensor * w = node->src[0];
     const tts_tensor * x = node->src[1];
     const int s = node->op_params[0], p = node->op_params[1], d = node->op_params[2], g = node->op_params[4];
     const bool w16 = w->type == TTS_TYPE_F16;
     const size_t wal = w16 ? 8 : 16;
     const bool wvec = w->nb[0] == (w16 ? 2u : 4u) && w->nb[1] % wal == 0 && w->nb[2] % wal == 0 && ((uintptr_t)w->data % 16) == 0;
-    if (d == 1 && g == 1 && w->ne[1] >= 16 && x->ne[1] >= 16 && (s == 2 || s == 4 || s == 6 || s == 8 || s == 10) && w->ne[0] == 2 * s && wvec &&
-        be->convt_lds && node->nb[0] == 4) {
-        const int64_t nq = (node->ne[0] + p) / s + 1;
-        dim3 grid((unsigned)((nq + 63) / 64), (unsigned)((w->ne[1] + 31) / 32));
+    if (!(d == 1 && g == 1 && w->ne[1] >= 16 && x->ne[1] >= 16 && (s == 2 || s == 4 || s == 6 || s == 8 || s == 10) && w->ne[0] == 2 * s && wvec &&
+          be->convt_lds && node->nb[0] == 4))
+        return false;
+    const int64_t nq = (node->ne[0] + p) / s + 1;
+    *grid = dim3((unsigned)((nq + 63) / 64), (unsigned)((w->ne[1] + 31) / 32));
+    const int64_t IC = x->ne[1], OL = node->ne[0], OC = node->ne[1];
+    const int64_t nchunk = (IC + 15) / 16;
+    *nz = split_count(be, (int64_t)grid->x * grid->y, nchunk, 2, OL * OC);
+    *icps = *nz > 1 ? (int)(((nchunk + *nz - 1) / *nz) * 16) : 0;
+    grid->z = *nz > 1 ? (unsigned)((IC + *icps - 1) / *icps) : 1u;
+    return true;
+}
+
+static size_t convt_x_bytes(const tts_tensor * x) { return (size_t)((x->ne[0] - 1) * x->nb[0] + (x->ne[1] - 1) * x->nb[1]) + 4; }
+
+bool convt_pack_key(const tts_hip_backend * be, const tts_tensor * node, int w_stable, ConvPackKey * k) {
+    if (!be->convt_pack || !w_stable) return false;
+    dim3 grid;
+    int nz = 1, icps = 0;
+    if (!convt_lds_geometry(be, node, &grid, &nz, &icps) || nz > 1) return false;
+    if (convt_x_bytes(node->src[1]) >= 0x80000000u) return false;
+    const tts_tensor * w = node->src[0];
+    const int64_t es = w->type == TTS_TYPE_F16 ? 2 : 4;
+    k->be = be, k->w = w->data, k->kind = 1, k->w16 = w->type == TTS_TYPE_F16, k->K = (int)w->ne[0];
+    k->oct = 32, k->icc = 16, k->rp = 16 * k->K;
+    k->IC = w->ne[2], k->OC = w->ne[1];
+    k->wk = (int64_t)w->nb[0] / es, k->woc = (int64_t)w->nb[1] / es, k->wic = (int64_t)w->nb[2] / es;
+    return true;
+}
+
+void launch_conv_transpose_1d(tts_hip_backend * be, const tts_tensor * node, int w_stable) {
+    const tts_tensor * w = node->src[0];
+    const tts_tensor * x = node->src[1];
+    const int s = node->op_params[0], p = node->op_params[1], d = node->op_params[2], g = node->op_params[4];
+    const bool w16 = w->type == TTS_TYPE_F16;
+    dim3 grid;
+    int nz = 1, icps = 0;
+    if (convt_lds_geometry(be, node, &grid, &nz, &icps)) {
         const TD Y = make_td(node), X = make_td(x), W = make_td(w);
-        const int64_t IC = x->ne[1], OL = node->ne[0], OC = node->ne[1];
-        const int64_t nchunk = (IC + 15) / 16;
-        const int nz = split_count(be, (int64_t)grid.x * grid.y, nchunk, 2, OL * OC);
-        const int icps = nz > 1 ? (int)(((nchunk + nz - 1) / nz) * 16) : 0;
+        const int64_t OL = node->ne[0], OC = node->ne[1];
         double * part = nz > 1 ? be->conv_part : nullptr;
-        grid.z = nz > 1 ? (unsigned)((IC + icps - 1) / icps) : 1u;
-#define TTS_CONVT_LDS(SS)                                                                                       \
+        ConvPackKey pk;
+        if (const float * img = convt_pack_key(be, node, w_stable, &pk) ? conv_pack_get(be, pk) : nullptr) {
+            const uint32_t xb = (uint32_t)convt_x_bytes(x);
+#define TTS_CONVT_IMG(SS, NWV)                                                                                                              \
+    do {                                                                                                                                    \
+        if (w16) hipLaunchKernelGGL((k_convt_f64_img<SS, true, NWV>), grid, dim3(64 * NWV), 0, be->stream, Y, X, xb, img, (int)OC, (int)x->ne[1], p);  \
+        else hipLaunchKernelGGL((k_convt_f64_img<SS, false, NWV>), grid, dim3(64 * NWV), 0, be->stream, Y, X, xb, img, (int)OC, (int)x->ne[1], p);     \
+    } while (0)
+            if (s == 2) TTS_CONVT_IMG(2, 4);
+            else if (s == 4) TTS_CONVT_IMG(4, 4);
+            else if (s == 6) TTS_CONVT_IMG(6, 8);
+            else if (s == 8) TTS_CONVT_IMG(8, 8);
+            else TTS_CONVT_IMG(10, 8);
+#undef TTS_CONVT_IMG
+            TTS_HIP_CHECK(hipGetLastError());
+            return;
+        }
+#define TTS_CONVT_LDS(SS)                                                                                      \
     do {                                                                                                        \
         if (w16) hipLaunchKernelGGL((k_convt_f64_lds<SS, true>), grid, dim3(256), 0, be->stream, Y, X, W, p, part, icps);  \
         else hipLaunchKernelGGL((k_convt_f64_lds<SS, false>), grid, dim3(256), 0, be->stream, Y, X, W, p, part, icps);     \
@@ -963,13 +1141,13 @@
     }
     if (d == 1 && g == 1 && w->ne[1] >= 16 && x->ne[1] >= 16) {
         const int64_t nq = (node->ne[0] + p) / s + 1;
-        const dim3 grid((unsigned)((nq + 15) / 16), (unsigned)((w->ne[1] + 15) / 16), (unsigned)s);
-        hipLaunchKernelGGL(k_conv_transpose_1d_mfma, grid, dim3(64), 0, be->stream, make_td(node), make_td(x), make_td(w), s, p);
+        const dim3 mgrid((unsigned)((nq + 15) / 16), (unsigned)((w->ne[1] + 15) / 16), (unsigned)s);
+        hipLaunchKernelGGL(k_conv_transpose_1d_mfma, mgrid, dim3(64), 0, be->stream, make_td(node), make_td(x), make_td(w), s, p);
         TTS_HIP_CHECK(hipGetLastError());
         return;
     }
-    const dim3 grid((unsigned)((node->ne[0] + 255) / 256), (unsigned)node->ne[1]);
-    hipLaunchKernelGGL(k_conv_transpose_1d, grid, dim3(256), 0, be->stream, make_td(node), make_td(x), make_td(w), node->op_params[0],
+    const dim3 vgrid((unsigned)((node->ne[0] + 255) / 256), (unsigned)node->ne[1]);
+    hipLaunchKernelGGL(k_conv_transpose_1d, vgrid, dim3(256), 0, be->stream, make_td(node), make_td(x), make_td(w), node->op_params[0],
                        node->op_params[1], node->op_params[2], node->op_params[4]);
     TTS_HIP_CHECK(hipGetLastError());
 }
diff --git a/tts.cpp_amd/ttship/__init__.py b/tts.cpp_amd/ttship/__init__.py
--- a/tts.cpp_amd/ttship/__init__.py
+++ b/tts.cpp_amd/ttship/__init__.py
@@ -20,7 +20,7 @@
 FUSE_ALL = sum(FUSE.values())
 UNARY = {"ABS": 0, "NEG": 1, "TANH": 2, "RELU": 3, "SIGMOID": 4, "GELU": 5, "SILU": 6, "EXP": 7}
 
-OPT = {"FUSION": 0, "PROFILE_GEMV": 1, "GRAPHS": 2, "CONV_F32ACC": 3, "CONVT_LDS": 4, "ATTN_SPLIT": 5, "KV_PREFETCH": 6, "KV_PREFETCH_BLOCKS": 7, "Q4K_TILE_BYTES": 8, "GEMV_DEBUG": 10, "GEMV_UNIQUE": 11, "CONV_SPLIT": 12, "GEMV_KS": 13, "ATTN_FUSED": 14, "ATTN_PV16": 15, "Q4K_DUAL_BYTES": 16, "GEMV_RSPLIT": 17, "GEMM_Q8": 18, "BGEMM_F32": 19, "CU_PARTITION": 20, "GEMV_PREQUANT": 21, "GEMV_KRELAY": 22, "ATTN_KS": 23, "ATTN_PV8": 24, "GEMV_NW_MIN": 25, "GEMV_KRELAY_LOOP": 26, "GEMV_Q80_PRO": 27, "GEMV_Q80_SLAB": 28, "GEMV_Q80_RW": 29, "GEMM_Q8_STAGED": 30, "GEMV_KR_INKERNEL": 31, "GEMV_F32_WIDE": 32, "ATTN_PV_MP": 33, "GEMM_KR_NW": 34, "GEMM_KR_INKERNEL": 35, "GEMM_KR_CT2": 36, "COALESCE": 37, "GEMM_KR_XCD": 38, "GEMM_KR_CP": 39, "GEMM_KR_WALK": 40, "GEMM_PF": 41, "GEMM_PF_NW": 42, "ATTN_ONE": 43, "GEMV_KR_TAIL": 44, "GEMV_Q50_SLAB": 45, "GEMV_Q50_RW": 46, "GEMM_Q5": 47, "GEMM_Q5_STAGED": 48, "GEMV_Q40_SLAB": 49, "GEMV_Q40_RW": 50, "GEMM_Q4_0": 51, "GEMM_Q4_0_STAGED": 52, "CONV_VFMA": 53, "CONV_TILE96": 54, "CONV_PACK": 55}
+OPT = {"FUSION": 0, "PROFILE_GEMV": 1, "GRAPHS": 2, "CONV_F32ACC": 3, "CONVT_LDS": 4, "ATTN_SPLIT": 5, "KV_PREFETCH": 6, "KV_PREFETCH_BLOCKS": 7, "Q4K_TILE_BYTES": 8, "GEMV_DEBUG": 10, "GEMV_UNIQUE": 11, "CONV_SPLIT": 12, "GEMV_KS": 13, "ATTN_FUSED": 14, "ATTN_PV16": 15, "Q4K_DUAL_BYTES": 16, "GEMV_RSPLIT": 17, "GEMM_Q8": 18, "BGEMM_F32": 19, "CU_PARTITION": 20, "GEMV_PREQUANT": 21, "GEMV_KRELAY": 22, "ATTN_KS": 23, "ATTN_PV8": 24, "GEMV_NW_MIN": 25, "GEMV_KRELAY_LOOP": 26, "GEMV_Q80_PRO": 27, "GEMV_Q80_SLAB": 28, "GEMV_Q80_RW": 29, "GEMM_Q8_STAGED": 30, "GEMV_KR_INKERNEL": 31, "GEMV_F32_WIDE": 32, "ATTN_PV_MP": 33, "GEMM_KR_NW": 34, "GEMM_KR_INKERNEL": 35, "GEMM_KR_CT2": 36, "COALESCE": 37, "GEMM_KR_XCD": 38, "GEMM_KR_CP": 39, "GEMM_KR_WALK": 40, "GEMM_PF": 41, "GEMM_PF_NW": 42, "ATTN_ONE": 43, "GEMV_KR_TAIL": 44, "GEMV_Q50_SLAB": 45, "GEMV_Q50_RW": 46, "GEMM_Q5": 47, "GEMM_Q5_STAGED": 48, "GEMV_Q40_SLAB": 49, "GEMV_Q40_RW": 50, "GEMM_Q4_0": 51, "GEMM_Q4_0_STAGED": 52, "CONV_VFMA": 53, "CONV_TILE96": 54, "CONV_PACK": 55, "CONVT_PACK": 56, "CONV_XREG": 57}
 ATTN_SPLIT_DEFAULT = 128
 ATTN_ONE_DEFAULT = 1
 GEMV_KR_TAIL_DEFAULT = 1
```
